# Vandermode/TFPnP

Hardware: AMD Instinct MI355X
Metric: PnP-ADMM iters/sec (and images/sec) at env_batch=48, 256x256, 30 inner iters (higher is better)
Workload: dtype f32 (v_mfma_f32_32x32x2_f32; Winograd F(2x2,3x3) on the layers with cout % 32 == 0); 1 GPU; CS-MRI ADMM 256x256 env_batch=48/GPU radial x4 sigma_n=15, 6 solver calls x 5 inner iters + PSNR reward, no early stop; global_batch=48, parallelism=single GPU

## Files before the change

### include/pnpx.h

```cpp
#ifndef PNPX_H
#define PNPX_H

#include <stddef.h>
#include <stdint.h>

#ifdef __cplusplus
extern "C" {
#endif

typedef struct pnpx_ctx pnpx_ctx;

enum pnpx_status {
  PNPX_OK = 0,
  PNPX_ERR_ARG = 1,
  PNPX_ERR_SHAPE = 2,
  PNPX_ERR_NO_WEIGHTS = 3,
  PNPX_ERR_ALLOC = 4,
  PNPX_ERR_HIP = 5,
  PNPX_ERR_RANGE = 6
};

const char* pnpx_version(void);
const char* pnpx_last_error(void);

int pnpx_ctx_create(int device, pnpx_ctx** out);
int pnpx_ctx_destroy(pnpx_ctx* ctx);
int pnpx_ctx_reserve(pnpx_ctx* ctx, int B, int H, int W);
int pnpx_ctx_set_option(pnpx_ctx* ctx, const char* key, int value);
int pnpx_ctx_get_option(pnpx_ctx* ctx, const char* key, int* value);
int pnpx_ctx_status(pnpx_ctx* ctx);
size_t pnpx_ctx_bytes(const pnpx_ctx* ctx);

size_t pnpx_unet_num_params(void);
int pnpx_unet_load(pnpx_ctx* ctx, const float* params_host, size_t n_params);
int pnpx_unet_denoise(pnpx_ctx* ctx, const float* x, const float* sigma, float* out, float* out_preclamp,
                      int B, int H, int W, void* stream);
size_t pnpx_drunet_num_params(int nb);
int pnpx_drunet_load(pnpx_ctx* ctx, const float* params_host, size_t n_params, int nb);
int pnpx_unet_denoise_backward(pnpx_ctx* ctx, const float* x, const float* sigma, const float* grad_out,
                               float* grad_x, float* grad_sigma, int B, int H, int W, void* stream);
int pnpx_unet_denoise_train(pnpx_ctx* ctx, const float* x, const float* sigma, float* out, int B, int H, int W,
                            unsigned long long* ticket, void* stream);
int pnpx_unet_denoise_backward_ticket(pnpx_ctx* ctx, const float* x, const float* sigma, const float* grad_out,
                                      float* grad_x, float* grad_sigma, int B, int H, int W, unsigned long long ticket,
                                      void* stream);
int pnpx_unet_profile(pnpx_ctx* ctx, const float* x, const float* sigma, float* out, int B, int H, int W,
                      void* stream, int cap, float* ms_out, double* flops_out, const char** names_out,
                      int* n_out);

size_t pnpx_policy_num_params(int num_inputs, int n_det, int spi_head);
int pnpx_policy_load(pnpx_ctx* ctx, const float* params_host, size_t n_params, int num_inputs, int n_det,
                     int spi_head);
int pnpx_policy_forward(pnpx_ctx* ctx, const float* ob, float* probs, float* det, int B, int H, int W,
                        void* stream);
int pnpx_policy_load_device(pnpx_ctx* ctx, const float* params_dev, size_t n_params, int num_inputs, int n_det, int spi_head,
                            void* stream);
int pnpx_policy_params(pnpx_ctx* ctx, float* dst_dev, size_t n_params, void* stream);
int pnpx_policy_forward_train(pnpx_ctx* ctx, const float* ob, float* probs, float* det, int B, int H, int W, float momentum,
                              int update_running, void* stream);
size_t pnpx_policy_num_bn_channels(void);
int pnpx_policy_bn_stats(pnpx_ctx* ctx, float* mean_dev, float* var_dev, size_t n, void* stream);
int pnpx_policy_param_grad(pnpx_ctx* ctx, const float* ob, const float* grad_probs , const float* grad_det ,
                           float* grad_params, size_t n_params, int B, int H, int W, void* stream);
int pnpx_policy_forward_train_keep(pnpx_ctx* ctx, const float* ob, float* probs, float* det, int B, int H, int W, float momentum,
                                   int update_running, void* stream);
int pnpx_policy_param_grad_kept(pnpx_ctx* ctx, const float* grad_probs , const float* grad_det ,
                                float* grad_params, size_t n_params, void* stream);
int pnpx_policy_adam_step(pnpx_ctx* ctx, const float* grad_dev, size_t n_params, float lr, float beta1, float beta2, float eps,
                          float max_norm, float* grad_norm_dev, void* stream);
int pnpx_policy_optim_state(pnpx_ctx* ctx, float* exp_avg_dst, float* exp_avg_sq_dst, size_t n_params, long long* step_host,
                            void* stream);
int pnpx_policy_optim_reset(pnpx_ctx* ctx);
int pnpx_policy_frozen_ranges(int num_inputs, int n_det, int spi_head, size_t* first, size_t* count, int capacity);

size_t pnpx_critic_num_params(int num_inputs);
int pnpx_critic_load(pnpx_ctx* ctx, const float* params_host, size_t n_params, int num_inputs);
int pnpx_critic_load_device(pnpx_ctx* ctx, const float* params_dev, size_t n_params, int num_inputs, void* stream);
int pnpx_critic_soft_update(pnpx_ctx* ctx, const float* src_params_dev, size_t n_params, float one_minus_tau, float tau,
                            void* stream);
int pnpx_critic_params(pnpx_ctx* ctx, float* dst_dev, size_t n_params, void* stream);
int pnpx_critic_forward(pnpx_ctx* ctx, const float* ob, float* value, int B, int H, int W, void* stream);
int pnpx_critic_backward(pnpx_ctx* ctx, const float* ob, const float* grad_value, float* grad_ob, int B, int H, int W,
                         void* stream);

int pnpx_critic_param_grad(pnpx_ctx* ctx, const float* ob, const float* grad_value, float* grad_params, size_t n_params, int B,
                           int H, int W, void* stream);
int pnpx_critic_value_loss_grad(pnpx_ctx* ctx, const float* ob, const float* q_target, float* value, float* loss, float* grad_params,
                                size_t n_params, int B, int H, int W, void* stream);
int pnpx_critic_adam_step(pnpx_ctx* ctx, const float* grad_dev, size_t n_params, float lr, float beta1, float beta2, float eps,
                          float max_norm, float* grad_norm_dev, void* stream);
int pnpx_critic_optim_state(pnpx_ctx* ctx, float* exp_avg_dst, float* exp_avg_sq_dst, size_t n_params, long long* step_host,
                            void* stream);
int pnpx_critic_optim_reset(pnpx_ctx* ctx);

int pnpx_fft2(pnpx_ctx* ctx, const float* in, float* out, int n_img, int H, int W, int inverse,
              int centered, void* stream);
int pnpx_cdp_forward(pnpx_ctx* ctx, const float* x, const float* mask, float* out, int B, int S, int H,
                     int W, void* stream);
int pnpx_cdp_backward(pnpx_ctx* ctx, const float* y, const float* mask, float* out, int B, int S, int H,
                      int W, void* stream);
int pnpx_spi_inverse(pnpx_ctx* ctx, const float* ztilde, const float* K1, const float* K, const float* mu,
                     float* out, int B, int H, int W, void* stream);
int pnpx_psnr(pnpx_ctx* ctx, const float* output, const float* gt, float* psnr, int B, int n_per_item,
              void* stream);

int pnpx_rows_gather(pnpx_ctx* ctx, int n_tensors, const void* const* src_host, void* const* dst_host,
                     const size_t* row_bytes_host, const int64_t* idx, int n_rows, void* stream);
int pnpx_rows_scatter(pnpx_ctx* ctx, int n_tensors, const void* const* src_host, void* const* dst_host,
                      const size_t* row_bytes_host, const int64_t* idx, int n_rows, void* stream);
int pnpx_ring_store(pnpx_ctx* ctx, int n_tensors, const void* const* src_host, void* const* dst_host,
                    const size_t* row_bytes_host, int64_t first_slot, int64_t capacity, int n_rows, void* stream);
int pnpx_live_compact(pnpx_ctx* ctx, const int64_t* idx_left, const int64_t* idx_stop, int n, int64_t* idx_out,
                      int* n_live_host, void* stream);
int pnpx_policy_ob_pack(pnpx_ctx* ctx, int n_entries, const void* const* src_host, const int* kind_host,
                        const int* channels_host, const int64_t* idx, int n_rows, int H, int W, float* out,
                        void* stream);

int pnpx_policy_ob_unpack(pnpx_ctx* ctx, int n_entries, void* const* dst_host, const int* kind_host,
                          const int* channels_host, int n_rows, int H, int W, const float* grad_out, void* stream);


int pnpx_csmri_admm(pnpx_ctx* ctx, const float* vars_in, float* vars_out, const float* y0,
                    const uint8_t* mask, const float* sigma_d, const float* mu, int param_stride, int B,
                    int H, int W, int T, void* stream);
int pnpx_csmri_admm_train(pnpx_ctx* ctx, const float* vars_in, float* vars_out, const float* y0,
                          const uint8_t* mask, const float* sigma_d, const float* mu, int param_stride, int B,
                          int H, int W, int T, float* saved, unsigned long long* ticket, void* stream);
int pnpx_csmri_admm_backward(pnpx_ctx* ctx, const float* y0, const uint8_t* mask, const float* sigma_d,
                             const float* mu, int param_stride, const float* saved, const float* grad_vars_out,
                             float* grad_vars_in, float* grad_sigma_d, float* grad_mu, float* work, int B, int H,
                             int W, int T, unsigned long long ticket, void* stream);
int pnpx_csmri_hqs(pnpx_ctx* ctx, const float* vars_in, float* vars_out, const float* y0,
                   const uint8_t* mask, const float* sigma_d, const float* mu, int param_stride, int B,
                   int H, int W, int T, void* stream);
int pnpx_csmri_hqs_train(pnpx_ctx* ctx, const float* vars_in, float* vars_out, const float* y0,
                         const uint8_t* mask, const float* sigma_d, const float* mu, int param_stride, int B,
                         int H, int W, int T, float* saved, unsigned long long* ticket, void* stream);
int pnpx_csmri_hqs_backward(pnpx_ctx* ctx, const float* y0, const uint8_t* mask, const float* sigma_d,
                            const float* mu, int param_stride, const float* saved, const float* grad_vars_out,
                            float* grad_vars_in, float* grad_sigma_d, float* grad_mu, float* work, int B, int H,
                            int W, int T, unsigned long long ticket, void* stream);
int pnpx_csmri_pg(pnpx_ctx* ctx, const float* vars_in, float* vars_out, const float* y0,
                  const uint8_t* mask, const float* sigma_d, const float* tau, int param_stride, int B,
                  int H, int W, int T, void* stream);
int pnpx_csmri_pg_train(pnpx_ctx* ctx, const float* vars_in, float* vars_out, const float* y0,
                        const uint8_t* mask, const float* sigma_d, const float* tau, int param_stride, int B,
                        int H, int W, int T, float* saved, unsigned long long* ticket, void* stream);
int pnpx_csmri_pg_backward(pnpx_ctx* ctx, const float* y0, const uint8_t* mask, const float* sigma_d,
                           const float* tau, int param_stride, const float* saved, const float* grad_vars_out,
                           float* grad_vars_in, float* grad_sigma_d, float* grad_tau, float* work, int B, int H,
                           int W, int T, unsigned long long ticket, void* stream);
int pnpx_csmri_apg(pnpx_ctx* ctx, const float* vars_in, float* vars_out, const float* y0,
                   const uint8_t* mask, const float* sigma_d, const float* tau, const float* beta,
                   int param_stride, int B, int H, int W, int T, void* stream);
int pnpx_csmri_apg_train(pnpx_ctx* ctx, const float* vars_in, float* vars_out, const float* y0,
                         const uint8_t* mask, const float* sigma_d, const float* tau, const float* beta,
                         int param_stride, int B, int H, int W, int T, float* saved, unsigned long long* ticket,
                         void* stream);
int pnpx_csmri_apg_backward(pnpx_ctx* ctx, const float* y0, const uint8_t* mask, const float* sigma_d,
                            const float* tau, const float* beta, int param_stride, const float* saved,
                            const float* grad_vars_out, float* grad_vars_in, float* grad_sigma_d, float* grad_tau,
                            float* grad_beta, float* work, int B, int H, int W, int T, unsigned long long ticket,
                            void* stream);
int pnpx_csmri_redadmm(pnpx_ctx* ctx, const float* vars_in, float* vars_out, const float* y0,
                       const uint8_t* mask, const float* sigma_d, const float* mu, const float* lamda,
                       int param_stride, int B, int H, int W, int T, void* stream);
int pnpx_csmri_redadmm_train(pnpx_ctx* ctx, const float* vars_in, float* vars_out, const float* y0,
                             const uint8_t* mask, const float* sigma_d, const float* mu, const float* lamda,
                             int param_stride, int B, int H, int W, int T, float* saved, unsigned long long* ticket,
                             void* stream);
int pnpx_csmri_redadmm_backward(pnpx_ctx* ctx, const float* y0, const uint8_t* mask, const float* sigma_d,
                                const float* mu, const float* lamda, int param_stride, const float* saved,
                                const float* grad_vars_out, float* grad_vars_in, float* grad_sigma_d, float* grad_mu,
                                float* grad_lamda, float* work, int B, int H, int W, int T, unsigned long long ticket,
                                void* stream);
int pnpx_csmri_amp(pnpx_ctx* ctx, const float* vars_in, float* vars_out, const float* y0, const uint8_t* mask,
                   const float* sigma_d, const float* probe, int param_stride, int B, int H, int W, int T,
                   void* stream);
int pnpx_pr_iadmm(pnpx_ctx* ctx, const float* vars_in, float* vars_out, const float* y0,
                  const float* mask, const float* sigma_d, const float* mu, const float* tau,
                  int param_stride, int B, int S, int H, int W, int T, void* stream);
int pnpx_pr_iadmm_train(pnpx_ctx* ctx, const float* vars_in, float* vars_out, const float* y0, const float* mask,
                        const float* sigma_d, const float* mu, const float* tau, int param_stride, int B, int S,
                        int H, int W, int T, float* saved, unsigned long long* ticket, void* stream);
int pnpx_pr_iadmm_backward(pnpx_ctx* ctx, const float* y0, const float* mask, const float* sigma_d, const float* mu,
                           const float* tau, int param_stride, const float* saved, const float* grad_vars_out,
                           float* grad_vars_in, float* grad_sigma_d, float* grad_mu, float* grad_tau, float* work,
                           int B, int S, int H, int W, int T, unsigned long long ticket, void* stream);
int pnpx_pr_pg(pnpx_ctx* ctx, const float* vars_in, float* vars_out, const float* y0, const float* mask,
               const float* sigma_d, const float* tau, int param_stride, int B, int S, int H, int W, int T,
               void* stream);
int pnpx_pr_pg_train(pnpx_ctx* ctx, const float* vars_in, float* vars_out, const float* y0, const float* mask,
                     const float* sigma_d, const float* tau, int param_stride, int B, int S, int H, int W, int T,
                     float* saved, unsigned long long* ticket, void* stream);
int pnpx_pr_pg_backward(pnpx_ctx* ctx, const float* y0, const float* mask, const float* sigma_d, const float* tau,
                        int param_stride, const float* saved, const float* grad_vars_out, float* grad_vars_in,
                        float* grad_sigma_d, float* grad_tau, float* work, int B, int S, int H, int W, int T,
                        unsigned long long ticket, void* stream);
int pnpx_spi_admm(pnpx_ctx* ctx, const float* vars_in, float* vars_out, const float* x0,
                  const float* Kmap, const float* sigma_d, const float* mu, int param_stride, int B, int H,
                  int W, int T, void* stream);
int pnpx_spi_admm_train(pnpx_ctx* ctx, const float* vars_in, float* vars_out, const float* x0, const float* Kmap,
                        const float* sigma_d, const float* mu, int param_stride, int B, int H, int W, int T,
                        float* saved, unsigned long long* ticket, void* stream);
int pnpx_spi_admm_backward(pnpx_ctx* ctx, const float* x0, const float* Kmap, const float* sigma_d, const float* mu,
                           int param_stride, const float* saved, const float* grad_vars_out, float* grad_vars_in,
                           float* grad_sigma_d, float* grad_mu, float* work, int B, int H, int W, int T,
                           unsigned long long ticket, void* stream);

int pnpx_radon_det_count(int R);
int pnpx_radon_forward(pnpx_ctx* ctx, const float* img, float* sino, int B, int R, int n_view, void* stream);
int pnpx_radon_backprojection(pnpx_ctx* ctx, const float* sino, float* img, int B, int R, int n_view,
                              void* stream);
int pnpx_ct_iadmm(pnpx_ctx* ctx, const float* vars_in, float* vars_out, const float* y0, int n_view,
                  float opnorm, const float* sigma_d, const float* mu, const float* tau, int param_stride,
                  int B, int R, int T, void* stream);
int pnpx_ct_iadmm_train(pnpx_ctx* ctx, const float* vars_in, float* vars_out, const float* y0, int n_view,
                        float opnorm, const float* sigma_d, const float* mu, const float* tau, int param_stride, int B,
                        int R, int T, float* saved, unsigned long long* ticket, void* stream);
int pnpx_ct_iadmm_backward(pnpx_ctx* ctx, int n_view, float opnorm, const float* sigma_d, const float* mu,
                           const float* tau, int param_stride, const float* saved, const float* grad_vars_out,
                           float* grad_vars_in, float* grad_sigma_d, float* grad_mu, float* grad_tau, float* work,
                           int B, int R, int T, unsigned long long ticket, void* stream);
int pnpx_ct_pg(pnpx_ctx* ctx, const float* vars_in, float* vars_out, const float* y0, int n_view,
               float opnorm, const float* sigma_d, const float* tau, int param_stride, int B, int R, int T,
               void* stream);
int pnpx_ct_pg_train(pnpx_ctx* ctx, const float* vars_in, float* vars_out, const float* y0, int n_view, float opnorm,
                     const float* sigma_d, const float* tau, int param_stride, int B, int R, int T, float* saved,
                     unsigned long long* ticket, void* stream);
int pnpx_ct_pg_backward(pnpx_ctx* ctx, int n_view, float opnorm, const float* sigma_d, const float* tau,
                        int param_stride, const float* saved, const float* grad_vars_out, float* grad_vars_in,
                        float* grad_sigma_d, float* grad_tau, float* work, int B, int R, int T,
                        unsigned long long ticket, void* stream);

void pnpx_winof4_matrices(double* g18, double* bt36, double* at24);
int pnpx_winof4_pack(const float* w, int cout, int cin, float* dst);
int pnpx_winof4_c32_pack(const float* w, int cout, int cin, float* dst);

enum pnpx_probe_kind {
  PNPX_PROBE_DIRECT = 0,
  PNPX_PROBE_WINO4 = 1,
  PNPX_PROBE_WINO8 = 2,
  PNPX_PROBE_WINO8_KSPLIT = 3,
  PNPX_PROBE_WINOF4 = 4,
  PNPX_PROBE_WINO8_UPS = 5,
  PNPX_PROBE_DIRECT_GRAD = 6,
  PNPX_PROBE_WINO8_GRAD = 7,
  PNPX_PROBE_WINOF4_2SRC = 8,
  PNPX_PROBE_WINOF4_UPS = 9,
  PNPX_PROBE_WINOF4_FUSE_UP = 11,
  PNPX_PROBE_WINOF4_C32 = 12
};
int pnpx_conv3x3_probe(pnpx_ctx* ctx, int kind, const float* w_host, const float* bias_host, int cout, const float* in0, int C0,
                       const float* in1, int C1, float* out, const float* res, const float* mask, float slope, float* pool_out,
                       int ks_rule, int B, int H, int W, void* stream);
int pnpx_conv3x3_probe_plan(int kind, int C0, int C1, int cout, int H, int W, int ks_rule);
int pnpx_upsample2x_probe(pnpx_ctx* ctx, const float* src, float* dst, int planes, int h, int w, void* stream);

typedef struct pnpx_conv_hs_probe_desc {
  const float *w, *bias, *outc_w, *outc_b, *first_w, *first_b;
  const void *in0, *in1, *res, *dmask;
  void *out, *pool_out;
  const float *x_in, *first_x, *first_sigma;
  float *out_img, *out_pre;
  int cin, cout, G0, G1, B, H, W;
  float slope;
  int taps, in0_groups, wreg, share, ups_h, ups_w, critic_epi;
  float alpha;
  int res_groups, first_sigma_stride;
  float first_slope;
  int want_range_flag;
  unsigned* range_flag_out;
} pnpx_conv_hs_probe_desc;
enum { PNPX_CONV_HS_PLAN_INTS = 12 };
int pnpx_conv_hs_probe(pnpx_ctx* ctx, const pnpx_conv_hs_probe_desc* desc, void* stream);
int pnpx_conv_hs_probe_plan(const pnpx_conv_hs_probe_desc* desc, int B, int H, int W, int* out);

enum pnpx_vjp_glue_op {
  PNPX_VJP_OUTC_BWD = 0,
  PNPX_VJP_UPSAMPLE_BWD = 1,
  PNPX_VJP_SKIP_POOL_MERGE = 2,
  PNPX_VJP_INPUT_GRAD = 3,
  PNPX_VJP_GRAD_SCALE = 4
};
typedef struct pnpx_vjp_glue_probe_desc {
  int op, family, form;
  int B, C, H, W, Ccat, c_off, Ht, Wt;
  const void *g, *act, *g_pool;
  const float *pre, *w, *g_res, *sc;
  void* out;
  float *out_res, *part, *gsigma;
  unsigned* bits;
} pnpx_vjp_glue_probe_desc;
int pnpx_vjp_glue_probe(pnpx_ctx* ctx, const pnpx_vjp_glue_probe_desc* desc, void* stream);
int pnpx_vjp_glue_probe_plan(const pnpx_vjp_glue_probe_desc* desc);

int pnpx_conv_f32_entry_plan(int opts, int ksplit, int ksplit_rule, int C0, int C1, int cout, int H, int W, int B_call);
int pnpx_conv_f32_forward_plan(int opts, int ksplit, int ksplit_rule, int C0, int C1, int cout, int H, int W, int B_call);

#ifdef __cplusplus
}
#endif
#endif
```

### tfpnp_amd/_lib.py

```python
import ctypes as C
import os
import threading

import torch

_HERE = os.path.dirname(os.path.abspath(__file__))
LIB_PATH = os.environ.get("PNPX_LIB", os.path.join(_HERE, "libpnpx.so"))

_lib = None
_lock = threading.Lock()

c_float_p = C.POINTER(C.c_float)
c_void_p = C.c_void_p


class PnpxError(RuntimeError):
    pass


PNPX_ERR_RANGE = 6


class ConvHsProbeDesc(C.Structure):
    _fields_ = ([(n, c_void_p) for n in ("w", "bias", "outc_w", "outc_b", "first_w", "first_b", "in0", "in1", "res", "dmask", "out", "pool_out",
                                         "x_in", "first_x", "first_sigma", "out_img", "out_pre")] +
                [(n, C.c_int) for n in ("cin", "cout", "G0", "G1", "B", "H", "W")] + [("slope", C.c_float)] +
                [(n, C.c_int) for n in ("taps", "in0_groups", "wreg", "share", "ups_h", "ups_w", "critic_epi")] + [("alpha", C.c_float)] +
                [("res_groups", C.c_int), ("first_sigma_stride", C.c_int), ("first_slope", C.c_float), ("want_range_flag", C.c_int),
                 ("range_flag_out", C.POINTER(C.c_uint))])
PNPX_CONV_HS_PLAN_INTS = 12


class VjpGlueProbeDesc(C.Structure):
    _fields_ = ([(n, C.c_int) for n in ("op", "family", "form", "B", "C", "H", "W", "Ccat", "c_off", "Ht", "Wt")] +
                [(n, c_void_p) for n in ("g", "act", "g_pool", "pre", "w", "g_res", "sc", "out", "out_res", "part", "gsigma", "bits")])


_P = c_void_p
_SIGNATURES = {
    "pnpx_version": (C.c_char_p, []),
    "pnpx_last_error": (C.c_char_p, []),
    "pnpx_ctx_create": (C.c_int, [C.c_int, C.POINTER(c_void_p)]),
    "pnpx_ctx_destroy": (C.c_int, [c_void_p]),
    "pnpx_ctx_reserve": (C.c_int, [c_void_p, C.c_int, C.c_int, C.c_int]),
    "pnpx_ctx_set_option": (C.c_int, [c_void_p, C.c_char_p, C.c_int]),
    "pnpx_ctx_get_option": (C.c_int, [c_void_p, C.c_char_p, C.POINTER(C.c_int)]),
    "pnpx_ctx_status": (C.c_int, [c_void_p]),
    "pnpx_ctx_bytes": (C.c_size_t, [c_void_p]),
    "pnpx_unet_num_params": (C.c_size_t, []),
    "pnpx_unet_load": (C.c_int, [c_void_p, c_void_p, C.c_size_t]),
    "pnpx_drunet_num_params": (C.c_size_t, [C.c_int]),
    "pnpx_drunet_load": (C.c_int, [c_void_p, c_void_p, C.c_size_t, C.c_int]),
    "pnpx_unet_denoise": (C.c_int, [c_void_p, _P, _P, _P, _P, C.c_int, C.c_int, C.c_int, c_void_p]),
    "pnpx_unet_denoise_backward": (C.c_int, [c_void_p, _P, _P, _P, _P, _P, C.c_int, C.c_int, C.c_int, c_void_p]),
    "pnpx_unet_denoise_train": (C.c_int, [c_void_p, _P, _P, _P, C.c_int, C.c_int, C.c_int, C.POINTER(C.c_ulonglong), c_void_p]),
    "pnpx_unet_denoise_backward_ticket": (C.c_int, [c_void_p, _P, _P, _P, _P, _P, C.c_int, C.c_int, C.c_int,
                                                    C.c_ulonglong, c_void_p]),
    "pnpx_policy_num_params": (C.c_size_t, [C.c_int, C.c_int, C.c_int]),
    "pnpx_policy_load": (C.c_int, [c_void_p, c_void_p, C.c_size_t, C.c_int, C.c_int, C.c_int]),
    "pnpx_policy_load_device": (C.c_int, [c_void_p, _P, C.c_size_t, C.c_int, C.c_int, C.c_int, c_void_p]),
    "pnpx_policy_params": (C.c_int, [c_void_p, _P, C.c_size_t, c_void_p]),
    "pnpx_policy_forward": (C.c_int, [c_void_p, _P, _P, _P, C.c_int, C.c_int, C.c_int, c_void_p]),
    "pnpx_policy_forward_train": (C.c_int, [c_void_p, _P, _P, _P, C.c_int, C.c_int, C.c_int, C.c_float, C.c_int, c_void_p]),
    "pnpx_policy_num_bn_channels": (C.c_size_t, []),
    "pnpx_policy_bn_stats": (C.c_int, [c_void_p, _P, _P, C.c_size_t, c_void_p]),
    "pnpx_policy_param_grad": (C.c_int, [c_void_p, _P, _P, _P, _P, C.c_size_t, C.c_int, C.c_int, C.c_int, c_void_p]),
    "pnpx_policy_forward_train_keep": (C.c_int, [c_void_p, _P, _P, _P, C.c_int, C.c_int, C.c_int, C.c_float, C.c_int, c_void_p]),
    "pnpx_policy_param_grad_kept": (C.c_int, [c_void_p, _P, _P, _P, C.c_size_t, c_void_p]),
    "pnpx_policy_adam_step": (C.c_int, [c_void_p, _P, C.c_size_t] + [C.c_float] * 5 + [_P, c_void_p]),
    "pnpx_policy_optim_state": (C.c_int, [c_void_p, _P, _P, C.c_size_t, C.POINTER(C.c_longlong), c_void_p]),
    "pnpx_policy_optim_reset": (C.c_int, [c_void_p]),
    "pnpx_policy_frozen_ranges": (C.c_int, [C.c_int, C.c_int, C.c_int, C.POINTER(C.c_size_t), C.POINTER(C.c_size_t), C.c_int]),
    "pnpx_critic_num_params": (C.c_size_t, [C.c_int]),
    "pnpx_critic_load": (C.c_int, [c_void_p, c_void_p, C.c_size_t, C.c_int]),
    "pnpx_critic_load_device": (C.c_int, [c_void_p, _P, C.c_size_t, C.c_int, c_void_p]),
    "pnpx_critic_soft_update": (C.c_int, [c_void_p, _P, C.c_size_t, C.c_float, C.c_float, c_void_p]),
    "pnpx_critic_params": (C.c_int, [c_void_p, _P, C.c_size_t, c_void_p]),
    "pnpx_critic_forward": (C.c_int, [c_void_p, _P, _P, C.c_int, C.c_int, C.c_int, c_void_p]),
    "pnpx_critic_backward": (C.c_int, [c_void_p, _P, _P, _P, C.c_int, C.c_int, C.c_int, c_void_p]),
    "pnpx_critic_param_grad": (C.c_int, [c_void_p, _P, _P, _P, C.c_size_t, C.c_int, C.c_int, C.c_int, c_void_p]),
    "pnpx_critic_value_loss_grad": (C.c_int, [c_void_p, _P, _P, _P, _P, _P, C.c_size_t, C.c_int, C.c_int, C.c_int, c_void_p]),
    "pnpx_critic_adam_step": (C.c_int, [c_void_p, _P, C.c_size_t] + [C.c_float] * 5 + [_P, c_void_p]),
    "pnpx_critic_optim_state": (C.c_int, [c_void_p, _P, _P, C.c_size_t, C.POINTER(C.c_longlong), c_void_p]),
    "pnpx_critic_optim_reset": (C.c_int, [c_void_p]),
    "pnpx_unet_profile": (C.c_int, [c_void_p, _P, _P, _P, C.c_int, C.c_int, C.c_int, c_void_p, C.c_int,
                                    c_float_p, C.POINTER(C.c_double), C.POINTER(C.c_char_p), C.POINTER(C.c_int)]),
    "pnpx_fft2": (C.c_int, [c_void_p, _P, _P, C.c_int, C.c_int, C.c_int, C.c_int, C.c_int, c_void_p]),
    "pnpx_cdp_forward": (C.c_int, [c_void_p, _P, _P, _P, C.c_int, C.c_int, C.c_int, C.c_int, c_void_p]),
    "pnpx_cdp_backward": (C.c_int, [c_void_p, _P, _P, _P, C.c_int, C.c_int, C.c_int, C.c_int, c_void_p]),
    "pnpx_spi_inverse": (C.c_int, [c_void_p, _P, _P, _P, _P, _P, C.c_int, C.c_int, C.c_int, c_void_p]),
    "pnpx_psnr": (C.c_int, [c_void_p, _P, _P, _P, C.c_int, C.c_int, c_void_p]),
    "pnpx_rows_gather": (C.c_int, [c_void_p, C.c_int, C.POINTER(c_void_p), C.POINTER(c_void_p), C.POINTER(C.c_size_t), _P,
                                   C.c_int, c_void_p]),
    "pnpx_rows_scatter": (C.c_int, [c_void_p, C.c_int, C.POINTER(c_void_p), C.POINTER(c_void_p), C.POINTER(C.c_size_t), _P,
                                    C.c_int, c_void_p]),
    "pnpx_ring_store": (C.c_int, [c_void_p, C.c_int, C.POINTER(c_void_p), C.POINTER(c_void_p), C.POINTER(C.c_size_t),
                                  C.c_int64, C.c_int64, C.c_int, c_void_p]),
    "pnpx_live_compact": (C.c_int, [c_void_p, _P, _P, C.c_int, _P, C.POINTER(C.c_int), c_void_p]),
    "pnpx_policy_ob_pack": (C.c_int, [c_void_p, C.c_int, C.POINTER(c_void_p), C.POINTER(C.c_int), C.POINTER(C.c_int), _P,
                                      C.c_int, C.c_int, C.c_int, _P, c_void_p]),
    "pnpx_policy_ob_unpack": (C.c_int, [c_void_p, C.c_int, C.POINTER(c_void_p), C.POINTER(C.c_int), C.POINTER(C.c_int),
                                        C.c_int, C.c_int, C.c_int, _P, c_void_p]),
    "pnpx_csmri_admm": (C.c_int, [c_void_p, _P, _P, _P, _P, _P, _P] + [C.c_int] * 5 + [c_void_p]),
    "pnpx_csmri_admm_train": (C.c_int, [c_void_p, _P, _P, _P, _P, _P, _P] + [C.c_int] * 5 +
                              [_P, C.POINTER(C.c_ulonglong), c_void_p]),
    "pnpx_csmri_admm_backward": (C.c_int, [c_void_p, _P, _P, _P, _P, C.c_int, _P, _P, _P, _P, _P, _P] + [C.c_int] * 4 +
                                 [C.c_ulonglong, c_void_p]),
    "pnpx_csmri_hqs_train": (C.c_int, [c_void_p, _P, _P, _P, _P, _P, _P] + [C.c_int] * 5 +
                             [_P, C.POINTER(C.c_ulonglong), c_void_p]),
    "pnpx_csmri_hqs_backward": (C.c_int, [c_void_p, _P, _P, _P, _P, C.c_int, _P, _P, _P, _P, _P, _P] + [C.c_int] * 4 +
                                [C.c_ulonglong, c_void_p]),
    "pnpx_csmri_hqs": (C.c_int, [c_void_p, _P, _P, _P, _P, _P, _P] + [C.c_int] * 5 + [c_void_p]),
    "pnpx_csmri_amp": (C.c_int, [c_void_p, _P, _P, _P, _P, _P, _P] + [C.c_int] * 5 + [c_void_p]),
    "pnpx_csmri_pg_train": (C.c_int, [c_void_p, _P, _P, _P, _P, _P, _P] + [C.c_int] * 5 +
                            [_P, C.POINTER(C.c_ulonglong), c_void_p]),
    "pnpx_csmri_pg_backward": (C.c_int, [c_void_p, _P, _P, _P, _P, C.c_int, _P, _P, _P, _P, _P, _P] + [C.c_int] * 4 +
                               [C.c_ulonglong, c_void_p]),
    "pnpx_csmri_pg": (C.c_int, [c_void_p, _P, _P, _P, _P, _P, _P] + [C.c_int] * 5 + [c_void_p]),
    "pnpx_csmri_apg_train": (C.c_int, [c_void_p, _P, _P, _P, _P, _P, _P, _P] + [C.c_int] * 5 +
                             [_P, C.POINTER(C.c_ulonglong), c_void_p]),
    "pnpx_csmri_apg_backward": (C.c_int, [c_void_p, _P, _P, _P, _P, _P, C.c_int, _P, _P, _P, _P, _P, _P, _P] + [C.c_int] * 4 +
                                [C.c_ulonglong, c_void_p]),
    "pnpx_csmri_apg": (C.c_int, [c_void_p, _P, _P, _P, _P, _P, _P, _P] + [C.c_int] * 5 + [c_void_p]),
    "pnpx_csmri_redadmm_train": (C.c_int, [c_void_p, _P, _P, _P, _P, _P, _P, _P] + [C.c_int] * 5 +
                                 [_P, C.POINTER(C.c_ulonglong), c_void_p]),
    "pnpx_csmri_redadmm_backward": (C.c_int, [c_void_p, _P, _P, _P, _P, _P, C.c_int, _P, _P, _P, _P, _P, _P, _P] +
                                    [C.c_int] * 4 + [C.c_ulonglong, c_void_p]),
    "pnpx_csmri_redadmm": (C.c_int, [c_void_p, _P, _P, _P, _P, _P, _P, _P] + [C.c_int] * 5 + [c_void_p]),
    "pnpx_pr_iadmm_train": (C.c_int, [c_void_p, _P, _P, _P, _P, _P, _P, _P] + [C.c_int] * 6 +
                            [_P, C.POINTER(C.c_ulonglong), c_void_p]),
    "pnpx_pr_iadmm_backward": (C.c_int, [c_void_p, _P, _P, _P, _P, _P, C.c_int, _P, _P, _P, _P, _P, _P, _P] + [C.c_int] * 5 +
                               [C.c_ulonglong, c_void_p]),
    "pnpx_pr_iadmm": (C.c_int, [c_void_p, _P, _P, _P, _P, _P, _P, _P] + [C.c_int] * 6 + [c_void_p]),
    "pnpx_pr_pg_train": (C.c_int, [c_void_p, _P, _P, _P, _P, _P, _P] + [C.c_int] * 6 +
                         [_P, C.POINTER(C.c_ulonglong), c_void_p]),
    "pnpx_pr_pg_backward": (C.c_int, [c_void_p, _P, _P, _P, _P, C.c_int, _P, _P, _P, _P, _P, _P] + [C.c_int] * 5 +
                            [C.c_ulonglong, c_void_p]),
    "pnpx_pr_pg": (C.c_int, [c_void_p, _P, _P, _P, _P, _P, _P] + [C.c_int] * 6 + [c_void_p]),
    "pnpx_spi_admm_train": (C.c_int, [c_void_p, _P, _P, _P, _P, _P, _P] + [C.c_int] * 5 +
                            [_P, C.POINTER(C.c_ulonglong), c_void_p]),
    "pnpx_spi_admm_backward": (C.c_int, [c_void_p, _P, _P, _P, _P, C.c_int, _P, _P, _P, _P, _P, _P] + [C.c_int] * 4 +
                               [C.c_ulonglong, c_void_p]),
    "pnpx_spi_admm": (C.c_int, [c_void_p, _P, _P, _P, _P, _P, _P] + [C.c_int] * 5 + [c_void_p]),
    "pnpx_radon_det_count": (C.c_int, [C.c_int]),
    "pnpx_radon_forward": (C.c_int, [c_void_p, _P, _P, C.c_int, C.c_int, C.c_int, c_void_p]),
    "pnpx_radon_backprojection": (C.c_int, [c_void_p, _P, _P, C.c_int, C.c_int, C.c_int, c_void_p]),
    "pnpx_ct_iadmm_train": (C.c_int, [c_void_p, _P, _P, _P, C.c_int, C.c_float, _P, _P, _P] + [C.c_int] * 4 +
                            [_P, C.POINTER(C.c_ulonglong), c_void_p]),
    "pnpx_ct_iadmm_backward": (C.c_int, [c_void_p, C.c_int, C.c_float, _P, _P, _P, C.c_int, _P, _P, _P, _P, _P, _P, _P] +
                               [C.c_int] * 3 + [C.c_ulonglong, c_void_p]),
    "pnpx_ct_pg_train": (C.c_int, [c_void_p, _P, _P, _P, C.c_int, C.c_float, _P, _P] + [C.c_int] * 4 +
                         [_P, C.POINTER(C.c_ulonglong), c_void_p]),
    "pnpx_ct_pg_backward": (C.c_int, [c_void_p, C.c_int, C.c_float, _P, _P, C.c_int, _P, _P, _P, _P, _P, _P] +
                            [C.c_int] * 3 + [C.c_ulonglong, c_void_p]),
    "pnpx_ct_iadmm": (C.c_int, [c_void_p, _P, _P, _P, C.c_int, C.c_float, _P, _P, _P] + [C.c_int] * 4 + [c_void_p]),
    "pnpx_ct_pg": (C.c_int, [c_void_p, _P, _P, _P, C.c_int, C.c_float, _P, _P] + [C.c_int] * 4 + [c_void_p]),
    "pnpx_winof4_matrices": (None, [c_void_p, c_void_p, c_void_p]),
    "pnpx_winof4_pack": (C.c_int, [c_void_p, C.c_int, C.c_int, c_void_p]),
    "pnpx_conv3x3_probe": (C.c_int, [c_void_p, C.c_int, c_void_p, c_void_p, C.c_int, _P, C.c_int, _P, C.c_int, _P, _P, _P, C.c_float, _P,
                                     C.c_int, C.c_int, C.c_int, C.c_int, c_void_p]),
    "pnpx_conv3x3_probe_plan": (C.c_int, [C.c_int] * 7),
    "pnpx_upsample2x_probe": (C.c_int, [c_void_p, _P, _P, C.c_int, C.c_int, C.c_int, c_void_p]),
    "pnpx_conv_f32_entry_plan": (C.c_int, [C.c_int] * 9),
    "pnpx_conv_f32_forward_plan": (C.c_int, [C.c_int] * 9),
    "pnpx_winof4_c32_pack": (C.c_int, [c_void_p, C.c_int, C.c_int, c_void_p]),
    "pnpx_conv_hs_probe": (C.c_int, [c_void_p, c_void_p, c_void_p]),
    "pnpx_conv_hs_probe_plan": (C.c_int, [c_void_p, C.c_int, C.c_int, C.c_int, C.POINTER(C.c_int)]),
    "pnpx_vjp_glue_probe": (C.c_int, [c_void_p, c_void_p, c_void_p]),
    "pnpx_vjp_glue_probe_plan": (C.c_int, [c_void_p]),
}
EXPORTED_SYMBOLS = tuple(_SIGNATURES)


def lib():
    global _lib
    if _lib is None:
        with _lock:
            if _lib is None:
                if not os.path.exists(LIB_PATH):
                    raise PnpxError(
                        f"{LIB_PATH} not found: the HIP library has not been built "
                        "(run `make -C tfpnp_amd/csrc` or __graft_entry__.build()). There is no CPU fallback.")
                l = C.CDLL(LIB_PATH)
                missing = []
                for name, (res, args) in _SIGNATURES.items():
                    try:
                        fn = getattr(l, name)
                    except AttributeError:
                        if "PNPX_LIB" in os.environ:
                            missing.append(name)
                            continue
                        raise
                    fn.restype = res
                    fn.argtypes = args
                if missing:
                    import warnings
                    warnings.warn(f"PNPX_LIB={LIB_PATH} lacks {len(missing)} symbol(s) of include/pnpx.h: "
                                  + ", ".join(missing) + " -- calls to them will fail with AttributeError")
                _lib = l
    return _lib


def check(status):
    if status != 0:
        msg = lib().pnpx_last_error().decode("utf-8", "replace")
        raise PnpxError(f"pnpx call failed (status {status}): {msg}")
```

### tfpnp_amd/csrc/api.hip

```cpp
#include <climits>
#include <cstring>

#include "common.h"
#include "conv3x3.h"
#include "conv_hs.h"
#include "solver_loop.h"

namespace pnpx {

static thread_local std::string g_err;

void set_error(const char* fmt, ...) {
  char buf[1024];
  va_list ap;
  va_start(ap, fmt);
  vsnprintf(buf, sizeof(buf), fmt, ap);
  va_end(ap);
  g_err = buf;
}

int hip_fail(hipError_t e, const char* what, const char* file, int line) {
  set_error("HIP error %d (%s) at %s:%d in %s", (int)e, hipGetErrorString(e), file, line, what);
  return PNPX_ERR_HIP;
}
// ... 213 lines not shown
                          float max_norm, float* grad_norm_dev, void* stream) {
  LOCK_CTX(ctx);
  return policy_adam_step(ctx, grad_dev, n_params, lr, beta1, beta2, eps, max_norm, grad_norm_dev, static_cast<hipStream_t>(stream));
}

int pnpx_policy_optim_state(pnpx_ctx* ctx, float* exp_avg_dst, float* exp_avg_sq_dst, size_t n_params, long long* step_host,
                            void* stream) {
  LOCK_CTX(ctx);
  return policy_optim_state(ctx, exp_avg_dst, exp_avg_sq_dst, n_params, step_host, static_cast<hipStream_t>(stream));
}

int pnpx_policy_optim_reset(pnpx_ctx* ctx) {
  LOCK_CTX(ctx);
  return policy_optim_reset(ctx);
}

int pnpx_policy_frozen_ranges(int num_inputs, int n_det, int spi_head, size_t* first, size_t* count, int capacity) {
  if (num_inputs < 1 || num_inputs > 64 || n_det < 1 || n_det > 64) return -1;
  FrozenRange r[LIVE_OPTIM_MAX_FROZEN];
  int n = 0;
  if (policy_frozen_ranges(num_inputs, n_det, spi_head, r, &n) != PNPX_OK) return -1;
  for (int i = 0; i < n && i < capacity && first && count; ++i) {
    first[i] = r[i].first;
    count[i] = r[i].count;
  }
  return n;
}

size_t pnpx_policy_num_bn_channels(void) { return POLICY_BN_CHANNELS; }

int pnpx_policy_bn_stats(pnpx_ctx* ctx, float* mean_dev, float* var_dev, size_t n, void* stream) {
  LOCK_CTX(ctx);
  return policy_bn_stats(ctx, mean_dev, var_dev, n, static_cast<hipStream_t>(stream));
}

size_t pnpx_critic_num_params(int num_inputs) {
  return (num_inputs >= 1 && num_inputs <= 64) ? critic_num_params(num_inputs) : 0;
}

int pnpx_critic_load(pnpx_ctx* ctx, const float* params_host, size_t n_params, int num_inputs) {
  LOCK_CTX(ctx);
  return critic_load(ctx, params_host, n_params, num_inputs);
}

int pnpx_critic_load_device(pnpx_ctx* ctx, const float* params_dev, size_t n_params, int num_inputs, void* stream) {
  LOCK_CTX(ctx);
  return critic_load_device(ctx, params_dev, n_params, num_inputs, static_cast<hipStream_t>(stream));
}

int pnpx_critic_soft_update(pnpx_ctx* ctx, const float* src_params_dev, size_t n_params, float one_minus_tau, float tau,
                            void* stream) {
  LOCK_CTX(ctx);
  return critic_soft_update(ctx, src_params_dev, n_params, one_minus_tau, tau, static_cast<hipStream_t>(stream));
}

int pnpx_critic_params(pnpx_ctx* ctx, float* dst_dev, size_t n_params, void* stream) {
  LOCK_CTX(ctx);
  return critic_params(ctx, dst_dev, n_params, static_cast<hipStream_t>(stream));
}

int pnpx_critic_forward(pnpx_ctx* ctx, const float* ob, float* value, int B, int H, int W, void* stream) {
  LOCK_CTX(ctx);
  if (!ob || !value) {
    set_error("pnpx_critic_forward: null pointer");
    return PNPX_ERR_ARG;
  }
  return critic_forward(ctx, ob, value, B, H, W, static_cast<hipStream_t>(stream));
}

int pnpx_critic_backward(pnpx_ctx* ctx, const float* ob, const float* grad_value, float* grad_ob, int B, int H, int W,
                         void* stream) {
  LOCK_CTX(ctx);
  if (!ob || !grad_value || !grad_ob) {
    set_error("pnpx_critic_backward: null pointer");
    return PNPX_ERR_ARG;
  }
  return critic_backward(ctx, ob, grad_value, grad_ob, B, H, W, static_cast<hipStream_t>(stream));
}

int pnpx_critic_param_grad(pnpx_ctx* ctx, const float* ob, const float* grad_value, float* grad_params, size_t n_params, int B, int H,
                           int W, void* stream) {
  LOCK_CTX(ctx);
  if (!ob || !grad_value || !grad_params) {
    set_error("pnpx_critic_param_grad: null pointer");
    return PNPX_ERR_ARG;
  }
  return critic_param_grad(ctx, ob, grad_value, grad_params, n_params, B, H, W, static_cast<hipStream_t>(stream));
}

int pnpx_critic_value_loss_grad(pnpx_ctx* ctx, const float* ob, const float* q_target, float* value, float* loss, float* grad_params,
                                size_t n_params, int B, int H, int W, void* stream) {
  LOCK_CTX(ctx);
  if (!ob || !q_target || !value || !loss || !grad_params) {
    set_error("pnpx_critic_value_loss_grad: null pointer");
    return PNPX_ERR_ARG;
  }
  return critic_value_loss_grad(ctx, ob, q_target, value, loss, grad_params, n_params, B, H, W, static_cast<hipStream_t>(stream));
}

int pnpx_critic_adam_step(pnpx_ctx* ctx, const float* grad_dev, size_t n_params, float lr, float beta1, float beta2, float eps,
                          float max_norm, float* grad_norm_dev, void* stream) {
  LOCK_CTX(ctx);
  return critic_adam_step(ctx, grad_dev, n_params, lr, beta1, beta2, eps, max_norm, grad_norm_dev, static_cast<hipStream_t>(stream));
}

int pnpx_critic_optim_state(pnpx_ctx* ctx, float* exp_avg_dst, float* exp_avg_sq_dst, size_t n_params, long long* step_host,
                            void* stream) {
  LOCK_CTX(ctx);
  return critic_optim_state(ctx, exp_avg_dst, exp_avg_sq_dst, n_params, step_host, static_cast<hipStream_t>(stream));
}

int pnpx_critic_optim_reset(pnpx_ctx* ctx) {
  LOCK_CTX(ctx);
  return critic_optim_reset(ctx);
}

int pnpx_ctx_reserve(pnpx_ctx* ctx, int B, int H, int W) {
  LOCK_CTX(ctx);
  if (B <= 0 || H < 16 || W < 16) {
    set_error("pnpx_ctx_reserve: need B > 0 and H, W >= 16");
    return PNPX_ERR_SHAPE;
  }
  return ctx_reserve_unet(ctx, B, H, W);
}

namespace {
struct PlainOption {
  const char* name;
  int pnpx_ctx::*field;
  int lo, hi;
};
const PlainOption PLAIN_OPTIONS[] = {
    {"conv_mode", &pnpx_ctx::conv_mode, CONV_F32, CONV_HS},
    {"subbatch", &pnpx_ctx::opt_subbatch, 0, INT_MAX},
    {"fuse_pool", &pnpx_ctx::opt_fuse_pool, 0, 1},
    {"fuse_outc", &pnpx_ctx::opt_fuse_outc, 0, 1},
    {"fuse_first", &pnpx_ctx::opt_fuse_first, 0, 1},
    {"fold_first", &pnpx_ctx::opt_fold_first, 0, 1},
    {"fft_tile", &pnpx_ctx::opt_fft_tile, 0, 8192},
    {"fft_fast", &pnpx_ctx::opt_fft_fast, 0, 1},
    {"fft_affine", &pnpx_ctx::opt_fft_affine, 0, 1},
    {"chains", &pnpx_ctx::opt_chains, 0, 8},
    {"wreg", &pnpx_ctx::opt_wreg, 0, 2},
    {"fuse_up", &pnpx_ctx::opt_fuse_up, 0, 2},
    {"fp32_winograd", &pnpx_ctx::opt_fp32_winograd, 0, 1},
    {"fp32_chains", &pnpx_ctx::opt_fp32_chains, 0, 8},
    {"fp32_fuse_up", &pnpx_ctx::opt_fp32_fuse_up, 0, 1},
    {"fp32_ksplit", &pnpx_ctx::opt_fp32_ksplit, 0, 2},
    {"fp32_ksplit_rule", &pnpx_ctx::opt_ksplit_rule, 1, 255},
    {"fp32_wino8_layers", &pnpx_ctx::opt_fp32_wino8, 0, (1 << 27) - 1},
    {"fp32_winof4_layers", &pnpx_ctx::opt_fp32_winof4, 0, (1 << 27) - 1},
    {"fp32_winof4_entries", &pnpx_ctx::opt_fp32_winof4_entries, 0, (1 << 27) - 1},
    {"fp32_winof4_fuse_up", &pnpx_ctx::opt_fp32_winof4_fuse_up, 0, (1 << 27) - 1},
};
constexpr int WINOF4_C32_BITS = (1 << 1) | (1 << 2) | (1 << 25);
const PlainOption* plain_option(const char* key) {
  for (const PlainOption& o : PLAIN_OPTIONS)
    if (key && !std::strcmp(key, o.name)) return &o;
  return nullptr;
}
}

int pnpx_ctx_set_option(pnpx_ctx* ctx, const char* key, int value) {
  LOCK_CTX(ctx);
  auto is = [&](const char* k) { return key && !std::strcmp(key, k); };
  if (const PlainOption* o = plain_option(key)) {
    if (value >= o->lo && value <= o->hi) {
      ctx->*(o->field) = value;
      return PNPX_OK;
    }
  }
  if (is("fp32_winof4_c32") && value >= 0 && (value & ~WINOF4_C32_BITS) == 0) {
    ctx->opt_fp32_winof4_c32 = value;
    return PNPX_OK;
  }
  if (is("drunet_shift") && value >= 0 && value <= 8 && (value & 3) == 0) {
    ctx->drunet.shift = value;
    return PNPX_OK;
  }
  if (is("policy_s2_hs") && (value == 0 || value == 1)) return PNPX_OK;
  if (is("range_guard") && value >= 0 && value <= 2) {
    PNPX_HIP(hipDeviceSynchronize());
    ctx->opt_range_guard = value;
    ctx->range_tripped = false;
    *ctx->range_flag_host = 0;
    return PNPX_OK;
  }
  if (is("train_cache_gb") && value >= -1) {
    ctx->opt_train_cache_gb = value;
    ctx->train_alloc_failed = false;
    ctx->train_budget_bytes = 0;
    if (value == 0) pnpx::train_cache_free(ctx);
    return PNPX_OK;
  }
  if (is("train_cache_release")) {
    pnpx::train_cache_free(ctx);
    ctx->train_alloc_failed = false;
    ctx->train_budget_bytes = 0;
    return PNPX_OK;
  }
  set_error("pnpx_ctx_set_option: unknown option '%s' or bad value %d", key ? key : "(null)", value);
  return PNPX_ERR_ARG;
}

int pnpx_ctx_get_option(pnpx_ctx* ctx, const char* key, int* value) {
  LOCK_CTX(ctx);
  auto is = [&](const char* k) { return key && !std::strcmp(key, k); };
  if (!value) {
    set_error("pnpx_ctx_get_option: null value pointer");
    return PNPX_ERR_ARG;
  }
  if (const PlainOption* o = plain_option(key)) *value = ctx->*(o->field);
  else if (is("fp32_winof4_c32")) *value = ctx->opt_fp32_winof4_c32;
  else if (is("drunet_shift")) *value = ctx->drunet.shift;
  else if (is("policy_s2_hs")) *value = 1;
  else if (is("range_guard")) *value = ctx->opt_range_guard;
  else if (is("train_cache_gb")) *value = ctx->opt_train_cache_gb;
  else {
    set_error("pnpx_ctx_get_option: unknown option '%s'", key ? key : "(null)");
    return PNPX_ERR_ARG;
  }
  return PNPX_OK;
}

int pnpx_ctx_status(pnpx_ctx* ctx) {
  LOCK_CTX(ctx);
  range_guard_enter(ctx);
  if (ctx->range_tripped) {
    if (ctx->drunet.loaded)
      set_error("half-split range guard tripped: an activation of an earlier DRUNet call left the f16 hi/lo range (|v| >= 4095 "
                "or NaN); that call's output is invalid.  The context now runs %s (the bias-free network is positively "
                "homogeneous: inputs scaled by 2^-%d, the tail multiplies back; a trip at 2^-8 selects exact fp32); acknowledge "
                "with pnpx_ctx_set_option(ctx, \"range_guard\", 1)", ctx->conv_mode == CONV_HS ? "re-scaled passes" : "conv_mode 0",
                ctx->drunet.shift);
    else
    set_error("half-split range guard tripped: an activation of an earlier call left the f16 hi/lo range (|v| >= 4095 or "
              "NaN); that call's output is invalid.  The context now runs conv_mode 0 (exact fp32 MFMA); re-arm with "
              "pnpx_ctx_set_option(ctx, \"range_guard\", 1)");
    return PNPX_ERR_RANGE;
  }
  return PNPX_OK;
}

size_t pnpx_ctx_bytes(const pnpx_ctx* ctx) {
  if (!ctx) return 0;
  size_t n = ctx->weights.bytes + ctx->arena.buf.bytes + ctx->arena_grad.buf.bytes + ctx->scratch.bytes +
             ctx->drunet.weights.bytes + ctx->drunet.arena.bytes + ctx->drunet.arena_grad.bytes + ctx->drunet.f32_weights.bytes +
             ctx->drunet.f32_arena.bytes + ctx->drunet.f32_weights_bwd.bytes + ctx->drunet.f32_arena_grad.bytes +
             ctx->policy.weights.bytes + ctx->policy.arena.bytes + ctx->policy.live.master.bytes + ctx->policy.pack_ws.ws.bytes + ctx->policy.raw.weights.bytes + ctx->policy.raw_ws.ws.bytes +
             ctx->policy.train_ws.bytes + ctx->policy.bn_buf.bytes + ctx->policy.optim.state.bytes + ctx->critic.weights.bytes + ctx->critic.arena.bytes +
             ctx->critic.live.master.bytes + ctx->critic.pack_ws.ws.bytes + ctx->critic.optim.state.bytes;
  for (const auto& sl : ctx->train_ring) n += sl.arena.buf.bytes + sl.pre.bytes;
  return n;
}

size_t pnpx_unet_num_params(void) {
  LayerSpec L[27];
  unet_layers(L);
  size_t n = 0;
  for (int i = 0; i < 27; ++i) n += (size_t)L[i].cin * L[i].cout * 9 + L[i].cout;
  return n + 32 + 1;
}

size_t pnpx_drunet_num_params(int nb) { return (nb >= 1 && nb <= 8) ? pnpx::drunet_num_params(nb) : 0; }

int pnpx_drunet_load(pnpx_ctx* ctx, const float* params_host, size_t n_params, int nb) {
  LOCK_CTX(ctx);
  return pnpx::drunet_load(ctx, params_host, n_params, nb);
}

int pnpx_unet_load(pnpx_ctx* ctx, const float* params_host, size_t n_params) {
  LOCK_CTX(ctx);
  pnpx::drunet_free(ctx);
  if (!params_host || n_params != pnpx_unet_num_params()) {
    set_error("pnpx_unet_load: expected %zu parameters, got %zu", pnpx_unet_num_params(), n_params);
    return PNPX_ERR_ARG;
  }
  LayerSpec L[27];
  unet_layers(L);
  std::vector<float> host;
  size_t woff[27], boff[27];
  auto align = [&]() { host.resize((host.size() + 255) & ~(size_t)255, 0.f); };
  const float* src = params_host;
  for (int i = 0; i < 27; ++i) {
    const int mt = conv_pack_mt(L[i].cout), cc = conv_pack_cc(L[i].cin);
    align();
    woff[i] = host.size();
    host.resize(host.size() + (size_t)L[i].cin * L[i].cout * 9);
    pack_conv_weights(src, L[i].cout, L[i].cin, mt, cc, host.data() + woff[i]);
    src += (size_t)L[i].cin * L[i].cout * 9;
    align();
    boff[i] = host.size();
    host.insert(host.end(), src, src + L[i].cout);
    src += L[i].cout;
    ctx->conv[i].cin = L[i].cin;
    ctx->conv[i].cout = L[i].cout;
    ctx->conv[i].mt = mt;
    ctx->conv[i].cc = cc;
  }
  size_t uoff[27];
  {
    const float* wsrc = params_host;
    for (int i = 0; i < 27; ++i) {
      uoff[i] = 0;
      if (conv3x3_wino_packs(L[i].cout, L[i].cin)) {
        align();
        uoff[i] = host.size();
        host.resize(host.size() + conv3x3_wino_floats(L[i].cout, L[i].cin));
        pack_conv_weights_wino(wsrc, L[i].cout, L[i].cin, host.data() + uoff[i]);
      }
      wsrc += (size_t)L[i].cin * L[i].cout * 9 + L[i].cout;
    }
  }
  size_t hoff[27];
  float hscale[27];
  for (int i = 0; i < 27; ++i) {
    const int mt = conv_hs_mt(L[i].cout);
    const int cin_pad = (L[i].cin + 15) / 16 * 16;
    align();
    hoff[i] = host.size();
    const size_t n16 = (size_t)L[i].cout * cin_pad * 9 * 2;
    host.resize(host.size() + (n16 + 1) / 2, 0.f);
    const float* wsrc = params_host;
    for (int k = 0; k < i; ++k) wsrc += (size_t)L[k].cin * L[k].cout * 9 + L[k].cout;
    hscale[i] = pack_conv_weights_hs(wsrc, L[i].cout, L[i].cin, mt, reinterpret_cast<uint16_t*>(host.data() + hoff[i]));
    ctx->conv_hs[i].cin = L[i].cin;
    ctx->conv_hs[i].cout = L[i].cout;
    ctx->conv_hs[i].cin_pad = cin_pad;
    ctx->conv_hs[i].mt = mt;
    ctx->conv_hs[i].inv_scale = 1.0f / (hscale[i] * HS_ASCALE);
  }
  size_t toff[27];
  for (int i = 0; i < 27; ++i) {
    const int cout_pad = (L[i].cin + 31) / 32 * 32;
    const int mt = (cout_pad % 64 == 0) ? 64 : 32;
    align();
    toff[i] = host.size();
    host.resize(host.size() + (size_t)cout_pad * L[i].cout * 9);
    const float* wsrc = params_host;
    for (int k = 0; k < i; ++k) wsrc += (size_t)L[k].cin * L[k].cout * 9 + L[k].cout;
    pack_conv_weights_transposed(wsrc, L[i].cout, L[i].cin, cout_pad, mt, 8, host.data() + toff[i]);
    ctx->conv_bwd[i].cin = L[i].cout;
    ctx->conv_bwd[i].cout = cout_pad;
    ctx->conv_bwd[i].mt = mt;
    ctx->conv_bwd[i].cc = 8;
  }
  size_t u4off[27];
  {
    const float* wsrc = params_host;
    for (int i = 0; i < 27; ++i) {
      u4off[i] = 0;
      const bool plain = (i >= 3 && i <= 11) || i == 16 || i == 17 || i == 19 || i == 20 || i == 22 || i == 23;
      const bool entry = i == 15 || i == 18 || i == 21;
      if ((plain || entry) && conv3x3_winof4_packs(L[i].cout, L[i].cin)) {
        align();
        u4off[i] = host.size();
        host.resize(host.size() + conv3x3_winof4_floats(L[i].cout, L[i].cin));
        pack_conv_weights_winof4(wsrc, L[i].cout, L[i].cin, host.data() + u4off[i]);
      }
      wsrc += (size_t)L[i].cin * L[i].cout * 9 + L[i].cout;
    }
  }
  size_t u4c32off[27];
  {
    const float* wsrc = params_host;
    for (int i = 0; i < 27; ++i) {
      u4c32off[i] = 0;
      if (((WINOF4_C32_BITS >> i) & 1) && conv3x3_winof4_c32_packs(L[i].cout, L[i].cin)) {
        align();
        u4c32off[i] = host.size();
        host.resize(host.size() + conv3x3_winof4_floats(L[i].cout, L[i].cin));
        pack_conv_weights_winof4_c32(wsrc, L[i].cout, L[i].cin, host.data() + u4c32off[i]);
      }
      wsrc += (size_t)L[i].cin * L[i].cout * 9 + L[i].cout;
    }
  }
  size_t thoff[27], tuoff[27];
  float thscale[27];
  {
    std::vector<float> wt;
    for (int i = 0; i < 27; ++i) {
      const int cin_t = L[i].cout;
      const int cout_t = (L[i].cin + 31) / 32 * 32;
      const int mt = (cout_t % 64 == 0) ? 64 : 32;
      const float* wsrc = params_host;
      for (int k = 0; k < i; ++k) wsrc += (size_t)L[k].cin * L[k].cout * 9 + L[k].cout;
      transpose_flip_conv_weights(wsrc, L[i].cout, L[i].cin, cout_t, wt);
      align();
      thoff[i] = host.size();
      const size_t n16 = (size_t)cout_t * cin_t * 9 * 2;
      host.resize(host.size() + (n16 + 1) / 2, 0.f);
      thscale[i] = pack_conv_weights_hs(wt.data(), cout_t, cin_t, mt, reinterpret_cast<uint16_t*>(host.data() + thoff[i]));
      tuoff[i] = 0;
      if (conv3x3_wino_packs(cout_t, cin_t)) {
        align();
        tuoff[i] = host.size();
        host.resize(host.size() + conv3x3_wino_floats(cout_t, cin_t));
        pack_conv_weights_wino(wt.data(), cout_t, cin_t, host.data() + tuoff[i]);
      }
      ctx->conv_hs_bwd[i].cin = cin_t;
      ctx->conv_hs_bwd[i].cout = cout_t;
      ctx->conv_hs_bwd[i].cin_pad = cin_t;
      ctx->conv_hs_bwd[i].mt = mt;
      ctx->conv_hs_bwd[i].inv_scale = 1.0f / (thscale[i] * HS_ASCALE);
    }
  }
  align();
  const size_t oc0 = host.size();
  host.insert(host.end(), params_host, params_host + 32 * 2 * 9);
  align();
  const size_t ozero = host.size();
  host.resize(host.size() + 768, 0.f);
  align();
  const size_t ow = host.size();
  host.insert(host.end(), src, src + 32);
  src += 32;
  align();
  const size_t ob = host.size();
  host.push_back(*src);
  host.resize(host.size() + 1024, 0.f);
  PNPX_HIP(hipDeviceSynchronize());
  if (ctx->weights.p) PNPX_HIP(hipFree(ctx->weights.p));
  ctx->weights = DeviceBuf();
  ctx->has_weights = false;
  void* p = nullptr;
  hipError_t e = hipMalloc(&p, host.size() * sizeof(float));
  if (e != hipSuccess) {
    set_error("weight allocation of %zu bytes failed: %s", host.size() * sizeof(float), hipGetErrorString(e));
    return PNPX_ERR_ALLOC;
  }
  PNPX_HIP(hipMemcpy(p, host.data(), host.size() * sizeof(float), hipMemcpyHostToDevice));
  float* d = static_cast<float*>(p);
  for (int i = 0; i < 27; ++i) {
    ctx->conv[i].w = d + woff[i];
    ctx->conv[i].b = d + boff[i];
    ctx->conv_wino_u[i] = uoff[i] ? d + uoff[i] : nullptr;
    ctx->conv_wino_u_bwd[i] = tuoff[i] ? d + tuoff[i] : nullptr;
    ctx->conv_winof4_u[i] = u4off[i] ? d + u4off[i] : nullptr;
    ctx->conv_winof4_c32_u[i] = u4c32off[i] ? d + u4c32off[i] : nullptr;
    ctx->conv_hs[i].w = reinterpret_cast<char*>(d + hoff[i]);
    ctx->conv_bwd[i].w = d + toff[i];
    ctx->conv_bwd[i].b = nullptr;
    ctx->conv_hs_bwd[i].w = reinterpret_cast<char*>(d + thoff[i]);
  }
  ctx->conv0_w = d + oc0;
  ctx->zero_bias = d + ozero;
  ctx->outc_w = d + ow;
  ctx->outc_b = d + ob;
  ctx->weights.p = p;
  ctx->weights.bytes = host.size() * sizeof(float);
  ctx->has_weights = true;
  pnpx::train_cache_free(ctx);
  return PNPX_OK;
}

int pnpx_unet_denoise(pnpx_ctx* ctx, const float* x, const float* sigma, float* out, float* out_preclamp, int B,
                      int H, int W, void* stream) {
  LOCK_CTX(ctx);
  return pnpx::guarded(ctx, static_cast<hipStream_t>(stream), [&]() -> int {
  if (!x || !sigma || !out) {
    set_error("pnpx_unet_denoise: null pointer");
    return PNPX_ERR_ARG;
  }
  return unet_denoise(ctx, x, sigma, 1, out, out_preclamp, B, H, W, static_cast<hipStream_t>(stream), nullptr);
  });
}

int pnpx_unet_denoise_backward(pnpx_ctx* ctx, const float* x, const float* sigma, const float* grad_out, float* grad_x,
                               float* grad_sigma, int B, int H, int W, void* stream) {
  LOCK_CTX(ctx);
  return pnpx::guarded(ctx, static_cast<hipStream_t>(stream), [&]() -> int {
  if (!x || !sigma || !grad_out || !grad_x || !grad_sigma) {
    set_error("pnpx_unet_denoise_backward: null pointer");
    return PNPX_ERR_ARG;
  }
  return unet_denoise_backward(ctx, x, sigma, 1, grad_out, grad_x, grad_sigma, B, H, W, static_cast<hipStream_t>(stream));
  });
}

int pnpx_unet_denoise_train(pnpx_ctx* ctx, const float* x, const float* sigma, float* out, int B, int H, int W,
                            unsigned long long* ticket, void* stream) {
  LOCK_CTX(ctx);
  return pnpx::guarded(ctx, static_cast<hipStream_t>(stream), [&]() -> int {
    if (!x || !sigma || !out || !ticket) {
      set_error("pnpx_unet_denoise_train: null pointer");
      return PNPX_ERR_ARG;
    }
    return unet_denoise_train(ctx, x, sigma, 1, out, B, H, W, static_cast<hipStream_t>(stream), ticket);
  });
}

int pnpx_unet_denoise_backward_ticket(pnpx_ctx* ctx, const float* x, const float* sigma, const float* grad_out,
                                      float* grad_x, float* grad_sigma, int B, int H, int W, unsigned long long ticket,
                                      void* stream) {
  LOCK_CTX(ctx);
  return pnpx::guarded(ctx, static_cast<hipStream_t>(stream), [&]() -> int {
    if (!x || !sigma || !grad_out || !grad_x || !grad_sigma) {
      set_error("pnpx_unet_denoise_backward_ticket: null pointer");
      return PNPX_ERR_ARG;
    }
    return unet_denoise_backward_ticket(ctx, x, sigma, 1, grad_out, grad_x, grad_sigma, B, H, W,
                                        static_cast<hipStream_t>(stream), ticket);
  });
}

int pnpx_unet_profile(pnpx_ctx* ctx, const float* x, const float* sigma, float* out, int B, int H, int W,
                      void* stream, int cap, float* ms_out, double* flops_out, const char** names_out, int* n_out) {
  LOCK_CTX(ctx);
  if (!x || !sigma || !out || !ms_out || !flops_out || !names_out || !n_out || cap <= 0) {
    set_error("pnpx_unet_profile: null pointer");
    return PNPX_ERR_ARG;
  }
  hipStream_t s = static_cast<hipStream_t>(stream);
  PNPX_TRY(unet_denoise(ctx, x, sigma, 1, out, nullptr, B, H, W, s, nullptr));
  while (ctx->events.size() < 1024) {
    hipEvent_t e;
    PNPX_HIP(hipEventCreate(&e));
    ctx->events.push_back(e);
  }
  ProfileSink sink;
  sink.events = &ctx->events;
  PNPX_TRY(unet_denoise(ctx, x, sigma, 1, out, nullptr, B, H, W, s, &sink));
  PNPX_HIP(hipStreamSynchronize(s));
  int n = sink.n < cap ? sink.n : cap;
  for (int i = 0; i < n; ++i) {
    float ms = 0.f;
    PNPX_HIP(hipEventElapsedTime(&ms, ctx->events[i], ctx->events[i + 1]));
    ms_out[i] = ms;
    flops_out[i] = sink.flops[i];
    names_out[i] = sink.names[i];
  }
  *n_out = n;
  return PNPX_OK;
}

int pnpx_fft2(pnpx_ctx* ctx, const float* in, float* out, int n_img, int H, int W, int inverse, int centered,
              void* stream) {
  LOCK_CTX(ctx);
  if (!in || !out) {
    set_error("pnpx_fft2: null pointer");
    return PNPX_ERR_ARG;
  }
  return fft2(ctx, in, out, n_img, H, W, inverse != 0, centered != 0, static_cast<hipStream_t>(stream));
}

}
```

### tfpnp_amd/csrc/common.h

```cpp
#pragma once
#include <hip/hip_runtime.h>

#include <cstdarg>
#include <cstdint>
#include <cstdio>
#include <map>
#include <mutex>
#include <string>
#include <vector>

#include "pnpx.h"

namespace pnpx {

void set_error(const char* fmt, ...);
int hip_fail(hipError_t e, const char* what, const char* file, int line);

#define PNPX_HIP(expr)                                                       \
  do {                                                                       \
    hipError_t _e = (expr);                                                  \
    if (_e != hipSuccess) return ::pnpx::hip_fail(_e, #expr, __FILE__, __LINE__); \
  } while (0)
#define PNPX_TRY(expr)          \
  do {                          \
// ... 22 lines not shown
struct DeviceBuf {
  void* p = nullptr;
  size_t bytes = 0;
};
int alloc_dev(DeviceBuf& b, size_t bytes, const char* what);

}
#include "live_params.h"
namespace pnpx {

struct UNetArena {
  DeviceBuf buf;
  int capB = 0, capH = 0, capW = 0, mode = -1;
};

struct ConvLayerHsDev {
  int cin = 0, cout = 0, cin_pad = 0, mt = 0;
  char* w = nullptr;
  float inv_scale = 1.f;
};

enum ConvMode { CONV_F32 = 0, CONV_HS = 1 };

struct PolicyPack {
  ConvLayerHsDev hs[21];
  const float* hs_bias[21] = {};
  const float* fc_sm_w = nullptr;
  const float* fc_sm_b = nullptr;
  const float* fc_det_w = nullptr;
  const float* fc_det_b = nullptr;
  const float* fc_det2_w = nullptr;
  const float* fc_det2_b = nullptr;
  DeviceBuf weights;
};
struct PolicyNet : PolicyPack {
  bool loaded = false;
  int num_inputs = 0, cin_pad = 0, n_det = 0, spi_head = 0;
  DeviceBuf arena;
  int capB = 0, capH = 0, capW = 0;
  LiveParams live;
  PackWorkspace pack_ws;
  PolicyPack raw;
  PackWorkspace raw_ws;
  bool raw_valid = false, eval_stale = false;
  DeviceBuf train_ws;
  int tcapB = 0, tcapH = 0, tcapW = 0;
  DeviceBuf bn_buf;
  bool bn_have_stats = false;
  ConvLayerHsDev raw_bwd[21];
  DeviceBuf raw_adj, raw_adj_table;
  const float* raw_adj_zero = nullptr;
  bool adj_valid = false;
  DeviceBuf grad_ws;
  int gcapB = 0, gcapH = 0, gcapW = 0;
  DeviceBuf grad_slab;
  bool kept_valid = false;
  int keptB = 0, keptH = 0, keptW = 0, kept_capB = 0, kept_capH = 0, kept_capW = 0;
  const char* kept_lost = "no pnpx_policy_forward_train_keep has run on this actor";
  LiveOptim optim;
};
inline void policy_kept_drop(PolicyNet& N, const char* why) {
  if (N.kept_valid) N.kept_lost = why;
  N.kept_valid = false;
}

struct CriticNet {
  bool loaded = false;
  int num_inputs = 0, cin_pad = 0;
  ConvLayerHsDev fwd[21], bwd[21];
  const float* bias[21] = {};
  float alpha[21] = {};
  const float* fc_w = nullptr;
  const float* fc_b = nullptr;
  const float* zero = nullptr;
  float fc_wmax = 0.f;
  DeviceBuf weights, arena;
  int capB = 0, capH = 0, capW = 0;
  LiveParams live;
  PackWorkspace pack_ws;
  DeviceBuf grad_m, grad_wm, grad_slab;
  LiveOptim optim;
};

int launch_chains(const pnpx_ctx* ctx, int B, int H, int W);
void join_side_streams_after_failure(pnpx_ctx* ctx);
struct DruNet {
  bool loaded = false;
  int nb = 0;
  std::vector<ConvLayerHsDev> layers;
  std::vector<int> taps;
  const float* head_w = nullptr;
  const float* zero = nullptr;
  const float* e0 = nullptr;
  int shift = 0;
  std::vector<ConvLayerHsDev> layers_bwd;
  const float* tail_bwd_w = nullptr;
  DeviceBuf weights, arena, arena_grad;
  std::vector<float> params_host;
  bool f32_ready = false;
  std::vector<ConvLayer> f32_layers;
  std::vector<const float*> f32_wino;
  DeviceBuf f32_weights, f32_arena;
  int f32_capB = 0, f32_capH = 0, f32_capW = 0;
  bool f32_arena_keeps = false;
  bool f32_bwd_ready = false;
  std::vector<ConvLayer> f32_layers_bwd;
  std::vector<const float*> f32_wino_bwd;
  DeviceBuf f32_weights_bwd, f32_arena_grad;
  int f32_gcapB = 0, f32_gcapH = 0, f32_gcapW = 0;
  int capB = 0, capH = 0, capW = 0;
  bool arena_keeps = false;
  int gcapB = 0, gcapH = 0, gcapW = 0;
};

}

struct pnpx_ctx {
  int device = 0;
  std::mutex mu;
  bool has_weights = false;
  pnpx::ConvLayer conv[27];
  pnpx::ConvLayerHsDev conv_hs[27];
  int conv_mode = pnpx::CONV_F32;
  int opt_subbatch = 24;
  int opt_fuse_pool = 1;
  int opt_fuse_outc = 1;
  int opt_fuse_first = 1;
  int opt_fuse_up = 1;
  int opt_fold_first = 0;
  int opt_fft_tile = 0;
  int opt_fft_fast = 1;
  int opt_fft_affine = 1;
  int lds_block_limit = 0;
  int opt_chains = 0;
  std::vector<hipStream_t> side_streams;
  std::vector<hipEvent_t> ev_pool;
  size_t ev_next = 0;
  int opt_wreg = 2;
  int opt_range_guard = 1;
  int opt_train_cache_gb = -1;
  size_t train_budget_bytes = 0;
  unsigned* range_flag_host = nullptr;
  unsigned* range_flag_dev = nullptr;
  bool range_tripped = false;
  float* conv_wino_u[27] = {};
  float* conv_wino_u_bwd[27] = {};
  int opt_fp32_winograd = 1;
  int opt_fp32_wino8 = (1 << 27) - 1;
  float* conv_winof4_u[27] = {};
  int opt_fp32_winof4 = (0x1ff << 3) | (3 << 16) | (3 << 19) | (3 << 22);
  int opt_fp32_winof4_entries = (1 << 15) | (1 << 18) | (1 << 21);
  int opt_fp32_winof4_fuse_up = 1 << 21;
  float* conv_winof4_c32_u[27] = {};
  int opt_fp32_winof4_c32 = (1 << 1) | (1 << 25);
  int opt_fp32_chains = 2;
  int opt_fp32_ksplit = 1;
  int opt_ksplit_rule = 1;
  int opt_fp32_fuse_up = 1;
  pnpx::ConvLayer conv_bwd[27];
  pnpx::ConvLayerHsDev conv_hs_bwd[27];
  float* zero_bias = nullptr;
  float* conv0_w = nullptr;
  float* outc_w = nullptr;
  float* outc_b = nullptr;
  pnpx::DeviceBuf weights;
  pnpx::UNetArena arena, arena_grad;
  struct TrainSlot {
    pnpx::UNetArena arena;
    pnpx::DeviceBuf pre;
    unsigned long long ticket = 0;
    int B = 0;
  };
  std::vector<TrainSlot> train_ring;
  unsigned long long train_counter = 0;
  int train_H = 0, train_W = 0, train_mode = -1;
  bool train_alloc_failed = false;
  pnpx::PolicyNet policy;
  pnpx::CriticNet critic;
  pnpx::DruNet drunet;
  pnpx::DeviceBuf scratch;
  std::map<int, float2*> twiddle;
  std::vector<hipEvent_t> events;
};

namespace pnpx {

int chain_event(pnpx_ctx* ctx, hipEvent_t* ev);
int chain_streams(pnpx_ctx* ctx, int chains);
template <class F>
int fan_out_chains(pnpx_ctx* ctx, int chains, int B, hipStream_t s, F&& run_slice) {
  PNPX_TRY(chain_streams(ctx, chains));
  hipEvent_t fork = nullptr, joins[16] = {};
  PNPX_TRY(chain_event(ctx, &fork));
  PNPX_HIP(hipEventRecord(fork, s));
  auto fail = [&](int rc) {
    join_side_streams_after_failure(ctx);
    return rc;
  };
  auto hip = [&](hipError_t e, const char* what) { return e == hipSuccess ? PNPX_OK : hip_fail(e, what, __FILE__, __LINE__); };
  for (int c = chains - 1; c >= 0; --c) {
    const int lo = (int)((long long)B * c / chains), hi = (int)((long long)B * (c + 1) / chains);
    hipStream_t st = c ? ctx->side_streams[c - 1] : s;
    int rc = c ? hip(hipStreamWaitEvent(st, fork, 0), "hipStreamWaitEvent(fork)") : PNPX_OK;
    if (rc == PNPX_OK) rc = run_slice(lo, hi, st);
    if (rc == PNPX_OK && c) rc = chain_event(ctx, &joins[c]);
    if (rc == PNPX_OK && c) rc = hip(hipEventRecord(joins[c], st), "hipEventRecord(join)");
    if (rc != PNPX_OK) return fail(rc);
  }
  for (int c = 1; c < chains; ++c) {
    const int rc = hip(hipStreamWaitEvent(s, joins[c], 0), "hipStreamWaitEvent(join)");
    if (rc != PNPX_OK) return fail(rc);
  }
  return PNPX_OK;
}

int ctx_reserve_unet(pnpx_ctx* ctx, int B, int H, int W);
int reserve_arena(pnpx_ctx* ctx, UNetArena& ar, int mode, int B, int H, int W, size_t extra_bytes);
int ctx_scratch(pnpx_ctx* ctx, size_t bytes, void** out);
int ctx_twiddle(pnpx_ctx* ctx, int N, const float2** out);
void range_guard_enter(pnpx_ctx* ctx);
int range_guard_strict(pnpx_ctx* ctx, hipStream_t s, bool* rerun);
template <class F>
int guarded(pnpx_ctx* ctx, hipStream_t s, F&& body) {
  range_guard_enter(ctx);
  int st = body();
  for (int attempt = 0; attempt < 4 && st == PNPX_OK && ctx->opt_range_guard == 2 && ctx->conv_mode == CONV_HS; ++attempt) {
    bool rerun = false;
    PNPX_TRY(range_guard_strict(ctx, s, &rerun));
    if (!rerun) break;
    st = body();
  }
  return st;
}

struct ProfileSink {
  std::vector<hipEvent_t>* events = nullptr;
  std::vector<const char*> names;
  std::vector<double> flops;
  int n = 0;
};

int unet_denoise(pnpx_ctx* ctx, const float* x, const float* sigma, int sigma_stride, float* out, float* out_pre,
                 int B, int H, int W, hipStream_t s, ProfileSink* prof, UNetArena* arena = nullptr, int mode = -1,
                 bool keep_all = false);
int unet_denoise_backward(pnpx_ctx* ctx, const float* x, const float* sigma, int sigma_stride, const float* grad_out,
                          float* grad_x, float* grad_sigma, int B, int H, int W, hipStream_t s,
                          UNetArena* cached = nullptr, const float* cached_pre = nullptr);
size_t unet_arena_bytes(int mode, int B, int H, int W);
void train_cache_free(pnpx_ctx* ctx);
int unet_denoise_train(pnpx_ctx* ctx, const float* x, const float* sigma, int sigma_stride, float* out, int B, int H,
                       int W, hipStream_t s, unsigned long long* ticket);
int unet_denoise_backward_ticket(pnpx_ctx* ctx, const float* x, const float* sigma, int sigma_stride,
                                 const float* grad_out, float* grad_x, float* grad_sigma, int B, int H, int W,
                                 hipStream_t s, unsigned long long ticket);

size_t drunet_num_params(int nb);
int drunet_load(pnpx_ctx* ctx, const float* params, size_t n, int nb);
int drunet_denoise(pnpx_ctx* ctx, const float* x, const float* sigma, int sigma_stride, float* out, float* out_pre, int B,
                   int H, int W, hipStream_t s, bool keep_mids = false);
int drunet_denoise_backward(pnpx_ctx* ctx, const float* x, const float* sigma, int sigma_stride, const float* grad_out,
                            float* grad_x, float* grad_sigma, int B, int H, int W, hipStream_t s);
void drunet_free(pnpx_ctx* ctx);
int drunet_denoise_f32(pnpx_ctx* ctx, const float* x, const float* sigma, int sigma_stride, float* out, float* out_pre, int B, int H,
                       int W, hipStream_t s, bool keep_mids = false);
int drunet_denoise_backward_f32(pnpx_ctx* ctx, const float* x, const float* sigma, int sigma_stride, const float* grad_out, float* grad_x,
                                float* grad_sigma, int B, int H, int W, hipStream_t s);
void drunet_f32_free(pnpx_ctx* ctx);

size_t policy_num_params(int num_inputs, int n_det, int spi_head);
int policy_load(pnpx_ctx* ctx, const float* params, size_t n, int num_inputs, int n_det, int spi_head);
int policy_forward(pnpx_ctx* ctx, const float* ob, float* probs, float* det, int B, int H, int W, hipStream_t s);
void policy_free(pnpx_ctx* ctx);
int policy_load_device(pnpx_ctx* ctx, const float* params_dev, size_t n, int num_inputs, int n_det, int spi_head, hipStream_t s);
int policy_params(pnpx_ctx* ctx, float* dst_dev, size_t n, hipStream_t s);
int policy_pack_raw(pnpx_ctx* ctx, hipStream_t s);
int policy_refresh_eval(pnpx_ctx* ctx, hipStream_t s);
struct Packed;
int policy_adopt_host_blob(pnpx_ctx* ctx, const Packed* pk21, const size_t* heads6, size_t total);
int policy_launch_heads(const PolicyPack& P, int n_det, int spi_head, const char* feat_hs, int h, int w, int B, float* probs, float* det,
                         hipStream_t s);
constexpr size_t POLICY_BN_CHANNELS = 4864;
int policy_forward_train(pnpx_ctx* ctx, const float* ob, float* probs, float* det, int B, int H, int W, float momentum, int update_running,
                         hipStream_t s);
int policy_bn_stats(pnpx_ctx* ctx, float* mean_dev, float* var_dev, size_t n, hipStream_t s);
int policy_param_grad(pnpx_ctx* ctx, const float* ob, const float* grad_probs, const float* grad_det, float* grad_params, size_t n, int B,
                      int H, int W, hipStream_t s);
int policy_pack_adj(pnpx_ctx* ctx, hipStream_t s);
int policy_forward_train_keep(pnpx_ctx* ctx, const float* ob, float* probs, float* det, int B, int H, int W, float momentum,
                              int update_running, hipStream_t s);
int policy_param_grad_kept(pnpx_ctx* ctx, const float* grad_probs, const float* grad_det, float* grad_params, size_t n, hipStream_t s);
int policy_frozen_ranges(int num_inputs, int n_det, int spi_head, FrozenRange* out, int* n_out);
int policy_upload_frozen(pnpx_ctx* ctx);
int policy_adam_step(pnpx_ctx* ctx, const float* grad_dev, size_t n, float lr, float beta1, float beta2, float eps, float max_norm,
                     float* grad_norm_dev, hipStream_t s);
int policy_optim_state(pnpx_ctx* ctx, float* exp_avg_dst, float* exp_avg_sq_dst, size_t n, long long* step_host, hipStream_t s);
int policy_optim_reset(pnpx_ctx* ctx);

size_t critic_num_params(int num_inputs);
int critic_load(pnpx_ctx* ctx, const float* params, size_t n, int num_inputs);
int critic_load_device(pnpx_ctx* ctx, const float* params_dev, size_t n, int num_inputs, hipStream_t s);
int critic_soft_update(pnpx_ctx* ctx, const float* src_dev, size_t n, float one_minus_tau, float tau, hipStream_t s);
int critic_params(pnpx_ctx* ctx, float* dst_dev, size_t n, hipStream_t s);
int critic_forward(pnpx_ctx* ctx, const float* ob, float* value, int B, int H, int W, hipStream_t s);
int critic_backward(pnpx_ctx* ctx, const float* ob, const float* grad_value, float* grad_ob, int B, int H, int W, hipStream_t s);
int critic_param_grad(pnpx_ctx* ctx, const float* ob, const float* grad_value, float* grad_params, size_t n, int B, int H, int W,
                      hipStream_t s);
int critic_value_loss_grad(pnpx_ctx* ctx, const float* ob, const float* q_target, float* value, float* loss, float* grad_params, size_t n,
// ... 12 lines not shown
```

### tfpnp_amd/csrc/conv3x3.h

```cpp
#pragma once
#include "common.h"

namespace pnpx {

struct ConvArgs {
  const float* in0;
  const float* in1;
  const float* wpk;
  const float* bias;
  float* out;
  int C0, C1;
  int H, W, Hp, Wp;
  int tilesX, tilesY, nct;
  float slope;
  int mode;
  const float* dmask;
  const char* dmask_hs = nullptr;
  const float* res = nullptr;
};

int conv_pack_mt(int cout);
int conv_pack_cc(int cin);
void pack_conv_weights(const float* w, int cout, int cin, int mt, int cc, float* dst);
int launch_conv3x3(const ConvLayer& L, const float* in0, int C0, const float* in1, int C1, float* out, int B,
                   int H, int W, hipStream_t s);
int launch_conv3x3_act(const ConvLayer& L, const float* in0, int C0, const float* in1, int C1, float* out, int B,
                       int H, int W, float slope, const float* res, hipStream_t s);
int launch_conv1x1_act(const ConvLayer& L, const float* in0, float* out, int B, int H, int W, float slope, const float* res, hipStream_t s);
void pack_conv_weights_1x1(const float* w, int cout, int cin, float* dst);
int launch_conv3x3_grad(const ConvLayer& L, const float* gin, float* gout, const float* dmask, int B, int H, int W,
                        hipStream_t s, const char* dmask_hs = nullptr, float mask_slope = 0.2f);
bool conv3x3_wino_ok(int C0, int C1, int cout, int H, int W);
bool conv3x3_wino_packs(int cout, int cin);
size_t conv3x3_wino_floats(int cout, int cin);
void pack_conv_weights_wino(const float* w, int cout, int cin, float* dst);
int launch_conv3x3_wino(const float* u, const float* bias, int cout, const float* in0, int C0, const float* in1, int C1,
                        float* out, int B, int H, int W, hipStream_t s, float slope = 0.2f, const float* res = nullptr,
                        float* pool_out = nullptr);
bool conv3x3_wino_outc_ok(int cin, int cout, int H, int W);
int launch_conv3x3_wino_outc(const float* u, const float* bias, const float* in0, int cin, const float* outc_w, const float* outc_b,
                             const float* x_img, float* img, float* img_pre, int B, int H, int W, hipStream_t s);
bool conv3x3_wino8_ok(int C0, int C1, int cout, int H, int W);
int launch_conv3x3_wino8(const float* u, const float* bias, int cout, const float* in0, int C0, const float* in1, int C1,
                         float* out, int B, int H, int W, hipStream_t s, float slope = 0.2f, const float* res = nullptr,
                         float* pool_out = nullptr, float* ks_part = nullptr, int ks_rule = 1);
int conv3x3_wino8_ksplit(int C0, int C1, int cout, int H, int W, int rule = 1);
size_t conv3x3_wino8_ksplit_bytes_per_image();
int launch_conv3x3_wino8_grad(const float* u, const float* zero_bias, int cout, const float* gin, int cin, float* gout, const float* dmask,
                              float mask_slope, int B, int H, int W, hipStream_t s);
bool conv3x3_wino8_ups_ok(int C0, int C1, int cout, int H, int W);
int launch_conv3x3_wino8_ups(const float* u, const float* bias, int cout, const float* in0, int C0, const float* in1_lowres, int C1,
                             float* out, int B, int H, int W, hipStream_t s, float slope = 0.2f);
int launch_conv3x3_wino8_outc(const float* u, const float* bias, const float* in0, int cin, const float* outc_w, const float* outc_b,
                              const float* x_img, float* img, float* img_pre, int B, int H, int W, hipStream_t s);
bool conv3x3_winof4_ok(int C0, int C1, int cout, int H, int W);
bool conv3x3_winof4_entry_ok(int C0, int C1, int cout, int H, int W);
bool conv3x3_winof4_packs(int cout, int cin);
size_t conv3x3_winof4_floats(int cout, int cin);
void pack_conv_weights_winof4(const float* w, int cout, int cin, float* dst);
int launch_conv3x3_winof4(const float* u, const float* bias, int cout, const float* in0, int C0, const float* in1, int C1, float* out, int B,
                          int H, int W, hipStream_t s, float slope = 0.2f, float* pool_out = nullptr);
bool conv3x3_winof4_c32_ok(int C0, int C1, int cout, int H, int W);
bool conv3x3_winof4_c32_packs(int cout, int cin);
void pack_conv_weights_winof4_c32(const float* w, int cout, int cin, float* dst);
int launch_conv3x3_winof4_c32(const float* u, const float* bias, int cout, const float* in0, int C0, float* out, int B, int H, int W,
                              hipStream_t s, float slope = 0.2f, float* pool_out = nullptr);
bool conv3x3_winof4_ups_ok(int C0, int C1, int cout, int H, int W);
int launch_conv3x3_winof4_ups(const float* u, const float* bias, int cout, const float* in0, int C0, const float* in1_lowres, int C1,
                              float* out, int B, int H, int W, hipStream_t s, float slope = 0.2f);
void launch_upsample2x_f32(const float* src, float* dst, size_t bc, int h, int w, int Ht, int Wt, hipStream_t s);
void pack_conv_weights_transposed(const float* w, int cout, int cin, int cout_pad, int mt, int cc, float* dst);
void transpose_flip_conv_weights(const float* w, int cout, int cin, int cout_pad, std::vector<float>& wt);

}
```

### tfpnp_amd/csrc/conv3x3_winof4.hip

```cpp
#include <cmath>
#include <mutex>
#include <utility>
#include <vector>

#include "common.h"
#include "conv3x3.h"
#include "wino_common.h"
#include "winof4_mats.h"

namespace pnpx {

namespace {

using namespace wino;

template <int CT_, int RW_, int NS>
struct GeoF4 {
  static constexpr int CT = CT_, RW = RW_, CK = 8;
  static constexpr int RWL = RW + 8;
  static constexpr int RPXL = 18 * RWL + 2;
  static constexpr int RAW_ELEMS = CK * RPXL;
  static constexpr int RAW_INSTR = (RAW_ELEMS + 63) / 64;
  static constexpr int RAW_BYTES = RAW_INSTR * 256;
  static constexpr int RAW_PER_WAVE = (RAW_INSTR + 7) / 8;
// ... 8 lines not shown
  static constexpr int NUW = USTG / 8192;
  static constexpr int SR = 11, SC = 20;
  static constexpr int QPLANE = SR * SC * 16;
  static constexpr int ST_INSTR = (2 * QPLANE + 255) / 256;
  static constexpr int ST_STRIDE = ST_INSTR * 256;
  static constexpr int ST_PER_WAVE = (ST_INSTR + 7) / 8;
  static constexpr int NST = ST_INSTR / 8;
  static constexpr int OFF_RAW_UPS = OFF_V + 2 * VSTG, OFF_ST = OFF_RAW_UPS + 2 * RAW_BYTES, OFF_TAB = OFF_ST + 2 * ST_STRIDE;
  static constexpr int LDS_USED_UPS = OFF_TAB + (18 + 34) * 16;
};
constexpr int LDS_REQF4 = 160 * 1024;
#ifndef WINOF4_ABL
#define WINOF4_ABL 0
#endif
static_assert(CfgF4::LDS_USED <= LDS_REQF4 && CfgF4::LDS_USED_UPS <= LDS_REQF4, "LDS budget");

template <int A>
__device__ __forceinline__ float bt_row(float d0, float d1, float d2, float d3, float d4, float d5) {
  if (A == 0) return fmaf(0.25f, d0, fmaf(-1.25f, d2, d4));
  if (A == 1) return fmaf(-0.25f, d2, d4) + fmaf(-0.25f, d1, d3);
  if (A == 2) return fmaf(-0.25f, d2, d4) - fmaf(-0.25f, d1, d3);
  if (A == 3) return fmaf(0.5f, d3 - d1, d4 - d2);
  if (A == 4) return fmaf(-0.5f, d3 - d1, d4 - d2);
  return fmaf(0.25f, d1, fmaf(-1.25f, d3, d5));
}
__device__ __forceinline__ void at_rows(float m0, float m1, float m2, float m3, float m4, float m5, float& o0, float& o1, float& o2, float& o3) {
  const float p12 = m1 + m2, m12 = m1 - m2, p34 = m3 + m4, m34 = m3 - m4;
  o0 = (m0 + p12) + p34;
  o1 = fmaf(0.5f, m34, m12);
  o2 = fmaf(0.25f, p34, p12);
  o3 = fmaf(0.125f, m34, m12) + m5;
}


struct Walk {
  int nregions, nx, xcd, slot, nslot;
};
__device__ __forceinline__ Walk make_walk(const WinoArgs& a) {
  Walk wk;
  wk.nregions = a.rx * a.ry * a.B;
  wk.nx = (gridDim.x % 8 == 0 && wk.nregions >= 32) ? 8 : 1;
  wk.xcd = blockIdx.x % wk.nx;
  wk.slot = blockIdx.x / wk.nx;
  wk.nslot = gridDim.x / wk.nx;
  return wk;
}
struct Tile {
  const float* s0;
  const float* w;
  int ct, b, x0, y0, ok;
};
template <class C>
__device__ __forceinline__ Tile decode_tile(const WinoArgs& a, const Walk& wk, int HpWp, int k) {
  Tile T;
  const int j = wk.slot + wk.nslot * k;
  const int q = j / a.nct;
  T.ct = j - q * a.nct;
  const int reg = wk.nx * q + wk.xcd;
  T.ok = reg < wk.nregions;
  const int t1 = reg / a.rx;
  const int tx = reg - t1 * a.rx;
  const int t2 = t1 / a.ry;
  const int ty = t1 - t2 * a.ry;
  T.b = t2;
  T.x0 = tx * C::RW;
  T.y0 = ty * 16;
  T.s0 = a.in0 + (size_t)T.b * a.C0 * HpWp + (size_t)T.y0 * a.Wp + T.x0 + (PADL - 1);
  T.w = a.u + (size_t)T.ct * a.nch * 3 * (C::USTG / 4);
  return T;
}

__device__ __forceinline__ void sync_all() {
  asm volatile("s_waitcnt vmcnt(0) lgkmcnt(0)" ::: "memory");
  __builtin_amdgcn_s_barrier();
}

template <class C>
struct HaloGather {
  unsigned roff[C::RAW_PER_WAVE];
  unsigned raw0;
  int wave;
  __device__ __forceinline__ HaloGather(const WinoArgs& a, int HpWp, unsigned raw0_, int wave_, int lane) : raw0(raw0_), wave(wave_) {
#pragma unroll
    for (int k = 0; k < C::RAW_PER_WAVE; ++k) {
      const int idx = (wave + 8 * k) * 64 + lane;
      const int c = idx / C::RPXL, r = idx - c * C::RPXL;
      const int hy = r / C::RWL, hx = r - hy * C::RWL;
      roff[k] = (c < C::CK && hy < 18 && hx < C::RW + 2) ? 4u * (unsigned)(c * HpWp + hy * a.Wp + hx) : 0u;
    }
  }
  __device__ __forceinline__ void piece(const float* src, int rbuf, int k) const {
    if (WINOF4_ABL & 2) return;
    if (k < C::NRAW || wave + 8 * k < C::RAW_INSTR) glds4(src, roff[k], raw0 + rbuf * C::RAW_BYTES + (wave + 8 * k) * 256);
  }
  __device__ __forceinline__ void all(const float* src, int rbuf) const {
#pragma unroll
    for (int k = 0; k < C::RAW_PER_WAVE; ++k) piece(src, rbuf, k);
  }
};

template <int A, int RWL, int VCP>
__device__ __forceinline__ void transform_tile(const char* rb, char* vb) {
  float d[6][6];
#pragma unroll
  for (int y = 0; y < 6; ++y) {
    const bool need = (A == 0) ? (y % 2 == 0) : (A == 5) ? (y % 2 == 1) : (y >= 1 && y <= 4);
#pragma unroll
    for (int x = 0; x < 6; x += 2) {
      if (need) {
        const f32x2 v = *reinterpret_cast<const f32x2*>(rb + (y * RWL + x) * 4);
        d[y][x] = v[0];
        d[y][x + 1] = v[1];
      } else {
        d[y][x] = d[y][x + 1] = 0.f;
      }
    }
  }
  float t[6];
#pragma unroll
  for (int x = 0; x < 6; ++x) t[x] = bt_row<A>(d[0][x], d[1][x], d[2][x], d[3][x], d[4][x], d[5][x]);
  *reinterpret_cast<f32x2*>(vb) = (f32x2){bt_row<0>(t[0], t[1], t[2], t[3], t[4], t[5]), bt_row<1>(t[0], t[1], t[2], t[3], t[4], t[5])};
  *reinterpret_cast<f32x2*>(vb + VCP) = (f32x2){bt_row<2>(t[0], t[1], t[2], t[3], t[4], t[5]), bt_row<3>(t[0], t[1], t[2], t[3], t[4], t[5])};
  *reinterpret_cast<f32x2*>(vb + 2 * VCP) = (f32x2){bt_row<4>(t[0], t[1], t[2], t[3], t[4], t[5]), bt_row<5>(t[0], t[1], t[2], t[3], t[4], t[5])};
}

template <int S, int UCP, int VCP, class Piece>
__device__ __forceinline__ void mfma_stage(f32x4 (&acc)[6][6], const char* ua, const char* vb, Piece&& piece) {
  f32x4 af[6], bf[6];
#pragma unroll
  for (int q = 0; q < 6; ++q) {
    af[q] = *reinterpret_cast<const f32x4*>(ua + q * UCP);
    bf[q] = *reinterpret_cast<const f32x4*>(vb + q * VCP);
  }
  static_for<6>([&](auto q_tag) {
    constexpr int Q = decltype(q_tag)::value, R = Q / 3, CP = Q % 3;
#pragma unroll
    for (int ks = 0; ks < 2; ++ks)
#pragma unroll
      for (int pos = 0; pos < 2; ++pos) {
        acc[2 * S + R][2 * CP + pos] = __builtin_amdgcn_mfma_f32_16x16x4f32(af[Q][2 * ks + pos], bf[Q][2 * ks + pos], acc[2 * S + R][2 * CP + pos], 0, 0, 0);
        piece(4 * Q + 2 * ks + pos);
        __builtin_amdgcn_sched_barrier(0);
      }
  });
}

__device__ __forceinline__ void clear_acc(f32x4 (&acc)[6][6]) {
#pragma unroll
  for (int i = 0; i < 6; ++i)
#pragma unroll
    for (int j = 0; j < 6; ++j) acc[i][j] = (f32x4){0.f, 0.f, 0.f, 0.f};
}

__device__ __forceinline__ void epilogue_tile(const WinoArgs& a, const f32x4 (&acc)[6][6], int HpWp, const Tile& T, int ty, int tx, int cbase) {
  float* ob = a.out + ((size_t)T.b * a.Cout + cbase) * HpWp + (size_t)(T.y0 + 4 * ty + 1) * a.Wp + T.x0 + 4 * tx + PADL;
  const int Hp_pool = padded_h(a.H / 2), Wp_pool = padded_w(a.W / 2);
  const size_t HpWp_pool = (size_t)Hp_pool * Wp_pool;
  float* pb = a.pool ? a.pool + ((size_t)T.b * a.Cout + cbase) * HpWp_pool + (size_t)(T.y0 / 2 + 2 * ty + 1) * Wp_pool + T.x0 / 2 + 2 * tx + PADL : nullptr;
  float bias4[4];
#pragma unroll
  for (int j = 0; j < 4; ++j) bias4[j] = a.bias[cbase + j];
  static_for<4>([&](auto j_tag) {
    constexpr int j = decltype(j_tag)::value;
    float s[4][6];
#pragma unroll
    for (int b = 0; b < 6; ++b) at_rows(acc[0][b][j], acc[1][b][j], acc[2][b][j], acc[3][b][j], acc[4][b][j], acc[5][b][j], s[0][b], s[1][b], s[2][b], s[3][b]);
    const float bias = bias4[j];
    float* o = ob + (size_t)j * HpWp;
    f32x4 y[4];
#pragma unroll
    for (int i = 0; i < 4; ++i) {
      float y0, y1, y2, y3;
      at_rows(s[i][0], s[i][1], s[i][2], s[i][3], s[i][4], s[i][5], y0, y1, y2, y3);
      y0 += bias;
      y1 += bias;
      y2 += bias;
      y3 += bias;
      y[i] = (f32x4){fmaxf(y0, y0 * a.slope), fmaxf(y1, y1 * a.slope), fmaxf(y2, y2 * a.slope), fmaxf(y3, y3 * a.slope)};
      if (!(WINOF4_ABL & 32) || a.slope == 123.f) *reinterpret_cast<f32x4*>(o + i * a.Wp) = y[i];
    }
    if (a.pool && (!(WINOF4_ABL & 32) || a.slope == 123.f)) {
      float* p = pb + (size_t)j * HpWp_pool;
      *reinterpret_cast<f32x2*>(p) = (f32x2){fmaxf(fmaxf(y[0][0], y[0][1]), fmaxf(y[1][0], y[1][1])), fmaxf(fmaxf(y[0][2], y[0][3]), fmaxf(y[1][2], y[1][3]))};
      *reinterpret_cast<f32x2*>(p + Wp_pool) = (f32x2){fmaxf(fmaxf(y[2][0], y[2][1]), fmaxf(y[3][0], y[3][1])), fmaxf(fmaxf(y[2][2], y[2][3]), fmaxf(y[3][2], y[3][3]))};
    }
  });
}

template <bool TWO, bool UPS = false>
__global__ __launch_bounds__(512, 1) void conv3x3_winof4_f32_kernel(WinoArgs a) {
  static_assert(TWO || !UPS, "the up-sampled source is the second one");
  using C = CfgF4;
  constexpr int CK = C::CK, RWL = C::RWL, RPXL = C::RPXL, RAW_BYTES = C::RAW_BYTES, RAW_PER_WAVE = C::RAW_PER_WAVE;
  constexpr int USTG = C::USTG, NUW = C::NUW, VSTG = C::VSTG, OFF_U = C::OFF_U, OFF_V = C::OFF_V, OFF_RAW = UPS ? C::OFF_RAW_UPS : C::OFF_RAW;
  constexpr int SC = C::SC, QPLANE = C::QPLANE, ST_STRIDE = C::ST_STRIDE, ST_PER_WAVE = C::ST_PER_WAVE, OFF_ST = C::OFF_ST, OFF_TAB = C::OFF_TAB;
  constexpr int UQ = USTG / 4;
  extern __shared__ __attribute__((aligned(16))) char lds[];
  const int tid = threadIdx.x, lane = tid & 63;
  const int wave = __builtin_amdgcn_readfirstlane(tid >> 6);
  const int sw = wave & 3;
  const int HpWp = a.Hp * a.Wp;
  const unsigned lds0 = (unsigned)(size_t)(lptr_t)lds;
  const Walk wk = make_walk(a);

  struct Tile2 : Tile {
    const float* s1;
    int rs, cs;
  };
  struct UpsStage {
    int vrd;
    int wait_n;
    bool raw, st, ip;
    const float* st_src;
    int st_buf, ip_sbuf, ip_rbuf;
  };
  const int h_lo = a.ups_h, w_lo = a.ups_w, hp_lo = padded_h(a.ups_h), wp_lo = padded_w(a.ups_w), hpwp_lo = hp_lo * wp_lo;
  auto decode = [&](int k) {
    Tile2 T;
    static_cast<Tile&>(T) = decode_tile<C>(a, wk, HpWp, k);
    if constexpr (UPS) {
      const int rl = (int)__fmul_rn(a.ups_sy, (float)max(T.y0 - 1, 0)) + 1, cl = (int)__fmul_rn(a.ups_sx, (float)max(T.x0 - 1, 0)) + PADL;
      T.rs = min(rl, max(hp_lo - C::SR, 0));
      T.cs = min(cl, wp_lo - SC);
      T.s1 = a.in1 + (size_t)T.b * a.C1 * hpwp_lo + (size_t)T.rs * wp_lo + T.cs;
    } else {
      T.rs = T.cs = 0;
      T.s1 = TWO ? a.in1 + (size_t)T.b * a.C1 * HpWp + (size_t)T.y0 * a.Wp + T.x0 + (PADL - 1) : nullptr;
    }
    return T;
  };
  const int nch0 = a.C0 / CK;
  auto raw_of = [&](const Tile2& X, int c) {
    if (TWO && !UPS && c >= nch0) return X.s1 + (size_t)CK * (c - nch0) * HpWp;
    return X.s0 + (size_t)CK * c * HpWp;
  };
  auto st_of = [&](const Tile2& X, int c) { return X.s1 + (size_t)CK * (c - nch0) * hpwp_lo; };

  const HaloGather<C> halo(a, HpWp, lds0 + OFF_RAW, wave, lane);
  const unsigned uoff = lane * 16u;
  auto dma_u_piece = [&](const float* src, int uslot, int k) {
    if (WINOF4_ABL & 4) return;
    glds16(src + wave * 256 + k * 2048, uoff, lds0 + OFF_U + uslot * USTG + (wave + 8 * k) * 1024);
  };
  auto dma_u = [&](const float* src, int uslot) {
#pragma unroll
    for (int k = 0; k < NUW; ++k) dma_u_piece(src, uslot, k);
  };

  unsigned stoff[UPS ? ST_PER_WAVE : 1];
  if constexpr (UPS) {
#pragma unroll
    for (int k = 0; k < ST_PER_WAVE; ++k) {
      const int idx = (wave + 8 * k) * 64 + lane;
      const int e = idx & 3, g = idx >> 2;
      const int sc = g % SC, g2 = g / SC;
      const int sr = g2 % C::SR, q = g2 / C::SR;
      stoff[k] = (q < CK / 4) ? 4u * (unsigned)((4 * q + e) * hpwp_lo + min(sr, hp_lo - 1) * wp_lo + sc) : 0u;
    }
  }
  auto dma_st_piece = [&](const float* src, int sbuf, int k) {
    if (WINOF4_ABL & 2) return;
    if (k < C::NST || wave + 8 * k < C::ST_INSTR) glds4(src, stoff[UPS ? k : 0], lds0 + OFF_ST + sbuf * ST_STRIDE + (wave + 8 * k) * 256);
  };
  auto write_tables = [&](const Tile2& X) {
    if (tid < 18 + 34) {
      const bool row = tid < 18;
      const int g = (row ? X.y0 : X.x0) - 1 + (row ? tid : tid - 18);
      const bool valid = g >= 0 && g < (row ? a.H : a.W);
      const float f = __fmul_rn(row ? a.ups_sy : a.ups_sx, (float)g);
      const int i0 = (int)f;
      const int i1 = i0 + (i0 < (row ? h_lo : w_lo) - 1 ? 1 : 0);
      const float l = __fsub_rn(f, (float)i0), h = __fsub_rn(1.f, l);
      f32x4 ent;
      ent[0] = __int_as_float(valid ? (row ? (i0 + 1 - X.rs) * SC * 16 : (i0 + PADL - X.cs) * 16) : 0);
      ent[1] = valid ? h : -1.f;
      ent[2] = valid ? l : 0.f;
      ent[3] = __int_as_float(valid ? (row ? (i1 + 1 - X.rs) * SC * 16 : (i1 + PADL - X.cs) * 16) : 0);
      *reinterpret_cast<f32x4*>(lds + OFF_TAB + tid * 16) = ent;
    }
  };
  auto blend = [](float hy, float ly, float hx, float lx, float v00, float v01, float v10, float v11) {
    return fmaf(hy, fmaf(hx, v00, __fmul_rn(lx, v01)), __fmul_rn(ly, fmaf(hx, v10, __fmul_rn(lx, v11))));
  };
  auto interp = [&](auto step_tag, int sbuf, int rbuf) {
    constexpr int STEP = decltype(step_tag)::value;
    if (WINOF4_ABL & 1) return;
    const int pix = STEP < 2 ? tid : min(512 + (tid >> 2), 18 * 34 - 1);
    const int hyi = pix / 34, hxi = pix - hyi * 34;
    const f32x4 rt = *reinterpret_cast<const f32x4*>(lds + OFF_TAB + hyi * 16);
    const f32x4 ct = *reinterpret_cast<const f32x4*>(lds + OFF_TAB + (18 + hxi) * 16);
    const bool inside = rt[1] >= 0.f && ct[1] >= 0.f;
    const int r0 = __float_as_int(rt[0]), r1 = __float_as_int(rt[3]), c0 = __float_as_int(ct[0]), c1 = __float_as_int(ct[3]);
    char* ob = lds + OFF_RAW + rbuf * RAW_BYTES + (hyi * RWL + hxi) * 4;
    if (STEP < 2) {
      const char* sb = lds + OFF_ST + sbuf * ST_STRIDE + STEP * QPLANE;
      const f32x4 v00 = *reinterpret_cast<const f32x4*>(sb + r0 + c0), v01 = *reinterpret_cast<const f32x4*>(sb + r0 + c1);
      const f32x4 v10 = *reinterpret_cast<const f32x4*>(sb + r1 + c0), v11 = *reinterpret_cast<const f32x4*>(sb + r1 + c1);
#pragma unroll
      for (int e = 0; e < 4; ++e)
        *reinterpret_cast<float*>(ob + (4 * STEP + e) * RPXL * 4) = inside ? blend(rt[1], rt[2], ct[1], ct[2], v00[e], v01[e], v10[e], v11[e]) : 0.f;
    } else {
      const int ch = 2 * (tid & 3);
      const char* sb = lds + OFF_ST + sbuf * ST_STRIDE + (ch >> 2) * QPLANE + (ch & 3) * 4;
      const f32x2 v00 = *reinterpret_cast<const f32x2*>(sb + r0 + c0), v01 = *reinterpret_cast<const f32x2*>(sb + r0 + c1);
      const f32x2 v10 = *reinterpret_cast<const f32x2*>(sb + r1 + c0), v11 = *reinterpret_cast<const f32x2*>(sb + r1 + c1);
#pragma unroll
      for (int e = 0; e < 2; ++e)
        *reinterpret_cast<float*>(ob + (ch + e) * RPXL * 4) = inside ? blend(rt[1], rt[2], ct[1], ct[2], v00[e], v01[e], v10[e], v11[e]) : 0.f;
    }
  };

  auto body = [&](auto role_tag) {
  constexpr int P = decltype(role_tag)::value;

  const int t_ks = lane & 1, t_t16 = (lane >> 1) & 15, t_kq = (lane >> 5) | ((sw & 1) << 1), t_wn = sw >> 1;
  const int t_tile = t_wn * 16 + t_t16;
  const int t_rd = ((2 * t_kq + t_ks) * RPXL + 4 * (t_tile >> 3) * RWL + 4 * (t_tile & 7)) * 4;
  const int t_wr = (P * 3 * 2 + t_wn) * 1024 + (t_kq * 16 + t_t16) * 16 + t_ks * 8;
  auto transform_row = [&](auto s_tag, int rbuf, int vslot_ups = 0) {
    constexpr int S = decltype(s_tag)::value;
    if (WINOF4_ABL & 1) return;
    transform_tile<2 * S + P, RWL, C::VCP>(lds + OFF_RAW + rbuf * RAW_BYTES + t_rd, lds + OFF_V + (UPS ? vslot_ups : S) * VSTG + t_wr);
  };

  const int mb = 2 * (sw & 1) + P, wn = sw >> 1;
  const int a_lane = mb * 1024 + lane * 16;
  const int b_lane = wn * 1024 + lane * 16;
  f32x4 acc[6][6];

  auto stage = [&](auto s_tag, auto wait_tag, const float* u_src, const float* raw_src, int raw_buf, int t_rbuf, const UpsStage& x) {
    constexpr int S = decltype(s_tag)::value, SN = (S + 1) % 3;
    constexpr int WAITN = decltype(wait_tag)::value;
    auto side = [&]() {
      transform_row(std::integral_constant<int, SN>{}, t_rbuf, x.vrd ^ 1);
      if constexpr (UPS) {
        if (x.ip) interp(std::integral_constant<int, SN>{}, x.ip_sbuf, x.ip_rbuf);
      }
    };
    auto piece = [&](int m) {
      if (m < NUW) dma_u_piece(u_src, (S + 2) % 3, m);
      if (S == 2 && m >= 4 && m < 4 + RAW_PER_WAVE && (!UPS || x.raw)) halo.piece(raw_src, raw_buf, m - 4);
      if constexpr (UPS) {
        if (S == 2 && m >= 16 && m < 16 + ST_PER_WAVE && x.st) dma_st_piece(x.st_src, x.st_buf, m - 16);
      }
    };
    auto mfmas = [&]() {
      if (WINOF4_ABL & 16) return;
      mfma_stage<S, C::UCP, C::VCP>(acc, lds + OFF_U + S * USTG + a_lane, lds + OFF_V + (UPS ? x.vrd : S) * VSTG + b_lane, piece);
    };
    if (P == 0) {
      mfmas();
      __builtin_amdgcn_sched_barrier(0);
      side();
    } else {
      side();
      __builtin_amdgcn_sched_barrier(0);
      mfmas();
    }
    if constexpr (UPS && S != 1) {
      if (x.wait_n == NUW + C::NRAW + C::NST) asm volatile("s_waitcnt vmcnt(%0) lgkmcnt(0)" ::"n"(NUW + C::NRAW + C::NST) : "memory");
      else if (x.wait_n == NUW + C::NRAW) asm volatile("s_waitcnt vmcnt(%0) lgkmcnt(0)" ::"n"(NUW + C::NRAW) : "memory");
      else if (x.wait_n == NUW + C::NST) asm volatile("s_waitcnt vmcnt(%0) lgkmcnt(0)" ::"n"(NUW + C::NST) : "memory");
      else asm volatile("s_waitcnt vmcnt(%0) lgkmcnt(0)" ::"n"(NUW) : "memory");
    } else {
      asm volatile("s_waitcnt vmcnt(%0) lgkmcnt(0)" ::"n"(WAITN) : "memory");
    }
    __builtin_amdgcn_s_barrier();
  };

  auto epilogue = [&](const Tile& T) {
    const int tile = wn * 16 + (lane & 15);
    epilogue_tile(a, acc, HpWp, T, tile >> 3, tile & 7, T.ct * 64 + mb * 16 + 4 * (lane >> 4));
  };

  using I0 = std::integral_constant<int, 0>;
  using I1 = std::integral_constant<int, 1>;
  using I2 = std::integral_constant<int, 2>;
  using WaitHalo = std::integral_constant<int, NUW + C::NRAW>;
  using WaitU = std::integral_constant<int, NUW>;

  int k = 0;
  Tile2 T = decode(0);
  if (!T.ok) return;
  halo.all(T.s0, 0);
  dma_u(T.w, 0);
  dma_u(T.w + UQ, 1);
  halo.all(raw_of(T, 1), 1);
  if constexpr (UPS) {
    if (nch0 == 2) {
#pragma unroll
      for (int q = 0; q < ST_PER_WAVE; ++q) dma_st_piece(st_of(T, 2), 0, q);
    }
  }
  sync_all();
  transform_row(I0{}, 0);
  sync_all();

  int cc = 0;
  int wait_prev = NUW;
  for (;;) {
    Tile2 Tn = decode(k + 1);
    const bool more = Tn.ok;
    if (!more) Tn = T;
    if constexpr (UPS) write_tables(T);
    clear_acc(acc);
    for (int c = 0; c < a.nch; ++c, ++cc) {
      const float* w_c = T.w + (size_t)c * 3 * UQ;
      const float* nu = (c + 1 < a.nch) ? w_c + 3 * UQ : Tn.w;
      const float* nraw = (c + 2 < a.nch) ? raw_of(T, c + 2) : raw_of(Tn, c + 2 - a.nch);
      const int rcur = cc & 1;
      if constexpr (UPS) {
        const bool up1 = c + 1 < a.nch && c + 1 >= nch0, up2 = c + 2 < a.nch && c + 2 >= nch0;
        const bool up3 = c + 3 < a.nch ? c + 3 >= nch0 : c + 3 - a.nch >= nch0;
        const float* nst = c + 3 < a.nch ? st_of(T, c + 3) : st_of(Tn, c + 3 - a.nch);
        const int wait_cur = NUW + (up2 ? 0 : C::NRAW) + (up3 ? C::NST : 0);
        UpsStage x{};
        x.ip = up1;
        x.ip_sbuf = x.ip_rbuf = rcur ^ 1;
        x.vrd = rcur;
        x.wait_n = wait_prev;
        stage(I0{}, WaitHalo{}, w_c + 2 * UQ, nullptr, 0, rcur, x);
        x.vrd = rcur ^ 1;
        stage(I1{}, WaitU{}, nu, nullptr, 0, rcur, x);
        x.vrd = rcur;
        x.ip = up2;
        x.ip_sbuf = x.ip_rbuf = rcur;
        x.raw = !up2;
        x.st = up3;
        x.st_src = nst;
        x.st_buf = rcur ^ 1;
        x.wait_n = wait_prev = wait_cur;
        stage(I2{}, WaitHalo{}, nu + UQ, nraw, rcur, rcur ^ 1, x);
        continue;
      }
      stage(I0{}, WaitHalo{}, w_c + 2 * UQ, nullptr, 0, rcur, UpsStage{});
      stage(I1{}, WaitU{}, nu, nullptr, 0, rcur, UpsStage{});
      stage(I2{}, WaitHalo{}, nu + UQ, nraw, rcur, rcur ^ 1, UpsStage{});
    }
    if (!(WINOF4_ABL & 8)) epilogue(T);
    if (!more) break;
    T = Tn;
    ++k;
  }
  sync_all();
  };
  if (wave < 4) body(std::integral_constant<int, 0>{});
  else body(std::integral_constant<int, 1>{});
}

using CfgF4C32 = GeoF4<32, 64, 2>;
static_assert(CfgF4C32::LDS_USED <= LDS_REQF4 && CfgF4C32::RAW_PER_WAVE + 3 <= 24 && CfgF4C32::USTG == 12 * 1024, "32-cout instance");

__global__ __launch_bounds__(512, 1) void conv3x3_winof4_c32_f32_kernel(WinoArgs a) {
  using C = CfgF4C32;
  constexpr int CK = C::CK, RWL = C::RWL, RPXL = C::RPXL, RAW_BYTES = C::RAW_BYTES, RAW_PER_WAVE = C::RAW_PER_WAVE;
  constexpr int USTG = C::USTG, VSTG = C::VSTG, OFF_U = C::OFF_U, OFF_V = C::OFF_V, OFF_RAW = C::OFF_RAW;
  constexpr int UQ = USTG / 4;
  extern __shared__ __attribute__((aligned(16))) char lds[];
  const int tid = threadIdx.x, lane = tid & 63;
  const int wave = __builtin_amdgcn_readfirstlane(tid >> 6);
  const int sw = wave & 3;
  const int HpWp = a.Hp * a.Wp;
  const unsigned lds0 = (unsigned)(size_t)(lptr_t)lds;
  const Walk wk = make_walk(a);
  auto decode = [&](int k) { return decode_tile<C>(a, wk, HpWp, k); };
  auto raw_of = [&](const Tile& X, int c) { return X.s0 + (size_t)CK * c * HpWp; };

  const HaloGather<C> halo(a, HpWp, lds0 + OFF_RAW, wave, lane);
  const unsigned uoff = lane * 16u;
  auto dma_u_piece = [&](const float* src, int uslot, int p) {
    if (WINOF4_ABL & 4) return;
    glds16(src + p * 256, uoff, lds0 + OFF_U + uslot * USTG + p * 1024);
  };

  auto body = [&](auto role_tag) {
  constexpr int P = decltype(role_tag)::value;

  const int t_ks = lane & 1, t_t16 = (lane >> 1) & 15, t_kq = (lane >> 5) | ((sw & 1) << 1), t_wn = sw >> 1;
  const int t_rd = ((2 * t_kq + t_ks) * RPXL + 4 * t_wn * RWL + 4 * t_t16) * 4;
  const int t_wr = (P * 3 * 4 + t_wn) * 1024 + (t_kq * 16 + t_t16) * 16 + t_ks * 8;
  auto transform_row = [&](auto s_tag, int rbuf, int vslot) {
    constexpr int S = decltype(s_tag)::value;
    if (WINOF4_ABL & 1) return;
    const char* rb = lds + OFF_RAW + rbuf * RAW_BYTES + t_rd;
    char* vb = lds + OFF_V + vslot * VSTG + t_wr;
    transform_tile<2 * S + P, RWL, C::VCP>(rb, vb);
    transform_tile<2 * S + P, RWL, C::VCP>(rb + 8 * RWL * 4, vb + 2048);
  };

  const int a_lane = P * 1024 + lane * 16;
  const int b_lane = sw * 1024 + lane * 16;
  f32x4 acc[6][6];

  auto stage = [&](auto s_tag, const float* u_src, const float* raw_src, int raw_buf, int t_rbuf, int vrd) {
    constexpr int S = decltype(s_tag)::value, SN = (S + 1) % 3;
    auto piece = [&](int m) {
      if (m == 0) dma_u_piece(u_src, vrd ^ 1, wave);
      if (m == 1 && P == 1) dma_u_piece(u_src, vrd ^ 1, 4 + wave);
      if (S == 2 && m >= 3 && m < 3 + RAW_PER_WAVE) halo.piece(raw_src, raw_buf, m - 3);
    };
    auto mfmas = [&]() {
      if (WINOF4_ABL & 16) {
#pragma unroll
        for (int m = 0; m < 24; ++m) piece(m);
        return;
      }
      mfma_stage<S, C::UCP, C::VCP>(acc, lds + OFF_U + vrd * USTG + a_lane, lds + OFF_V + vrd * VSTG + b_lane, piece);
    };
    if (P == 0) {
      mfmas();
      __builtin_amdgcn_sched_barrier(0);
      transform_row(std::integral_constant<int, SN>{}, t_rbuf, vrd ^ 1);
    } else {
      transform_row(std::integral_constant<int, SN>{}, t_rbuf, vrd ^ 1);
      __builtin_amdgcn_sched_barrier(0);
      mfmas();
    }
    if (S == 2 && !(WINOF4_ABL & 2)) asm volatile("s_waitcnt vmcnt(%0) lgkmcnt(0)" ::"n"(C::NRAW) : "memory");
    else asm volatile("s_waitcnt vmcnt(0) lgkmcnt(0)" ::: "memory");
    __builtin_amdgcn_s_barrier();
  };

  auto epilogue = [&](const Tile& T) { epilogue_tile(a, acc, HpWp, T, sw, lane & 15, T.ct * 32 + P * 16 + 4 * (lane >> 4)); };

  using I0 = std::integral_constant<int, 0>;
  using I1 = std::integral_constant<int, 1>;
  using I2 = std::integral_constant<int, 2>;

  int k = 0;
  Tile T = decode(0);
  if (!T.ok) return;
  halo.all(T.s0, 0);
  dma_u_piece(T.w, 0, wave);
  if (P == 1) dma_u_piece(T.w, 0, 4 + wave);
  halo.all(raw_of(T, 1), 1);
  sync_all();
  transform_row(I0{}, 0, 0);
  sync_all();

  int cc = 0;
  for (;;) {
    Tile Tn = decode(k + 1);
    const bool more = Tn.ok;
    if (!more) Tn = T;
    clear_acc(acc);
    for (int c = 0; c < a.nch; ++c, ++cc) {
      const float* w_c = T.w + (size_t)c * 3 * UQ;
      const float* nu = (c + 1 < a.nch) ? w_c + 3 * UQ : Tn.w;
      const float* nraw = (c + 2 < a.nch) ? raw_of(T, c + 2) : raw_of(Tn, c + 2 - a.nch);
      const int rcur = cc & 1;
      stage(I0{}, w_c + UQ, nullptr, 0, rcur, rcur);
      stage(I1{}, w_c + 2 * UQ, nullptr, 0, rcur, rcur ^ 1);
      stage(I2{}, nu, nraw, rcur, rcur ^ 1, rcur);
    }
    if (!(WINOF4_ABL & 8)) epilogue(T);
    if (!more) break;
    T = Tn;
    ++k;
  }
  sync_all();
  };
  if (wave < 4) body(std::integral_constant<int, 0>{});
  else body(std::integral_constant<int, 1>{});
}

}

bool conv3x3_winof4_ok(int C0, int C1, int cout, int H, int W) {
  return C1 == 0 && C0 >= 16 && C0 % 8 == 0 && cout > 0 && cout % 64 == 0 && H >= 16 && H % 16 == 0 && W >= 32 && W % 32 == 0;
}
bool conv3x3_winof4_entry_ok(int C0, int C1, int cout, int H, int W) {
  return conv3x3_winof4_ok(16, 0, cout, H, W) && H % 2 == 0 && W % 2 == 0 && C0 >= 8 && C0 % 8 == 0 && C1 >= 8 && C1 % 8 == 0;
}
bool conv3x3_winof4_ups_ok(int C0, int C1, int cout, int H, int W) { return conv3x3_winof4_entry_ok(C0, C1, cout, H, W) && C0 >= 16; }
bool conv3x3_winof4_packs(int cout, int cin) { return conv3x3_winof4_ok(cin, 0, cout, 16, 32); }
size_t conv3x3_winof4_floats(int cout, int cin) { return (size_t)36 * cout * cin; }

static void pack_winof4(const float* w, int cout, int cin, float* dst, int CT) {
  const int nch = cin / 8, nmb = CT / 16;
  for (int co = 0; co < cout; ++co)
    for (int ci = 0; ci < cin; ++ci) {
      const float* g = w + ((size_t)co * cin + ci) * 9;
      double gg[6][3], u[6][6];
      for (int i = 0; i < 6; ++i)
        for (int x = 0; x < 3; ++x) gg[i][x] = WINOF4_G[i][0] * g[0 * 3 + x] + WINOF4_G[i][1] * g[1 * 3 + x] + WINOF4_G[i][2] * g[2 * 3 + x];
      for (int i = 0; i < 6; ++i)
        for (int j = 0; j < 6; ++j) u[i][j] = gg[i][0] * WINOF4_G[j][0] + gg[i][1] * WINOF4_G[j][1] + gg[i][2] * WINOF4_G[j][2];
      const int ct = co / CT, mb = (co % CT) / 16, m = co % 16, ch = ci / 8, kq = (ci % 8) / 2, ks = ci % 2;
      for (int i = 0; i < 6; ++i)
        for (int j = 0; j < 6; ++j) {
          const size_t idx = (((((((((size_t)ct * nch + ch) * 3 + i / 2) * 2 + i % 2) * 3 + j / 2) * nmb + mb) * 4 + kq) * 16 + m) * 2 + ks) * 2 + j % 2;
          dst[idx] = (float)u[i][j];
        }
    }
}
void pack_conv_weights_winof4(const float* w, int cout, int cin, float* dst) { pack_winof4(w, cout, cin, dst, CfgF4::CT); }

bool conv3x3_winof4_c32_ok(int C0, int C1, int cout, int H, int W) {
  return C1 == 0 && C0 >= 16 && C0 % 8 == 0 && cout > 0 && cout % 32 == 0 && cout % 64 != 0 && H >= 16 && H % 16 == 0 && W >= 64 && W % 64 == 0;
}
bool conv3x3_winof4_c32_packs(int cout, int cin) { return conv3x3_winof4_c32_ok(cin, 0, cout, 16, 64); }
void pack_conv_weights_winof4_c32(const float* w, int cout, int cin, float* dst) { pack_winof4(w, cout, cin, dst, CfgF4C32::CT); }

enum class F4Inst { PLAIN, ENTRY, UPS, C32 };
static int launch_winof4(F4Inst inst, const float* u, const float* bias, int cout, const float* in0, int C0, const float* in1, int C1, float* out,
                         int B, int H, int W, hipStream_t s, float slope, float* pool_out) {
  const bool c32 = inst == F4Inst::C32, ups = inst == F4Inst::UPS;
  const bool ok = c32 ? conv3x3_winof4_c32_ok(C0, C1, cout, H, W)
                  : ups ? conv3x3_winof4_ups_ok(C0, C1, cout, H, W)
                        : inst == F4Inst::ENTRY ? conv3x3_winof4_entry_ok(C0, C1, cout, H, W) : conv3x3_winof4_ok(C0, C1, cout, H, W);
  if (!ok) {
    if (c32) set_error("conv3x3_winof4_c32: unsupported geometry (%d -> %d channels, %d x %d)", C0, cout, H, W);
    else set_error("conv3x3_winof4: unsupported geometry (%d + %d -> %d channels, %d x %d)", C0, C1, cout, H, W);
    return PNPX_ERR_SHAPE;
  }
  WinoArgs a{};
  a.in0 = in0;
  a.in1 = C1 != 0 ? in1 : in0;
  a.u = u;
  a.bias = bias;
  a.pool = pool_out;
  a.out = out;
  a.B = B;
  a.H = H;
  a.W = W;
  a.Hp = padded_h(H);
  a.Wp = padded_w(W);
  a.C0 = C0;
  a.C1 = C1;
  a.Cout = cout;
  a.slope = slope;
  a.nct = cout / (c32 ? CfgF4C32::CT : CfgF4::CT);
  a.nch = (C0 + C1) / CfgF4::CK;
  a.nch_all = a.nch;
  a.ksplit = 1;
  a.rx = W / (c32 ? CfgF4C32::RW : CfgF4::RW);
  a.ry = H / 16;
  if (ups) {
    a.ups_h = H / 2;
    a.ups_w = W / 2;
    a.ups_sy = (float)(H / 2 - 1) / (float)(H - 1);
    a.ups_sx = (float)(W / 2 - 1) / (float)(W - 1);
  }
  using Kernel = void (*)(WinoArgs);
  static const Kernel kernels[4] = {conv3x3_winof4_f32_kernel<false>, conv3x3_winof4_f32_kernel<true>, conv3x3_winof4_f32_kernel<true, true>,
                                    conv3x3_winof4_c32_f32_kernel};
  static std::once_flag attr_once[64];
  int dev = 0;
  PNPX_HIP(hipGetDevice(&dev));
  if (dev >= 0 && dev < 64) {
    hipError_t e = hipSuccess;
    std::call_once(attr_once[dev], [&] {
      for (int i = 0; i < 4 && e == hipSuccess; ++i)
        e = hipFuncSetAttribute(reinterpret_cast<const void*>(kernels[i]), hipFuncAttributeMaxDynamicSharedMemorySize, LDS_REQF4);
    });
    PNPX_HIP(e);
  }
  const long long nreg = (long long)a.rx * a.ry * a.B, ntiles = nreg * a.nct;
  long long grid = 256;
  if (grid >= ntiles) grid = ntiles;
  else if ((grid / 8) % a.nct != 0 && grid >= 8LL * a.nct) grid -= grid % (8 * a.nct);
  hipLaunchKernelGGL(kernels[(int)inst], dim3((unsigned)grid), dim3(512), LDS_REQF4, s, a);
  PNPX_LAUNCH_CHECK();
  return PNPX_OK;
}

int launch_conv3x3_winof4(const float* u, const float* bias, int cout, const float* in0, int C0, const float* in1, int C1, float* out, int B,
                          int H, int W, hipStream_t s, float slope, float* pool_out) {
  return launch_winof4(C1 != 0 ? F4Inst::ENTRY : F4Inst::PLAIN, u, bias, cout, in0, C0, in1, C1, out, B, H, W, s, slope, pool_out);
}
int launch_conv3x3_winof4_ups(const float* u, const float* bias, int cout, const float* in0, int C0, const float* in1_lowres, int C1,
                              float* out, int B, int H, int W, hipStream_t s, float slope) {
  return launch_winof4(F4Inst::UPS, u, bias, cout, in0, C0, in1_lowres, C1, out, B, H, W, s, slope, nullptr);
}
int launch_conv3x3_winof4_c32(const float* u, const float* bias, int cout, const float* in0, int C0, float* out, int B, int H, int W,
                              hipStream_t s, float slope, float* pool_out) {
  return launch_winof4(F4Inst::C32, u, bias, cout, in0, C0, nullptr, 0, out, B, H, W, s, slope, pool_out);
}

}

extern "C" void pnpx_winof4_matrices(double* g18, double* bt36, double* at24) {
  for (int i = 0; i < 6; ++i)
    for (int j = 0; j < 3; ++j) g18[i * 3 + j] = pnpx::WINOF4_G[i][j];
  for (int i = 0; i < 6; ++i)
    for (int j = 0; j < 6; ++j) bt36[i * 6 + j] = pnpx::WINOF4_BT[i][j];
  for (int i = 0; i < 4; ++i)
    for (int j = 0; j < 6; ++j) at24[i * 6 + j] = pnpx::WINOF4_AT[i][j];
}
extern "C" int pnpx_winof4_pack(const float* w, int cout, int cin, float* dst) {
  if (!w || !dst || cout <= 0 || cout % 64 != 0 || cin <= 0 || cin % 8 != 0) return PNPX_ERR_SHAPE;
  pnpx::pack_conv_weights_winof4(w, cout, cin, dst);
  return PNPX_OK;
}
extern "C" int pnpx_winof4_c32_pack(const float* w, int cout, int cin, float* dst) {
  if (!w || !dst || cout <= 0 || cout % 32 != 0 || cin <= 0 || cin % 8 != 0) return PNPX_ERR_SHAPE;
  pnpx::pack_conv_weights_winof4_c32(w, cout, cin, dst);
  return PNPX_OK;
}
```

### tfpnp_amd/csrc/conv_f32_select.h

```cpp
#pragma once
#include "conv3x3.h"

namespace pnpx {

enum class ConvF32Kernel { Direct, Wino4, Wino8, WinoF4, WinoF4C32 };

struct ConvF32Choice {
  ConvF32Kernel kernel = ConvF32Kernel::Direct;
  int pieces = 1;
  bool fused = false;
  bool wino() const { return kernel != ConvF32Kernel::Direct; }
};

struct ConvF32Sel {
  bool winograd = false;
  bool wino8 = false;
  bool winof4 = false;
  bool winof4_entry = false;
  bool winof4_fuse_up = false;
  bool winof4_c32 = false;
  int ksplit = 0;
  int ksplit_rule = 1;
  bool fuse_up = false;
  const float* u = nullptr;
  const float* u_f4 = nullptr;
  const float* u_f4c32 = nullptr;
  const float* u_bwd = nullptr;
};
ConvF32Sel conv_f32_sel(const pnpx_ctx* ctx, int li);
ConvF32Sel conv_f32_sel_drunet(const pnpx_ctx* ctx, const float* u, const float* u_bwd);

ConvF32Choice conv_f32_forward(const ConvF32Sel& v, int C0, int C1, int cout, int H, int W, int B_call);
ConvF32Choice conv_f32_entry(const ConvF32Sel& v, int C0, int C1, int cout, int H, int W, int B_call);
ConvF32Choice conv_f32_last(const ConvF32Sel& v, int cin, int cout, int H, int W, int B_call);
ConvF32Choice conv_f32_adjoint(const ConvF32Sel& v, int cin, int cout, int H, int W);
bool conv_f32_bottom_all8(const pnpx_ctx* ctx, int H, int W, int B_call, ConvF32Sel v[3], ConvF32Choice c[3]);

struct ConvF32Operands {
  const float* in0;
  int C0;
  const float* in1;
  int C1;
  float* out;
  int B, H, W;
  float slope = 0.2f;
  const float* res = nullptr;
  float* pool_out = nullptr;
  float* ks_part = nullptr;
  bool in1_lowres = false;
};
int launch_conv_f32(const ConvF32Choice& c, const ConvF32Sel& v, const ConvLayer& L, const ConvF32Operands& a, hipStream_t s);

}
```

### tfpnp_amd/csrc/conv_f32_select.hip

```cpp
#include "conv_f32_select.h"

namespace pnpx {

ConvF32Sel conv_f32_sel(const pnpx_ctx* ctx, int li) {
  ConvF32Sel v;
  v.winograd = ctx->opt_fp32_winograd != 0;
  v.wino8 = (ctx->opt_fp32_wino8 >> li) & 1;
  v.winof4 = (ctx->opt_fp32_winof4 >> li) & 1;
  v.winof4_entry = (ctx->opt_fp32_winof4_entries >> li) & 1;
  v.winof4_fuse_up = (ctx->opt_fp32_winof4_fuse_up >> li) & 1;
  v.winof4_c32 = (ctx->opt_fp32_winof4_c32 >> li) & 1;
  v.ksplit = ctx->opt_fp32_ksplit;
  v.ksplit_rule = ctx->opt_ksplit_rule;
  v.fuse_up = ctx->opt_fp32_fuse_up != 0;
  v.u = ctx->conv_wino_u[li];
  v.u_f4 = ctx->conv_winof4_u[li];
  v.u_f4c32 = ctx->conv_winof4_c32_u[li];
  v.u_bwd = ctx->conv_wino_u_bwd[li];
  return v;
}

ConvF32Sel conv_f32_sel_drunet(const pnpx_ctx* ctx, const float* u, const float* u_bwd) {
  ConvF32Sel v;
  v.winograd = ctx->opt_fp32_winograd != 0;
  v.wino8 = ctx->opt_fp32_wino8 != 0;
  v.u = u;
  v.u_bwd = u_bwd;
  return v;
}

static bool ksplit_on(const ConvF32Sel& v, int cout, int H, int W, int B_call) {
  if (v.ksplit == 2) return true;
  return v.ksplit == 1 && (long long)(H / 16) * (W / 16) * (cout / 64) * B_call < 256;
}

ConvF32Choice conv_f32_forward(const ConvF32Sel& v, int C0, int C1, int cout, int H, int W, int B_call) {
  ConvF32Choice c;
  if (!v.winograd || !v.u || !conv3x3_wino_ok(C0, C1, cout, H, W)) return c;
  c.fused = true;
  c.kernel = ConvF32Kernel::Wino4;
  if (!v.wino8 || !conv3x3_wino8_ok(C0, C1, cout, H, W)) return c;
  c.kernel = ConvF32Kernel::Wino8;
  if (ksplit_on(v, cout, H, W, B_call)) c.pieces = conv3x3_wino8_ksplit(C0, C1, cout, H, W, v.ksplit_rule);
  if (c.pieces == 1 && v.winof4 && v.u_f4 && C1 == 0 && conv3x3_winof4_ok(C0, 0, cout, H, W)) c.kernel = ConvF32Kernel::WinoF4;
  else if (c.pieces == 1 && v.winof4_c32 && v.u_f4c32 && C1 == 0 && conv3x3_winof4_c32_ok(C0, 0, cout, H, W)) c.kernel = ConvF32Kernel::WinoF4C32;
  return c;
}

ConvF32Choice conv_f32_entry(const ConvF32Sel& v, int C0, int C1, int cout, int H, int W, int B_call) {
  ConvF32Choice c = conv_f32_forward(v, C0, C1, cout, H, W, B_call);
  if (c.kernel == ConvF32Kernel::Wino8 && c.pieces == 1 && v.winof4_entry && v.u_f4 && conv3x3_winof4_entry_ok(C0, C1, cout, H, W)) {
    c.kernel = ConvF32Kernel::WinoF4;
    c.fused = v.winof4_fuse_up && conv3x3_winof4_ups_ok(C0, C1, cout, H, W);
    return c;
  }
  c.fused = c.kernel == ConvF32Kernel::Wino8 && c.pieces == 1 && v.fuse_up && conv3x3_wino8_ups_ok(C0, C1, cout, H, W);
  return c;
}

ConvF32Choice conv_f32_last(const ConvF32Sel& v, int cin, int cout, int H, int W, int B_call) {
  ConvF32Choice c = conv_f32_forward(v, cin, 0, cout, H, W, B_call);
  c.fused = false;
  if (v.winograd && v.u && conv3x3_wino_outc_ok(cin, cout, H, W)) {
    c.fused = true;
    c.kernel = v.wino8 && conv3x3_wino8_ok(cin, 0, cout, H, W) ? ConvF32Kernel::Wino8 : ConvF32Kernel::Wino4;
  }
  return c;
}

ConvF32Choice conv_f32_adjoint(const ConvF32Sel& v, int cin, int cout, int H, int W) {
  ConvF32Choice c;
  if (v.winograd && v.wino8 && v.u_bwd && conv3x3_wino8_ok(cin, 0, cout, H, W)) c.kernel = ConvF32Kernel::Wino8;
  return c;
}

bool conv_f32_bottom_all8(const pnpx_ctx* ctx, int H, int W, int B_call, ConvF32Sel v[3], ConvF32Choice c[3]) {
  bool all8 = true;
  for (int k = 0; k < 3; ++k) {
    const ConvLayer& L = ctx->conv[12 + k];
    v[k] = conv_f32_sel(ctx, 12 + k);
    v[k].u_f4 = nullptr;
    c[k] = conv_f32_forward(v[k], L.cin, 0, L.cout, H, W, B_call);
    all8 = all8 && c[k].kernel == ConvF32Kernel::Wino8;
  }
  return all8;
}

int launch_conv_f32(const ConvF32Choice& c, const ConvF32Sel& v, const ConvLayer& L, const ConvF32Operands& a, hipStream_t s) {
  switch (c.kernel) {
    case ConvF32Kernel::WinoF4:
      if (a.in1_lowres) return launch_conv3x3_winof4_ups(v.u_f4, L.b, L.cout, a.in0, a.C0, a.in1, a.C1, a.out, a.B, a.H, a.W, s, a.slope);
      return launch_conv3x3_winof4(v.u_f4, L.b, L.cout, a.in0, a.C0, a.in1, a.C1, a.out, a.B, a.H, a.W, s, a.slope, a.pool_out);
    case ConvF32Kernel::WinoF4C32:
      return launch_conv3x3_winof4_c32(v.u_f4c32, L.b, L.cout, a.in0, a.C0, a.out, a.B, a.H, a.W, s, a.slope, a.pool_out);
    case ConvF32Kernel::Wino8:
      return launch_conv3x3_wino8(v.u, L.b, L.cout, a.in0, a.C0, a.in1, a.C1, a.out, a.B, a.H, a.W, s, a.slope, a.res, a.pool_out,
                                  c.pieces > 1 ? a.ks_part : nullptr, v.ksplit_rule);
    case ConvF32Kernel::Wino4:
      return launch_conv3x3_wino(v.u, L.b, L.cout, a.in0, a.C0, a.in1, a.C1, a.out, a.B, a.H, a.W, s, a.slope, a.res, a.pool_out);
    case ConvF32Kernel::Direct:
      break;
  }
  return launch_conv3x3_act(L, a.in0, a.C0, a.in1, a.C1, a.out, a.B, a.H, a.W, a.slope, a.res, s);
}

}

extern "C" int pnpx_conv_f32_entry_plan(int opts, int ksplit, int ksplit_rule, int C0, int C1, int cout, int H, int W, int B_call) {
  static const float packed = 0.f;
  pnpx::ConvF32Sel v;
  v.winograd = opts & 1;
  v.wino8 = opts & 2;
  v.winof4 = opts & 4;
  v.winof4_entry = opts & 8;
  v.fuse_up = opts & 16;
  v.u = (opts & 32) ? &packed : nullptr;
  v.u_f4 = (opts & 64) ? &packed : nullptr;
  v.winof4_fuse_up = opts & 128;
  v.ksplit = ksplit;
  v.ksplit_rule = ksplit_rule;
  if (C0 <= 0 || C1 <= 0 || cout <= 0 || H <= 0 || W <= 0 || B_call <= 0) return -1;
  const pnpx::ConvF32Choice c = pnpx::conv_f32_entry(v, C0, C1, cout, H, W, B_call);
  return static_cast<int>(c.kernel) + 16 * c.pieces + 256 * (c.fused ? 1 : 0);
}

extern "C" int pnpx_conv_f32_forward_plan(int opts, int ksplit, int ksplit_rule, int C0, int C1, int cout, int H, int W, int B_call) {
  static const float packed = 0.f;
  pnpx::ConvF32Sel v;
  v.winograd = opts & 1;
  v.wino8 = opts & 2;
  v.winof4 = opts & 4;
  v.winof4_c32 = opts & 8;
  v.u = (opts & 16) ? &packed : nullptr;
  v.u_f4 = (opts & 32) ? &packed : nullptr;
  v.u_f4c32 = (opts & 64) ? &packed : nullptr;
  v.ksplit = ksplit;
  v.ksplit_rule = ksplit_rule;
  if (C0 <= 0 || C1 < 0 || cout <= 0 || H <= 0 || W <= 0 || B_call <= 0 || ((opts & 128) && C1 != 0)) return -1;
  const pnpx::ConvF32Choice c = (opts & 128) ? pnpx::conv_f32_last(v, C0, cout, H, W, B_call) : pnpx::conv_f32_forward(v, C0, C1, cout, H, W, B_call);
  return static_cast<int>(c.kernel) + 16 * c.pieces + 256 * (c.fused ? 1 : 0);
}
```

### tfpnp_amd/csrc/conv_probe.hip

```cpp
#include "common.h"
#include "conv3x3.h"

using namespace pnpx;

namespace {

bool is_grad(int kind) { return kind == PNPX_PROBE_DIRECT_GRAD || kind == PNPX_PROBE_WINO8_GRAD; }

int direct_ct(int C0, int C1, int cout) {
  if (C0 <= 0 || C1 < 0 || cout <= 0) return 0;
  const int mt = conv_pack_mt(cout), cc = conv_pack_cc(C0 + C1);
  if (C0 % cc != 0 || C1 % cc != 0 || cout % mt != 0 || (mt == 64 && cc != 8)) return 0;
  return mt;
}
int direct_grad_ct(int C0, int cout) {
  if (C0 <= 0 || C0 % 8 != 0 || cout <= 0 || cout % 32 != 0) return 0;
  return cout % 64 == 0 ? 64 : 32;
}

}

extern "C" int pnpx_conv3x3_probe_plan(int kind, int C0, int C1, int cout, int H, int W, int ks_rule) {
  if (C0 <= 0 || C1 < 0 || cout <= 0 || H <= 0 || W <= 0) return 0;
  const int wct = cout % 64 == 0 ? 64 : 32;
  switch (kind) {
    case PNPX_PROBE_DIRECT: return direct_ct(C0, C1, cout);
    case PNPX_PROBE_WINO4: return conv3x3_wino_ok(C0, C1, cout, H, W) ? wct : 0;
    case PNPX_PROBE_WINO8: return conv3x3_wino8_ok(C0, C1, cout, H, W) ? wct : 0;
    case PNPX_PROBE_WINO8_KSPLIT:
      return conv3x3_wino8_ok(C0, C1, cout, H, W) ? wct + 256 * conv3x3_wino8_ksplit(C0, C1, cout, H, W, ks_rule) : 0;
    case PNPX_PROBE_WINOF4: return conv3x3_winof4_ok(C0, C1, cout, H, W) ? 64 : 0;
    case PNPX_PROBE_WINO8_UPS: return conv3x3_wino8_ups_ok(C0, C1, cout, H, W) ? wct : 0;
    case PNPX_PROBE_DIRECT_GRAD: return C1 == 0 ? direct_grad_ct(C0, cout) : 0;
    case PNPX_PROBE_WINO8_GRAD: return C1 == 0 && conv3x3_wino8_ok(C0, 0, cout, H, W) ? wct : 0;
    case PNPX_PROBE_WINOF4_2SRC: return C1 > 0 && conv3x3_winof4_entry_ok(C0, C1, cout, H, W) ? 64 : 0;
    case PNPX_PROBE_WINOF4_UPS: return 0;
    case PNPX_PROBE_WINOF4_FUSE_UP: return C1 > 0 && conv3x3_winof4_ups_ok(C0, C1, cout, H, W) ? 64 : 0;
    case PNPX_PROBE_WINOF4_C32: return conv3x3_winof4_c32_ok(C0, C1, cout, H, W) ? 32 : 0;
  }
  return 0;
}

extern "C" int pnpx_conv3x3_probe(pnpx_ctx* ctx, int kind, const float* w_host, const float* bias_host, int cout, const float* in0, int C0,
                                  const float* in1, int C1, float* out, const float* res, const float* mask, float slope, float* pool_out,
                                  int ks_rule, int B, int H, int W, void* stream) {
  if (!ctx) {
    set_error("null context");
    return PNPX_ERR_ARG;
  }
  std::lock_guard<std::mutex> lk(ctx->mu);
  PNPX_HIP(hipSetDevice(ctx->device));
  hipStream_t s = static_cast<hipStream_t>(stream);
  const bool grad = is_grad(kind);
  if (kind < PNPX_PROBE_DIRECT || (kind > PNPX_PROBE_WINOF4_UPS && kind != PNPX_PROBE_WINOF4_FUSE_UP && kind != PNPX_PROBE_WINOF4_C32)) {
    set_error("pnpx_conv3x3_probe: unknown kind %d", kind);
    return PNPX_ERR_ARG;
  }
  if (!w_host || (!grad && !bias_host) || !in0 || !out || B <= 0 || H <= 0 || W <= 0 || cout <= 0 || C0 <= 0 || C1 < 0 || (C1 > 0 && !in1)) {
    set_error("pnpx_conv3x3_probe: null pointer or non-positive size");
    return PNPX_ERR_ARG;
  }
  const bool takes_res = kind == PNPX_PROBE_DIRECT || kind == PNPX_PROBE_WINO4 || kind == PNPX_PROBE_WINO8;
  const bool takes_pool = kind == PNPX_PROBE_WINO4 || kind == PNPX_PROBE_WINO8 || kind == PNPX_PROBE_WINOF4 || kind == PNPX_PROBE_WINOF4_2SRC ||
                          kind == PNPX_PROBE_WINOF4_C32;
  if ((res && !takes_res) || (pool_out && !takes_pool) || (mask && !grad) || (res && pool_out)) {
    set_error("pnpx_conv3x3_probe: kind %d takes no %s operand", kind, res && !takes_res ? "res" : (mask && !grad ? "mask" : "pool_out"));
    return PNPX_ERR_ARG;
  }
  if ((grad || kind == PNPX_PROBE_WINOF4 || kind == PNPX_PROBE_WINOF4_C32) && C1 != 0) {
    set_error("pnpx_conv3x3_probe: kind %d is single-source (C1 = %d)", kind, C1);
    return PNPX_ERR_SHAPE;
  }
  if (kind == PNPX_PROBE_WINOF4_UPS || ((kind == PNPX_PROBE_WINOF4_2SRC || kind == PNPX_PROBE_WINOF4_FUSE_UP) && C1 == 0)) {
    set_error(kind == PNPX_PROBE_WINOF4_UPS ? "pnpx_conv3x3_probe: unsupported geometry (kind %d has no instance)"
                                            : "pnpx_conv3x3_probe: unsupported geometry (kind %d needs a second source)", kind);
    return PNPX_ERR_SHAPE;
  }
  const int cin = C0 + C1;
  const int plan = pnpx_conv3x3_probe_plan(kind, C0, C1, cout, H, W, ks_rule);

  auto launch = [&](const float* pk, const float* b, float* ks) -> int {
    ConvLayer L;
    L.cin = grad ? C0 : cin;
    L.cout = cout;
    L.w = const_cast<float*>(pk);
    L.b = const_cast<float*>(b);
    switch (kind) {
      case PNPX_PROBE_DIRECT:
        L.mt = conv_pack_mt(cout);
        L.cc = conv_pack_cc(cin);
        return launch_conv3x3_act(L, in0, C0, in1, C1, out, B, H, W, slope, res, s);
      case PNPX_PROBE_WINO4: return launch_conv3x3_wino(pk, b, cout, in0, C0, in1, C1, out, B, H, W, s, slope, res, pool_out);
      case PNPX_PROBE_WINO8: return launch_conv3x3_wino8(pk, b, cout, in0, C0, in1, C1, out, B, H, W, s, slope, res, pool_out, nullptr, ks_rule);
      case PNPX_PROBE_WINO8_KSPLIT: return launch_conv3x3_wino8(pk, b, cout, in0, C0, in1, C1, out, B, H, W, s, slope, nullptr, nullptr, ks, ks_rule);
      case PNPX_PROBE_WINOF4: return launch_conv3x3_winof4(pk, b, cout, in0, C0, nullptr, 0, out, B, H, W, s, slope, pool_out);
      case PNPX_PROBE_WINOF4_2SRC: return launch_conv3x3_winof4(pk, b, cout, in0, C0, in1, C1, out, B, H, W, s, slope, pool_out);
      case PNPX_PROBE_WINO8_UPS: return launch_conv3x3_wino8_ups(pk, b, cout, in0, C0, in1, C1, out, B, H, W, s, slope);
      case PNPX_PROBE_WINOF4_FUSE_UP: return launch_conv3x3_winof4_ups(pk, b, cout, in0, C0, in1, C1, out, B, H, W, s, slope);
      case PNPX_PROBE_WINOF4_C32: return launch_conv3x3_winof4_c32(pk, b, cout, in0, C0, out, B, H, W, s, slope, pool_out);
      case PNPX_PROBE_DIRECT_GRAD:
        L.mt = cout % 64 == 0 ? 64 : 32;
        L.cc = 8;
        return launch_conv3x3_grad(L, in0, out, mask, B, H, W, s, nullptr, slope);
      case PNPX_PROBE_WINO8_GRAD: return launch_conv3x3_wino8_grad(pk, b, cout, in0, C0, out, mask, slope, B, H, W, s);
    }
    return PNPX_ERR_ARG;
  };
  if (!plan) {
    const int rc = launch(nullptr, nullptr, nullptr);
    if (rc == PNPX_OK) {
      set_error("pnpx_conv3x3_probe: the plan refuses a geometry kind %d's launcher accepts (%d + %d -> %d channels, %d x %d)", kind, C0, C1, cout, H, W);
      return PNPX_ERR_SHAPE;
    }
    return rc;
  }

  std::vector<float> host, wt;
  switch (kind) {
    case PNPX_PROBE_DIRECT:
      host.resize((size_t)cout * cin * 9);
      pack_conv_weights(w_host, cout, cin, conv_pack_mt(cout), conv_pack_cc(cin), host.data());
      break;
    case PNPX_PROBE_WINOF4:
    case PNPX_PROBE_WINOF4_2SRC:
    case PNPX_PROBE_WINOF4_FUSE_UP:
      host.resize(conv3x3_winof4_floats(cout, cin));
      pack_conv_weights_winof4(w_host, cout, cin, host.data());
      break;
    case PNPX_PROBE_WINOF4_C32:
      host.resize(conv3x3_winof4_floats(cout, cin));
      pack_conv_weights_winof4_c32(w_host, cout, cin, host.data());
      break;
    case PNPX_PROBE_DIRECT_GRAD:
      host.resize((size_t)cout * C0 * 9);
      pack_conv_weights_transposed(w_host, C0, cout, cout, cout % 64 == 0 ? 64 : 32, 8, host.data());
      break;
    case PNPX_PROBE_WINO8_GRAD:
      transpose_flip_conv_weights(w_host, C0, cout, cout, wt);
      host.resize(conv3x3_wino_floats(cout, C0));
      pack_conv_weights_wino(wt.data(), cout, C0, host.data());
      break;
    default:
      host.resize(conv3x3_wino_floats(cout, cin));
      pack_conv_weights_wino(w_host, cout, cin, host.data());
  }
  host.resize((host.size() + 255) & ~(size_t)255, 0.f);
  const size_t boff = host.size();
  if (grad) host.resize(boff + cout, 0.f);
  else host.insert(host.end(), bias_host, bias_host + cout);
  host.resize(host.size() + 1024, 0.f);

  DeviceBuf wbuf, ksbuf;
  auto release = [&]() {
    if (wbuf.p) (void)hipFree(wbuf.p);
    if (ksbuf.p) (void)hipFree(ksbuf.p);
  };
  int rc = alloc_dev(wbuf, host.size() * sizeof(float), "probe weight");
  if (rc == PNPX_OK && kind == PNPX_PROBE_WINO8_KSPLIT) rc = alloc_dev(ksbuf, conv3x3_wino8_ksplit_bytes_per_image() * (size_t)B, "probe K-split scratch");
  if (rc == PNPX_OK) {
    const hipError_t e = hipMemcpy(wbuf.p, host.data(), host.size() * sizeof(float), hipMemcpyHostToDevice);
    if (e != hipSuccess) rc = hip_fail(e, "hipMemcpy(probe weights)", __FILE__, __LINE__);
  }
  if (rc == PNPX_OK) rc = launch(static_cast<float*>(wbuf.p), static_cast<float*>(wbuf.p) + boff, static_cast<float*>(ksbuf.p));
  const hipError_t e = hipStreamSynchronize(s);
  release();
  if (rc == PNPX_OK && e != hipSuccess) rc = hip_fail(e, "hipStreamSynchronize(probe)", __FILE__, __LINE__);
  return rc;
}

extern "C" int pnpx_upsample2x_probe(pnpx_ctx* ctx, const float* src, float* dst, int planes, int h, int w, void* stream) {
  if (!ctx || !src || !dst || planes <= 0 || h <= 0 || w <= 0) {
    set_error("pnpx_upsample2x_probe: null pointer or non-positive size");
    return PNPX_ERR_ARG;
  }
  std::lock_guard<std::mutex> lk(ctx->mu);
  PNPX_HIP(hipSetDevice(ctx->device));
  launch_upsample2x_f32(src, dst, (size_t)planes, h, w, 2 * h, 2 * w, static_cast<hipStream_t>(stream));
  PNPX_LAUNCH_CHECK();
  return PNPX_OK;
}
```

### tfpnp_amd/csrc/unet.hip

```cpp
#include <cstdlib>

#include "common.h"
#include "conv_f32_select.h"
#include "conv_hs.h"
#include "conv_first.h"
#include "hs_rec.h"
#include "unet_plan.h"

namespace pnpx {

__global__ void prep_input_kernel(const float* __restrict__ x, const float* __restrict__ sigma, int sigma_stride,
                                  float* __restrict__ dst, int H, int W, int Hp, int Wp) {
  const int b = blockIdx.z;
  const int y = blockIdx.y;
  const int xx = blockIdx.x * blockDim.x + threadIdx.x;
  if (xx >= W) return;
  const float v = x[((size_t)b * H + y) * W + xx];
  float* d = dst + (size_t)b * 2 * Hp * Wp + (size_t)(y + 1) * Wp + xx + PADL;
  d[0] = v;
  d[(size_t)Hp * Wp] = sigma[(size_t)b * sigma_stride];
}

__global__ __launch_bounds__(256) void maxpool2_kernel(const float* __restrict__ src, float* __restrict__ dst,
                                                       size_t n_out, int H, int W) {
  const int Ho = H / 2, Wo = W / 2;
  const int Hp = padded_h(H), Wp = padded_w(W), Hpo = padded_h(Ho), Wpo = padded_w(Wo);
  const size_t i = (size_t)blockIdx.x * blockDim.x + threadIdx.x;
  if (i >= n_out) return;
  const int xo = (int)(i % Wo);
  const size_t t = i / Wo;
  const int yo = (int)(t % Ho);
  const size_t bc = t / Ho;
  const float* s = src + bc * Hp * Wp + (size_t)(2 * yo + 1) * Wp + 2 * xo + PADL;
  const float2 r0 = *reinterpret_cast<const float2*>(s);
  const float2 r1 = *reinterpret_cast<const float2*>(s + Wp);
  dst[bc * Hpo * Wpo + (size_t)(yo + 1) * Wpo + xo + PADL] = fmaxf(fmaxf(r0.x, r0.y), fmaxf(r1.x, r1.y));
}

__global__ __launch_bounds__(256) void upsample2x_kernel(const float* __restrict__ src, float* __restrict__ dst,
                                                         size_t n_out, int h, int w, int Ht, int Wt, float sy, float sx) {
  const int H = 2 * h, W = 2 * w;
  const int hp = padded_h(h), wp = padded_w(w), Hp = padded_h(Ht), Wp = padded_w(Wt);
  const size_t i = (size_t)blockIdx.x * blockDim.x + threadIdx.x;
  if (i >= n_out) return;
  const int x = (int)(i % W);
  const size_t t = i / W;
  const int y = (int)(t % H);
  const size_t bc = t / H;
  const float fy = sy * y, fx = sx * x;
  const int y0 = (int)fy, x0 = (int)fx;
  const int y1 = y0 + (y0 < h - 1 ? 1 : 0), x1 = x0 + (x0 < w - 1 ? 1 : 0);
  const float ly = fy - y0, lx = fx - x0;
  const float hy = 1.f - ly, hx = 1.f - lx;
  const float* s = src + bc * hp * wp + PADL;
  const float v00 = s[(size_t)(y0 + 1) * wp + x0], v01 = s[(size_t)(y0 + 1) * wp + x1];
  const float v10 = s[(size_t)(y1 + 1) * wp + x0], v11 = s[(size_t)(y1 + 1) * wp + x1];
  dst[bc * Hp * Wp + (size_t)(y + 1) * Wp + x + PADL] = hy * (hx * v00 + lx * v01) + ly * (hx * v10 + lx * v11);
}

constexpr int UPS_ROWS = 4;
__global__ __launch_bounds__(256) void upsample2x_v4_kernel(const float* __restrict__ src, float* __restrict__ dst, int h, int w,
                                                            int Ht, int Wt, float sy, float sx) {
  const int W = 2 * w;
  const int hp = padded_h(h), wp = padded_w(w), Hp = padded_h(Ht), Wp = padded_w(Wt);
  const int xq = blockIdx.x * blockDim.x + threadIdx.x;
  const int yb = (blockIdx.y * blockDim.y + threadIdx.y) * UPS_ROWS;
  if (4 * xq >= W || yb >= 2 * h) return;
  const size_t bc = blockIdx.z;
  const int xs = (int)(sx * (4 * xq));
  int i0[4], i1[4], xi[4];
  float lx[4], hx[4];
#pragma unroll
  for (int j = 0; j < 4; ++j) {
    const int x = 4 * xq + j;
    const float fx = sx * x;
    const int x0 = (int)fx;
    const int x1 = x0 + (x0 < w - 1 ? 1 : 0);
    lx[j] = fx - x0;
    hx[j] = 1.f - lx[j];
    i0[j] = x0 - xs;
    i1[j] = x1 - xs;
    xi[j] = xs + j < w ? xs + j : w - 1;
  }
  auto pick = [](const float* v, int i) { return i == 0 ? v[0] : i == 1 ? v[1] : i == 2 ? v[2] : v[3]; };
  const float* sb = src + bc * hp * wp + PADL;
  float* db = dst + bc * Hp * Wp + 4 * xq + PADL;
#pragma unroll
  for (int r = 0; r < UPS_ROWS; ++r) {
    const int y = yb + r;
    if (y >= 2 * h) break;
    const float fy = sy * y;
    const int y0 = (int)fy;
    const int y1 = y0 + (y0 < h - 1 ? 1 : 0);
    const float ly = fy - y0, hy = 1.f - ly;
    const float* s0 = sb + (size_t)(y0 + 1) * wp;
    const float* s1 = sb + (size_t)(y1 + 1) * wp;
    float a0[4], a1[4], o[4];
#pragma unroll
    for (int j = 0; j < 4; ++j) {
      a0[j] = s0[xi[j]];
      a1[j] = s1[xi[j]];
    }
#pragma unroll
    for (int j = 0; j < 4; ++j)
      o[j] = hy * (hx[j] * pick(a0, i0[j]) + lx[j] * pick(a0, i1[j])) + ly * (hx[j] * pick(a1, i0[j]) + lx[j] * pick(a1, i1[j]));
    *reinterpret_cast<float4*>(db + (size_t)(y + 1) * Wp) = make_float4(o[0], o[1], o[2], o[3]);
  }
}

__global__ void outc_residual_kernel(const float* __restrict__ feat, const float* __restrict__ x,
                                     const float* __restrict__ w, const float* __restrict__ bias,
                                     float* __restrict__ out, float* __restrict__ out_pre, int H, int W) {
  const int Hp = padded_h(H), Wp = padded_w(W);
  const int xx = blockIdx.x * blockDim.x + threadIdx.x;
  const int y = blockIdx.y;
  const int b = blockIdx.z;
  if (xx >= W) return;
  const float* f = feat + (size_t)b * 32 * Hp * Wp + (size_t)(y + 1) * Wp + xx + PADL;
  float acc = 0.f;
#pragma unroll
  for (int c = 0; c < 32; ++c) acc = fmaf(w[c], f[(size_t)c * Hp * Wp], acc);
  const size_t o = ((size_t)b * H + y) * W + xx;
  const float v = x[o] + (acc + bias[0]);
  if (out_pre) out_pre[o] = v;
  out[o] = fminf(fmaxf(v, 0.f), 1.f);
}

__global__ __launch_bounds__(256) void prep_input_hs_kernel(const float* __restrict__ x, const float* __restrict__ sigma,
                                                            int sigma_stride, HsRec* __restrict__ dst, int H, int W,
                                                            size_t n) {
  const size_t i = (size_t)blockIdx.x * blockDim.x + threadIdx.x;
  if (i >= n) return;
  const int xx = (int)(i % W);
  const size_t t = i / W;
  const int y = (int)(t % H);
  const size_t b = t / H;
  float v[8] = {x[i] * HS_ASCALE, sigma[b * sigma_stride] * HS_ASCALE, 0.f, 0.f, 0.f, 0.f, 0.f, 0.f};
  dst[(b * 2 * (H + 2) + (y + 1)) * (W + 2) + xx + 1] = hs_pack(v);
}

__global__ __launch_bounds__(256) void maxpool2_hs_kernel(const HsRec* __restrict__ src, HsRec* __restrict__ dst,
                                                          size_t n_out, int H, int W) {
  const int Ho = H / 2, Wo = W / 2;
  const size_t i = (size_t)blockIdx.x * blockDim.x + threadIdx.x;
  if (i >= n_out) return;
  const int xo = (int)(i % Wo);
  const size_t t = i / Wo;
  const int yo = (int)(t % Ho);
  const size_t bg = t / Ho;
  const HsRec* s = src + (bg * (H + 2) + (2 * yo + 1)) * (W + 2) + 2 * xo + 1;
  float a[8], c[8], d[8], e[8], o[8];
  hs_unpack(s[0], a);
  hs_unpack(s[1], c);
  hs_unpack(s[W + 2], d);
  hs_unpack(s[W + 3], e);
#pragma unroll
  for (int k = 0; k < 8; ++k) o[k] = fmaxf(fmaxf(a[k], c[k]), fmaxf(d[k], e[k]));
  dst[(bg * (Ho + 2) + (yo + 1)) * (Wo + 2) + xo + 1] = hs_pack(o);
}

template <int TX, int R>
__global__ __launch_bounds__(256) void upsample2x_hs_kernel(const HsRec* __restrict__ src, HsRec* __restrict__ dst, int h,
                                                            int w, int Ht, int Wt, float sy, float sx) {
  constexpr int TYP = 256 / TX, TY = TYP * R;
  constexpr int SW = TX / 2 + 2, SH = TY / 2 + 2;
  constexpr int NREC = SH * SW;
  __shared__ uint4 tile[NREC * 2];
  const int H = 2 * h, W = 2 * w;
  const int X0 = blockIdx.x * TX, Y0 = blockIdx.y * TY;
  const size_t bg = blockIdx.z;
  const int c_lo = (int)(sx * X0), r_lo = (int)(sy * Y0);
  const uint4* s = reinterpret_cast<const uint4*>(src + bg * (size_t)(h + 2) * (w + 2) + 1);
  for (int k = threadIdx.x; k < NREC * 2; k += 256) {
    const int rec = k >> 1, piece = k & 1;
    const int rr = rec / SW, cc = rec - rr * SW;
    const int yy = min(r_lo + rr, h - 1), xx = min(c_lo + cc, w - 1);
    tile[piece * NREC + rec] = s[((size_t)(yy + 1) * (w + 2) + xx) * 2 + piece];
  }
  __syncthreads();
  const int tx = threadIdx.x % TX, ty0 = threadIdx.x / TX;
  const int x = X0 + tx;
  if (x >= W) return;
  const float fx = sx * x;
  const int x0 = (int)fx;
  const int x1 = x0 + (x0 < w - 1 ? 1 : 0);
  const float lx = fx - x0;
  const float hx = 1.f - lx;
  auto unpack = [&](int idx, float v[8]) {
    HsRec r;
    r.hi = *reinterpret_cast<const h8v*>(&tile[idx]);
    r.lo = *reinterpret_cast<const h8v*>(&tile[NREC + idx]);
    hs_unpack(r, v);
  };
#pragma unroll
  for (int r = 0; r < R; ++r) {
    const int y = Y0 + ty0 + r * TYP;
    if (y >= H) return;
    const float fy = sy * y;
    const int y0 = (int)fy;
    const int y1 = y0 + (y0 < h - 1 ? 1 : 0);
    const float ly = fy - y0;
    const float hy = 1.f - ly;
    float v00[8], v01[8], v10[8], v11[8], o[8];
    unpack((y0 - r_lo) * SW + (x0 - c_lo), v00);
    unpack((y0 - r_lo) * SW + (x1 - c_lo), v01);
    unpack((y1 - r_lo) * SW + (x0 - c_lo), v10);
    unpack((y1 - r_lo) * SW + (x1 - c_lo), v11);
#pragma unroll
    for (int k = 0; k < 8; ++k) o[k] = hy * (hx * v00[k] + lx * v01[k]) + ly * (hx * v10[k] + lx * v11[k]);
    const HsRec ro = hs_pack(o);
    uint4* dp = reinterpret_cast<uint4*>(dst + (bg * (Ht + 2) + (y + 1)) * (Wt + 2) + x + 1);
    dp[0] = __builtin_bit_cast(uint4, ro.hi);
    dp[1] = __builtin_bit_cast(uint4, ro.lo);
  }
}

__global__ __launch_bounds__(256) void outc_residual_hs_kernel(const HsRec* __restrict__ feat, const float* __restrict__ x,
                                                               const float* __restrict__ w, const float* __restrict__ bias,
                                                               float* __restrict__ out, float* __restrict__ out_pre, int H,
                                                               int W, size_t n) {
  const size_t i = (size_t)blockIdx.x * blockDim.x + threadIdx.x;
  if (i >= n) return;
  const int xx = (int)(i % W);
  const size_t t = i / W;
  const int y = (int)(t % H);
  const size_t b = t / H;
  const size_t plane = (size_t)(H + 2) * (W + 2);
  const HsRec* f = feat + b * 4 * plane + (size_t)(y + 1) * (W + 2) + xx + 1;
  float acc = 0.f;
#pragma unroll
  for (int g = 0; g < 4; ++g) {
    float v[8];
    hs_unpack(f[g * plane], v);
#pragma unroll
    for (int k = 0; k < 8; ++k) acc = fmaf(w[g * 8 + k], v[k], acc);
  }
  const float r = x[i] + (acc * (1.f / HS_ASCALE) + bias[0]);
  if (out_pre) out_pre[i] = r;
  out[i] = fminf(fmaxf(r, 0.f), 1.f);
}

int reserve_arena(pnpx_ctx* ctx, UNetArena& ar, int mode, int B, int H, int W, size_t extra_bytes) {
  if (B <= ar.capB && H == ar.capH && W == ar.capW && mode == ar.mode) return PNPX_OK;
  const bool same_geom = (H == ar.capH && W == ar.capW);
  const int nb = same_geom ? (B > ar.capB ? B : ar.capB) : B;
  UNetPlan P = make_plan(mode, nb, H, W);
  const size_t total = P.total + extra_bytes * (size_t)nb;
  PNPX_HIP(hipSetDevice(ctx->device));
  PNPX_HIP(hipDeviceSynchronize());
  if (ar.buf.bytes < total) {
    if (ar.buf.p) PNPX_HIP(hipFree(ar.buf.p));
    ar = UNetArena();
    void* p = nullptr;
    hipError_t e = hipMalloc(&p, total);
    if (e != hipSuccess) {
      set_error("arena allocation of %zu bytes failed: %s", total, hipGetErrorString(e));
      return PNPX_ERR_ALLOC;
    }
    ar.buf.p = p;
    ar.buf.bytes = total;
  }
  PNPX_HIP(hipMemset(ar.buf.p, 0, total));
  PNPX_HIP(hipDeviceSynchronize());
  ar.capB = nb;
  ar.capH = H;
  ar.capW = W;
  ar.mode = mode;
  return PNPX_OK;
}

size_t unet_arena_bytes(int mode, int B, int H, int W) { return make_plan(mode, B, H, W).total; }

void train_cache_free(pnpx_ctx* ctx) {
  (void)hipDeviceSynchronize();
// ... 222 lines not shown
  const Act* below = &P.x[4];
  for (int l = 3; l >= 0; --l) {
    const int h = below->H, w = below->W;
    const float sy = (2 * h > 1) ? (float)(h - 1) / (float)(2 * h - 1) : 0.f;
    const float sx = (2 * w > 1) ? (float)(w - 1) / (float)(2 * w - 1) : 0.f;
    const int sb = sub_of(l);
    for (int b0 = 0; b0 < B; b0 += sb) {
      const int nb = (B - b0 < sb) ? (B - b0) : sb;
      ConvHsFuse f;
      ConvHsFuse f_first;
      bool ups_fused = false;
      if (ctx->opt_fuse_up >= (l == 0 ? 1 : 2)) {
        const ConvLayerHsDev& D0 = ctx->conv_hs[15 + 3 * (3 - l)];
        ConvLayerHs L0;
        L0.cout = D0.cout;
        L0.mt = D0.mt;
        ups_fused = P.u[l].H == 2 * h && P.u[l].W == 2 * w && P.x[l].H == 2 * h && P.x[l].W == 2 * w &&
                    conv_hs_can_fuse_upsample(L0, P.x[l].C / 8, below->C / 8, 2 * h, 2 * w);
      }
      if (ups_fused) {
        f_first.ups_h = h;
        f_first.ups_w = w;
      } else {
        const unsigned nbg = (unsigned)(nb * (below->C / 8));
        const int Wo = 2 * w, Ho = 2 * h;
        if (Wo > 32) {
          hipLaunchKernelGGL((upsample2x_hs_kernel<64, 4>), dim3((Wo + 63) / 64, (Ho + 15) / 16, nbg), dim3(256), 0, s,
                             rat(*below, b0), rat(P.u[l], b0), h, w, P.u[l].H, P.u[l].W, sy, sx);
        } else {
          hipLaunchKernelGGL((upsample2x_hs_kernel<32, 2>), dim3((Wo + 31) / 32, (Ho + 15) / 16, nbg), dim3(256), 0, s,
                             rat(*below, b0), rat(P.u[l], b0), h, w, P.u[l].H, P.u[l].W, sy, sx);
        }
        PNPX_LAUNCH_CHECK();
        PNPX_TRY(rec.mark("upsample2x", 0));
      }
      if (l == 0 && !no_outc_fuse) {
        f.outc_w = ctx->outc_w;
        f.outc_b = ctx->outc_b;
        f.x_in = x + (size_t)b0 * H * W;
        f.out_img = out + (size_t)b0 * H * W;
        f.out_pre = out_pre ? out_pre + (size_t)b0 * H * W : nullptr;
      }
      PNPX_TRY(block(15 + 3 * (3 - l), P.x[l], ups_fused ? below : &P.u[l], l, P.y[l], b0, nb, f, f_first));
    }
    below = &P.y[l];
  }
  if (no_outc_fuse) {
    hipLaunchKernelGGL(outc_residual_hs_kernel, g1d(npix), dim3(256), 0, s, rat(P.y[0], 0), x, ctx->outc_w, ctx->outc_b,
                       out, out_pre, H, W, npix);
    PNPX_LAUNCH_CHECK();
    PNPX_TRY(rec.mark("outc_residual_clamp", 2.0 * 32 * (double)H * W * B));
  }
  return PNPX_OK;
}

static int unet_forward_f32(pnpx_ctx* ctx, UNetArena& ar, const UNetPlan& P, const float* x, const float* sigma, int sigma_stride, float* out,
                            float* out_pre, int B, int H, int W, hipStream_t s, Recorder& rec, bool keep_all, bool level_chains, int b_base = 0, int B_call = 0) {
  if (B_call <= 0) B_call = B;
  char* A = static_cast<char*>(ar.buf.p);
  auto fptr = [&](const Act& d) { return reinterpret_cast<float*>(A + d.off + (size_t)b_base * act_bytes_per_image(CONV_F32, d.C, d.H, d.W)); };
  float* const ks_part0 = reinterpret_cast<float*>(A + P.ks_part + (size_t)b_base * P.ks_part_per_image);
  const bool first_valu = ctx->opt_fuse_first && W % 4 == 0 && ctx->conv[0].cout == 32;
  if (!first_valu) {
    hipLaunchKernelGGL(prep_input_kernel, dim3((W + 63) / 64, H, B), dim3(64), 0, s, x, sigma, sigma_stride, fptr(P.in0), H,
                       W, padded_h(H), padded_w(W));
    PNPX_LAUNCH_CHECK();
    PNPX_TRY(rec.mark("prep_input", 0));
  }
  auto conv = [&](int li, const Act& i0, const Act* i1, const Act& o, const Act* pooled = nullptr, bool* pooled_done = nullptr) -> int {
    const ConvLayer& L = ctx->conv[li];
    const int C1 = i1 ? i1->C : 0;
    const ConvF32Sel v = conv_f32_sel(ctx, li);
    const ConvF32Choice c = conv_f32_forward(v, i0.C, C1, L.cout, o.H, o.W, B_call);
    ConvF32Operands a{fptr(i0), i0.C, i1 ? fptr(*i1) : nullptr, C1, fptr(o), B, o.H, o.W};
    a.pool_out = pooled ? fptr(*pooled) : nullptr;
    a.ks_part = ks_part0;
    PNPX_TRY(launch_conv_f32(c, v, L, a, s));
    if (pooled_done) *pooled_done = pooled && c.fused;
    return rec.mark(c.wino() ? "conv3x3_wino" : "conv3x3", 2.0 * 9.0 * L.cin * L.cout * (double)o.H * o.W * B);
  };
  auto block = [&](int li, const Act& i0, const Act* i1, int lvl, const Act& o, const Act* pooled = nullptr, bool* pooled_done = nullptr) -> int {
    const Act& ta = i1 ? P.da[lvl] : P.a[lvl];
    const Act& tb = i1 ? P.db[lvl] : P.b[lvl];
    if (li == 0 && first_valu) {
      hipLaunchKernelGGL(conv_first_f32_kernel, dim3((H * (W / 4) + 255) / 256, 4, B), dim3(256), 0, s, x, sigma, sigma_stride, ctx->conv0_w,
                         ctx->conv[0].b, fptr(ta), H, W, 0.2f);
      PNPX_LAUNCH_CHECK();
      PNPX_TRY(rec.mark("conv3x3", 2.0 * 9.0 * 2 * 32 * (double)H * W * B));
    } else
    PNPX_TRY(conv(li, i0, i1, ta));
    PNPX_TRY(conv(li + 1, ta, nullptr, tb));
    return conv(li + 2, tb, nullptr, o, pooled, pooled_done);
  };
  bool pooled = false;
  PNPX_TRY(block(0, P.in0, nullptr, 0, P.x[0], &P.p[1], &pooled));
  for (int l = 1; l < 5; ++l) {
    const Act& src = P.x[l - 1];
    if (!pooled) {
      const size_t n_pool = (size_t)B * src.C * (src.H / 2) * (src.W / 2);
      hipLaunchKernelGGL(maxpool2_kernel, g1d(n_pool), dim3(256), 0, s, fptr(src), fptr(P.p[l]), n_pool, src.H, src.W);
      PNPX_LAUNCH_CHECK();
      PNPX_TRY(rec.mark("maxpool2", 0));
    }
    if (l == 4 && level_chains && B >= 2) {
      const Act& o4 = P.x[4];
      ConvF32Sel v4[3];
      ConvF32Choice c4[3];
      const bool all8 = conv_f32_bottom_all8(ctx, o4.H, o4.W, B_call, v4, c4);
      const long long ntiles = (long long)(o4.H / 16) * (o4.W / 16) * B * (ctx->conv[13].cout / 64);
      if (all8 && ntiles > 256 && ntiles < 768 && ntiles % 256 != 0) {
        PNPX_TRY(fan_out_chains(ctx, 2, B, s, [&](int lo, int hi, hipStream_t st) -> int {
          auto slice = [&](int li, const Act& i, const Act& o) -> int {
            ConvF32Operands a{fptr(i) + (size_t)lo * i.C * padded_h(i.H) * padded_w(i.W), i.C, nullptr, 0,
                              fptr(o) + (size_t)lo * o.C * padded_h(o.H) * padded_w(o.W), hi - lo, o.H, o.W};
            a.ks_part = ks_part0 + (size_t)lo * (P.ks_part_per_image / sizeof(float));
            return launch_conv_f32(c4[li - 12], v4[li - 12], ctx->conv[li], a, st);
          };
          PNPX_TRY(slice(12, P.p[4], P.a[4]));
          PNPX_TRY(slice(13, P.a[4], P.b[4]));
          return slice(14, P.b[4], P.x[4]);
        }));
        pooled = false;
        continue;
      }
    }
    PNPX_TRY(block(3 * l, P.p[l], nullptr, l, P.x[l], l < 4 ? &P.p[l + 1] : nullptr, &pooled));
  }
  const ConvF32Choice c26 = conv_f32_last(conv_f32_sel(ctx, 26), ctx->conv[26].cin, ctx->conv[26].cout, H, W, B_call);
  const Act* below = &P.x[4];
  for (int l = 3; l >= 0; --l) {
    const int h = below->H, w = below->W;
    const int li0 = 15 + 3 * (3 - l);
    const ConvF32Sel v0 = conv_f32_sel(ctx, li0);
    const bool even = P.x[l].H == 2 * h && P.x[l].W == 2 * w;
    const ConvF32Choice c0 = even ? conv_f32_entry(v0, P.x[l].C, below->C, ctx->conv[li0].cout, 2 * h, 2 * w, B_call) : ConvF32Choice();
    const bool ups_fused = c0.fused;
    if (!ups_fused) {
      launch_upsample2x_f32(fptr(*below), fptr(P.u[l]), (size_t)B * below->C, h, w, P.u[l].H, P.u[l].W, s);
      PNPX_LAUNCH_CHECK();
      PNPX_TRY(rec.mark("upsample2x", 0));
    }
    auto entry = [&](const Act& ta) -> int {
      const ConvLayer& L = ctx->conv[li0];
      if (c0.kernel == ConvF32Kernel::WinoF4) {
        ConvF32Operands a{fptr(P.x[l]), P.x[l].C, ups_fused ? fptr(*below) : fptr(P.u[l]), P.u[l].C, fptr(ta), B, ta.H, ta.W};
        a.in1_lowres = ups_fused;
        PNPX_TRY(launch_conv_f32(c0, v0, L, a, s));
        return rec.mark("conv3x3_wino", 2.0 * 9.0 * L.cin * L.cout * (double)ta.H * ta.W * B);
      }
      if (!ups_fused) return conv(li0, P.x[l], &P.u[l], ta);
      PNPX_TRY(launch_conv3x3_wino8_ups(ctx->conv_wino_u[li0], L.b, L.cout, fptr(P.x[l]), P.x[l].C, fptr(*below), below->C, fptr(ta), B, 2 * h, 2 * w, s));
      return rec.mark("conv3x3_wino", 2.0 * 9.0 * L.cin * L.cout * (double)(2 * h) * (2 * w) * B);
    };
    if (l == 0 && !keep_all && ctx->opt_fuse_outc && c26.fused) {
      PNPX_TRY(entry(P.da[0]));
      PNPX_TRY(conv(25, P.da[0], nullptr, P.db[0]));
      PNPX_TRY((c26.kernel == ConvF32Kernel::Wino8 ? launch_conv3x3_wino8_outc : launch_conv3x3_wino_outc)(
          ctx->conv_wino_u[26], ctx->conv[26].b, fptr(P.db[0]), ctx->conv[26].cin, ctx->outc_w, ctx->outc_b, x, out, out_pre, B, H, W, s));
      return rec.mark("conv3x3_wino", 2.0 * 9.0 * ctx->conv[26].cin * ctx->conv[26].cout * (double)H * W * B);
    }
    PNPX_TRY(entry(P.da[l]));
    PNPX_TRY(conv(li0 + 1, P.da[l], nullptr, P.db[l]));
    PNPX_TRY(conv(li0 + 2, P.db[l], nullptr, P.y[l]));
    below = &P.y[l];
  }
  hipLaunchKernelGGL(outc_residual_kernel, dim3((W + 63) / 64, H, B), dim3(64), 0, s, fptr(P.y[0]), x, ctx->outc_w,
                     ctx->outc_b, out, out_pre, H, W);
  PNPX_LAUNCH_CHECK();
  PNPX_TRY(rec.mark("outc_residual_clamp", 2.0 * 32 * (double)H * W * B));
  return PNPX_OK;
}

int launch_chains(const pnpx_ctx* ctx, int B, int H, int W) {
  int n = ctx->opt_chains;
  if (n == 0) {
    const long long q = (long long)B * H * W / (256 * 256);
    n = (q >= 5 && q != 8) ? 2 : 1;
  }
  if (n > 8) n = 8;
  return n > B ? B : (n < 1 ? 1 : n);
}

void join_side_streams_after_failure(pnpx_ctx* ctx) {
  for (hipStream_t st : ctx->side_streams) (void)hipStreamSynchronize(st);
}
int chain_streams(pnpx_ctx* ctx, int chains) {
  if (chains > 16) {
    set_error("launch chains: at most 16 slices");
    return PNPX_ERR_ARG;
  }
  while ((int)ctx->side_streams.size() < chains - 1) {
    hipStream_t st = nullptr;
    PNPX_HIP(hipStreamCreateWithFlags(&st, hipStreamNonBlocking));
    ctx->side_streams.push_back(st);
  }
  return PNPX_OK;
}
int chain_event(pnpx_ctx* ctx, hipEvent_t* ev) {
  constexpr size_t POOL = 256;
  if (ctx->ev_pool.size() < POOL) {
    hipEvent_t e = nullptr;
    PNPX_HIP(hipEventCreateWithFlags(&e, hipEventDisableTiming));
    ctx->ev_pool.push_back(e);
    *ev = e;
    return PNPX_OK;
  }
  *ev = ctx->ev_pool[ctx->ev_next++ % POOL];
  return PNPX_OK;
}

int unet_denoise(pnpx_ctx* ctx, const float* x, const float* sigma, int sigma_stride, float* out, float* out_pre,
                 int B, int H, int W, hipStream_t s, ProfileSink* prof, UNetArena* arena, int mode, bool keep_all) {
  if (ctx->drunet.loaded) {
    if (arena || keep_all || prof) {
      set_error("the DRUNet denoiser keeps its activations in its own arena (drunet_denoise_backward re-computes them) and has no per-launch profile");
      return PNPX_ERR_ARG;
    }
    return drunet_denoise(ctx, x, sigma, sigma_stride, out, out_pre, B, H, W, s);
  }
  if (!ctx->has_weights) {
    set_error("denoiser called before pnpx_unet_load");
    return PNPX_ERR_NO_WEIGHTS;
  }
  if (B <= 0 || H < 16 || W < 16) {
    set_error("denoiser: need B > 0 and H, W >= 16 (four 2x2 poolings; got B=%d H=%d W=%d)", B, H, W);
    return PNPX_ERR_SHAPE;
  }
  UNetArena& ar = arena ? *arena : ctx->arena;
  if (mode < 0) mode = ctx->conv_mode;
  PNPX_TRY(reserve_arena(ctx, ar, mode, B, H, W, 0));
  const bool hs = (mode == CONV_HS);
  const UNetPlan P = make_plan(mode, ar.capB, H, W);
  Recorder rec{prof, s};
  if (prof) PNPX_HIP(hipEventRecord((*prof->events)[0], s));
  const int chains = hs && !prof ? launch_chains(ctx, B, H, W) : 1;
  if (chains > 1) {
    const size_t px = (size_t)H * W;
    return fan_out_chains(ctx, chains, B, s, [&](int lo, int hi, hipStream_t st) -> int {
      Recorder none{nullptr, st};
      return unet_forward_hs(ctx, ar, P, x + lo * px, sigma + (size_t)lo * sigma_stride, sigma_stride, out + lo * px,
                             out_pre ? out_pre + lo * px : nullptr, hi - lo, H, W, st, none, keep_all, lo, chains);
    });
  }
  if (hs) return unet_forward_hs(ctx, ar, P, x, sigma, sigma_stride, out, out_pre, B, H, W, s, rec, keep_all);

  if (!prof && ctx->opt_fp32_chains >= 2 && B >= ctx->opt_fp32_chains) {
    const size_t px = (size_t)H * W;
    return fan_out_chains(ctx, ctx->opt_fp32_chains, B, s, [&](int lo, int hi, hipStream_t st) -> int {
      Recorder none{nullptr, st};
      return unet_forward_f32(ctx, ar, P, x + lo * px, sigma + (size_t)lo * sigma_stride, sigma_stride, out + lo * px,
                              out_pre ? out_pre + lo * px : nullptr, hi - lo, H, W, st, none, keep_all, false, lo, B);
    });
  }
  return unet_forward_f32(ctx, ar, P, x, sigma, sigma_stride, out, out_pre, B, H, W, s, rec, keep_all, !prof && ctx->opt_fp32_chains == 1);
}

}
```

Before: 141.3 iters/s.

## Fuse output 1x1 conv and residual clamp into 32-cout Winograd F4 kernel

Adds an OUTC variant of the 32-output-channel Winograd F(4x4) kernel that folds the final 1x1 output conv, residual add and clamp into its epilogue. Partial sums are combined across lanes with shuffles and across the two channel halves through an LDS exchange, so the last feature map need not be written and read back. The fused path is gated by a new option that defaults to off. The default C32 layer mask also gains layer 2, which changes kernel selection for that layer on the default path. A keep-all variant and a Wino8-order residual kernel are added so summation order matches training.

```diff
diff --git a/include/pnpx.h b/include/pnpx.h
--- a/include/pnpx.h
+++ b/include/pnpx.h
@@ -35,6 +35,8 @@
 int pnpx_unet_load(pnpx_ctx* ctx, const float* params_host, size_t n_params);
 int pnpx_unet_denoise(pnpx_ctx* ctx, const float* x, const float* sigma, float* out, float* out_preclamp,
                       int B, int H, int W, void* stream);
+int pnpx_unet_denoise_keep(pnpx_ctx* ctx, const float* x, const float* sigma, float* out, float* out_preclamp,
+                           int B, int H, int W, void* stream);
 size_t pnpx_drunet_num_params(int nb);
 int pnpx_drunet_load(pnpx_ctx* ctx, const float* params_host, size_t n_params, int nb);
 int pnpx_unet_denoise_backward(pnpx_ctx* ctx, const float* x, const float* sigma, const float* grad_out,
@@ -249,12 +251,16 @@
   PNPX_PROBE_WINOF4_2SRC = 8,
   PNPX_PROBE_WINOF4_UPS = 9,
   PNPX_PROBE_WINOF4_FUSE_UP = 11,
-  PNPX_PROBE_WINOF4_C32 = 12
+  PNPX_PROBE_WINOF4_C32 = 12,
+  PNPX_PROBE_WINOF4_C32_OUTC = 13
 };
 int pnpx_conv3x3_probe(pnpx_ctx* ctx, int kind, const float* w_host, const float* bias_host, int cout, const float* in0, int C0,
                        const float* in1, int C1, float* out, const float* res, const float* mask, float slope, float* pool_out,
                        int ks_rule, int B, int H, int W, void* stream);
 int pnpx_conv3x3_probe_plan(int kind, int C0, int C1, int cout, int H, int W, int ks_rule);
+int pnpx_conv3x3_outc_probe(pnpx_ctx* ctx, const float* w_host, const float* bias_host, const float* outc_w_host, const float* outc_b_host,
+                            const float* in0, int cin, const float* x_img, float* img, float* img_pre, float* keep_out, int B, int H, int W,
+                            void* stream);
 int pnpx_upsample2x_probe(pnpx_ctx* ctx, const float* src, float* dst, int planes, int h, int w, void* stream);
 
 typedef struct pnpx_conv_hs_probe_desc {
@@ -297,6 +303,7 @@
 
 int pnpx_conv_f32_entry_plan(int opts, int ksplit, int ksplit_rule, int C0, int C1, int cout, int H, int W, int B_call);
 int pnpx_conv_f32_forward_plan(int opts, int ksplit, int ksplit_rule, int C0, int C1, int cout, int H, int W, int B_call);
+int pnpx_conv_f32_last_plan(int opts, int ksplit, int ksplit_rule, int cin, int cout, int H, int W, int B_call);
 
 #ifdef __cplusplus
 }
diff --git a/tfpnp_amd/_lib.py b/tfpnp_amd/_lib.py
--- a/tfpnp_amd/_lib.py
+++ b/tfpnp_amd/_lib.py
@@ -52,6 +52,7 @@
     "pnpx_drunet_num_params": (C.c_size_t, [C.c_int]),
     "pnpx_drunet_load": (C.c_int, [c_void_p, c_void_p, C.c_size_t, C.c_int]),
     "pnpx_unet_denoise": (C.c_int, [c_void_p, _P, _P, _P, _P, C.c_int, C.c_int, C.c_int, c_void_p]),
+    "pnpx_unet_denoise_keep": (C.c_int, [c_void_p, _P, _P, _P, _P, C.c_int, C.c_int, C.c_int, c_void_p]),
     "pnpx_unet_denoise_backward": (C.c_int, [c_void_p, _P, _P, _P, _P, _P, C.c_int, C.c_int, C.c_int, c_void_p]),
     "pnpx_unet_denoise_train": (C.c_int, [c_void_p, _P, _P, _P, C.c_int, C.c_int, C.c_int, C.POINTER(C.c_ulonglong), c_void_p]),
     "pnpx_unet_denoise_backward_ticket": (C.c_int, [c_void_p, _P, _P, _P, _P, _P, C.c_int, C.c_int, C.c_int,
@@ -164,6 +165,9 @@
     "pnpx_conv_f32_entry_plan": (C.c_int, [C.c_int] * 9),
     "pnpx_conv_f32_forward_plan": (C.c_int, [C.c_int] * 9),
     "pnpx_winof4_c32_pack": (C.c_int, [c_void_p, C.c_int, C.c_int, c_void_p]),
+    "pnpx_conv_f32_last_plan": (C.c_int, [C.c_int] * 8),
+    "pnpx_conv3x3_outc_probe": (C.c_int, [c_void_p, c_void_p, c_void_p, c_void_p, c_void_p, _P, C.c_int, _P, _P, _P, _P,
+                                          C.c_int, C.c_int, C.c_int, c_void_p]),
     "pnpx_conv_hs_probe": (C.c_int, [c_void_p, c_void_p, c_void_p]),
     "pnpx_conv_hs_probe_plan": (C.c_int, [c_void_p, C.c_int, C.c_int, C.c_int, C.POINTER(C.c_int)]),
     "pnpx_vjp_glue_probe": (C.c_int, [c_void_p, c_void_p, c_void_p]),
diff --git a/tfpnp_amd/csrc/api.hip b/tfpnp_amd/csrc/api.hip
--- a/tfpnp_amd/csrc/api.hip
+++ b/tfpnp_amd/csrc/api.hip
@@ -389,8 +389,10 @@
     {"fp32_winof4_layers", &pnpx_ctx::opt_fp32_winof4, 0, (1 << 27) - 1},
     {"fp32_winof4_entries", &pnpx_ctx::opt_fp32_winof4_entries, 0, (1 << 27) - 1},
     {"fp32_winof4_fuse_up", &pnpx_ctx::opt_fp32_winof4_fuse_up, 0, (1 << 27) - 1},
+    {"fp32_winof4_outc", &pnpx_ctx::opt_fp32_winof4_outc, 0, 1},
 };
 constexpr int WINOF4_C32_BITS = (1 << 1) | (1 << 2) | (1 << 25);
+constexpr int WINOF4_C32_PACKED = WINOF4_C32_BITS | (1 << 26);
 const PlainOption* plain_option(const char* key) {
   for (const PlainOption& o : PLAIN_OPTIONS)
     if (key && !std::strcmp(key, o.name)) return &o;
@@ -603,7 +605,7 @@
     const float* wsrc = params_host;
     for (int i = 0; i < 27; ++i) {
       u4c32off[i] = 0;
-      if (((WINOF4_C32_BITS >> i) & 1) && conv3x3_winof4_c32_packs(L[i].cout, L[i].cin)) {
+      if (((WINOF4_C32_PACKED >> i) & 1) && conv3x3_winof4_c32_packs(L[i].cout, L[i].cin)) {
         align();
         u4c32off[i] = host.size();
         host.resize(host.size() + conv3x3_winof4_floats(L[i].cout, L[i].cin));
@@ -703,6 +705,18 @@
   });
 }
 
+int pnpx_unet_denoise_keep(pnpx_ctx* ctx, const float* x, const float* sigma, float* out, float* out_preclamp, int B, int H, int W,
+                           void* stream) {
+  LOCK_CTX(ctx);
+  return pnpx::guarded(ctx, static_cast<hipStream_t>(stream), [&]() -> int {
+    if (!x || !sigma || !out) {
+      set_error("pnpx_unet_denoise_keep: null pointer");
+      return PNPX_ERR_ARG;
+    }
+    return unet_denoise(ctx, x, sigma, 1, out, out_preclamp, B, H, W, static_cast<hipStream_t>(stream), nullptr, &ctx->arena, -1, true);
+  });
+}
+
 int pnpx_unet_denoise_backward(pnpx_ctx* ctx, const float* x, const float* sigma, const float* grad_out, float* grad_x,
                                float* grad_sigma, int B, int H, int W, void* stream) {
   LOCK_CTX(ctx);
diff --git a/tfpnp_amd/csrc/common.h b/tfpnp_amd/csrc/common.h
--- a/tfpnp_amd/csrc/common.h
+++ b/tfpnp_amd/csrc/common.h
@@ -198,7 +198,8 @@
   int opt_fp32_winof4_entries = (1 << 15) | (1 << 18) | (1 << 21);
   int opt_fp32_winof4_fuse_up = 1 << 21;
   float* conv_winof4_c32_u[27] = {};
-  int opt_fp32_winof4_c32 = (1 << 1) | (1 << 25);
+  int opt_fp32_winof4_c32 = (1 << 1) | (1 << 2) | (1 << 25);
+  int opt_fp32_winof4_outc = 0;
   int opt_fp32_chains = 2;
   int opt_fp32_ksplit = 1;
   int opt_ksplit_rule = 1;
diff --git a/tfpnp_amd/csrc/conv3x3.h b/tfpnp_amd/csrc/conv3x3.h
--- a/tfpnp_amd/csrc/conv3x3.h
+++ b/tfpnp_amd/csrc/conv3x3.h
@@ -65,6 +65,9 @@
 void pack_conv_weights_winof4_c32(const float* w, int cout, int cin, float* dst);
 int launch_conv3x3_winof4_c32(const float* u, const float* bias, int cout, const float* in0, int C0, float* out, int B, int H, int W,
                               hipStream_t s, float slope = 0.2f, float* pool_out = nullptr);
+bool conv3x3_winof4_c32_outc_ok(int cin, int cout, int H, int W);
+int launch_conv3x3_winof4_c32_outc(const float* u, const float* bias, const float* in0, int cin, const float* outc_w, const float* outc_b,
+                                   const float* x_img, float* img, float* img_pre, float* keep_out, int B, int H, int W, hipStream_t s);
 bool conv3x3_winof4_ups_ok(int C0, int C1, int cout, int H, int W);
 int launch_conv3x3_winof4_ups(const float* u, const float* bias, int cout, const float* in0, int C0, const float* in1_lowres, int C1,
                               float* out, int B, int H, int W, hipStream_t s, float slope = 0.2f);
diff --git a/tfpnp_amd/csrc/conv3x3_winof4.hip b/tfpnp_amd/csrc/conv3x3_winof4.hip
--- a/tfpnp_amd/csrc/conv3x3_winof4.hip
+++ b/tfpnp_amd/csrc/conv3x3_winof4.hip
@@ -184,7 +184,9 @@
     for (int j = 0; j < 6; ++j) acc[i][j] = (f32x4){0.f, 0.f, 0.f, 0.f};
 }
 
-__device__ __forceinline__ void epilogue_tile(const WinoArgs& a, const f32x4 (&acc)[6][6], int HpWp, const Tile& T, int ty, int tx, int cbase) {
+template <bool OUTC = false>
+__device__ __forceinline__ void epilogue_tile(const WinoArgs& a, const f32x4 (&acc)[6][6], int HpWp, const Tile& T, int ty, int tx, int cbase,
+                                              f32x4* osum = nullptr) {
   float* ob = a.out + ((size_t)T.b * a.Cout + cbase) * HpWp + (size_t)(T.y0 + 4 * ty + 1) * a.Wp + T.x0 + 4 * tx + PADL;
   const int Hp_pool = padded_h(a.H / 2), Wp_pool = padded_w(a.W / 2);
   const size_t HpWp_pool = (size_t)Hp_pool * Wp_pool;
@@ -192,6 +194,14 @@
   float bias4[4];
 #pragma unroll
   for (int j = 0; j < 4; ++j) bias4[j] = a.bias[cbase + j];
+  float ow4[4];
+  if constexpr (OUTC) {
+#pragma unroll
+    for (int j = 0; j < 4; ++j) ow4[j] = a.outc_w[cbase + j];
+#pragma unroll
+    for (int i = 0; i < 4; ++i) osum[i] = (f32x4){0.f, 0.f, 0.f, 0.f};
+  }
+  const bool keep = !OUTC || a.out != nullptr;
   static_for<4>([&](auto j_tag) {
     constexpr int j = decltype(j_tag)::value;
     float s[4][6];
@@ -209,9 +219,15 @@
       y2 += bias;
       y3 += bias;
       y[i] = (f32x4){fmaxf(y0, y0 * a.slope), fmaxf(y1, y1 * a.slope), fmaxf(y2, y2 * a.slope), fmaxf(y3, y3 * a.slope)};
-      if (!(WINOF4_ABL & 32) || a.slope == 123.f) *reinterpret_cast<f32x4*>(o + i * a.Wp) = y[i];
-    }
-    if (a.pool && (!(WINOF4_ABL & 32) || a.slope == 123.f)) {
+      if constexpr (OUTC) {
+#pragma unroll
+        for (int e = 0; e < 4; ++e) osum[i][e] = fmaf(ow4[j], y[i][e], osum[i][e]);
+        if (keep && (!(WINOF4_ABL & 32) || a.slope == 123.f)) *reinterpret_cast<f32x4*>(o + i * a.Wp) = y[i];
+      } else {
+        if (!(WINOF4_ABL & 32) || a.slope == 123.f) *reinterpret_cast<f32x4*>(o + i * a.Wp) = y[i];
+      }
+    }
+    if (!OUTC && a.pool && (!(WINOF4_ABL & 32) || a.slope == 123.f)) {
       float* p = pb + (size_t)j * HpWp_pool;
       *reinterpret_cast<f32x2*>(p) = (f32x2){fmaxf(fmaxf(y[0][0], y[0][1]), fmaxf(y[1][0], y[1][1])), fmaxf(fmaxf(y[0][2], y[0][3]), fmaxf(y[1][2], y[1][3]))};
       *reinterpret_cast<f32x2*>(p + Wp_pool) = (f32x2){fmaxf(fmaxf(y[2][0], y[2][1]), fmaxf(y[3][0], y[3][1])), fmaxf(fmaxf(y[2][2], y[2][3]), fmaxf(y[3][2], y[3][3]))};
@@ -482,8 +498,11 @@
 
 using CfgF4C32 = GeoF4<32, 64, 2>;
 static_assert(CfgF4C32::LDS_USED <= LDS_REQF4 && CfgF4C32::RAW_PER_WAVE + 3 <= 24 && CfgF4C32::USTG == 12 * 1024, "32-cout instance");
-
-__global__ __launch_bounds__(512, 1) void conv3x3_winof4_c32_f32_kernel(WinoArgs a) {
+constexpr int OFF_Z_C32 = CfgF4C32::LDS_USED;
+static_assert(OFF_Z_C32 % 16 == 0 && OFF_Z_C32 + 4096 <= LDS_REQF4, "out-conv exchange region");
+
+template <bool OUTC>
+__device__ __forceinline__ void winof4_c32_body(const WinoArgs a) {
   using C = CfgF4C32;
   constexpr int CK = C::CK, RWL = C::RWL, RPXL = C::RPXL, RAW_BYTES = C::RAW_BYTES, RAW_PER_WAVE = C::RAW_PER_WAVE;
   constexpr int USTG = C::USTG, VSTG = C::VSTG, OFF_U = C::OFF_U, OFF_V = C::OFF_V, OFF_RAW = C::OFF_RAW;
@@ -553,7 +572,43 @@
     __builtin_amdgcn_s_barrier();
   };
 
-  auto epilogue = [&](const Tile& T) { epilogue_tile(a, acc, HpWp, T, sw, lane & 15, T.ct * 32 + P * 16 + 4 * (lane >> 4)); };
+  auto epilogue = [&](const Tile& T) {
+    if constexpr (!OUTC) {
+      epilogue_tile(a, acc, HpWp, T, sw, lane & 15, T.ct * 32 + P * 16 + 4 * (lane >> 4));
+    } else {
+      const int g = lane >> 4;
+      f32x4 os[4];
+      epilogue_tile<true>(a, acc, HpWp, T, sw, lane & 15, P * 16 + 4 * g, os);
+      const size_t px = ((size_t)T.b * a.H + T.y0 + 4 * sw + g) * a.W + T.x0 + 4 * (lane & 15);
+      f32x4 xi = {0.f, 0.f, 0.f, 0.f};
+      if (P == 0) xi = *reinterpret_cast<const f32x4*>(a.x_img + px);
+#pragma unroll
+      for (int i = 0; i < 4; ++i)
+#pragma unroll
+        for (int e = 0; e < 4; ++e) os[i][e] += __shfl_xor(os[i][e], 16);
+#pragma unroll
+      for (int i = 0; i < 4; ++i)
+#pragma unroll
+        for (int e = 0; e < 4; ++e) os[i][e] += __shfl_xor(os[i][e], 32);
+      const f32x4 mine = g == 0 ? os[0] : g == 1 ? os[1] : g == 2 ? os[2] : os[3];
+      char* zb = lds + OFF_Z_C32 + sw * 1024 + lane * 16;
+      if (P == 1) {
+        *reinterpret_cast<f32x4*>(zb) = mine;
+        asm volatile("s_waitcnt lgkmcnt(0)" ::: "memory");
+      }
+      __builtin_amdgcn_s_barrier();
+      if (P == 0) {
+        const f32x4 o = *reinterpret_cast<const f32x4*>(zb);
+        const float ob0 = a.outc_b[0];
+        f32x4 v;
+#pragma unroll
+        for (int e = 0; e < 4; ++e) v[e] = xi[e] + ((mine[e] + o[e]) + ob0);
+        *reinterpret_cast<f32x4*>(a.img_pre + px) = v;
+        *reinterpret_cast<f32x4*>(a.img + px) = (f32x4){fminf(fmaxf(v[0], 0.f), 1.f), fminf(fmaxf(v[1], 0.f), 1.f), fminf(fmaxf(v[2], 0.f), 1.f),
+                                                        fminf(fmaxf(v[3], 0.f), 1.f)};
+      }
+    }
+  };
 
   using I0 = std::integral_constant<int, 0>;
   using I1 = std::integral_constant<int, 1>;
@@ -595,6 +650,9 @@
   if (wave < 4) body(std::integral_constant<int, 0>{});
   else body(std::integral_constant<int, 1>{});
 }
+
+__global__ __launch_bounds__(512, 1) void conv3x3_winof4_c32_f32_kernel(WinoArgs a) { winof4_c32_body<false>(a); }
+__global__ __launch_bounds__(512, 1) void conv3x3_winof4_c32_f32_kernel_outc(WinoArgs a) { winof4_c32_body<true>(a); }
 
 }
 
@@ -632,13 +690,19 @@
   return C1 == 0 && C0 >= 16 && C0 % 8 == 0 && cout > 0 && cout % 32 == 0 && cout % 64 != 0 && H >= 16 && H % 16 == 0 && W >= 64 && W % 64 == 0;
 }
 bool conv3x3_winof4_c32_packs(int cout, int cin) { return conv3x3_winof4_c32_ok(cin, 0, cout, 16, 64); }
+bool conv3x3_winof4_c32_outc_ok(int cin, int cout, int H, int W) { return cout == 32 && conv3x3_winof4_c32_ok(cin, 0, cout, H, W); }
 void pack_conv_weights_winof4_c32(const float* w, int cout, int cin, float* dst) { pack_winof4(w, cout, cin, dst, CfgF4C32::CT); }
 
-enum class F4Inst { PLAIN, ENTRY, UPS, C32 };
+enum class F4Inst { PLAIN, ENTRY, UPS, C32, C32_OUTC };
+struct F4Outc {
+  const float *w, *b, *x_img;
+  float *img, *img_pre;
+};
 static int launch_winof4(F4Inst inst, const float* u, const float* bias, int cout, const float* in0, int C0, const float* in1, int C1, float* out,
-                         int B, int H, int W, hipStream_t s, float slope, float* pool_out) {
-  const bool c32 = inst == F4Inst::C32, ups = inst == F4Inst::UPS;
-  const bool ok = c32 ? conv3x3_winof4_c32_ok(C0, C1, cout, H, W)
+                         int B, int H, int W, hipStream_t s, float slope, float* pool_out, const F4Outc* outc = nullptr) {
+  const bool c32 = inst == F4Inst::C32 || inst == F4Inst::C32_OUTC, ups = inst == F4Inst::UPS;
+  const bool ok = inst == F4Inst::C32_OUTC ? conv3x3_winof4_c32_outc_ok(C0, cout, H, W)
+                  : c32 ? conv3x3_winof4_c32_ok(C0, C1, cout, H, W)
                   : ups ? conv3x3_winof4_ups_ok(C0, C1, cout, H, W)
                         : inst == F4Inst::ENTRY ? conv3x3_winof4_entry_ok(C0, C1, cout, H, W) : conv3x3_winof4_ok(C0, C1, cout, H, W);
   if (!ok) {
@@ -653,6 +717,13 @@
   a.bias = bias;
   a.pool = pool_out;
   a.out = out;
+  if (outc) {
+    a.outc_w = outc->w;
+    a.outc_b = outc->b;
+    a.x_img = outc->x_img;
+    a.img = outc->img;
+    a.img_pre = outc->img_pre ? outc->img_pre : outc->img;
+  }
   a.B = B;
   a.H = H;
   a.W = W;
@@ -675,15 +746,15 @@
     a.ups_sx = (float)(W / 2 - 1) / (float)(W - 1);
   }
   using Kernel = void (*)(WinoArgs);
-  static const Kernel kernels[4] = {conv3x3_winof4_f32_kernel<false>, conv3x3_winof4_f32_kernel<true>, conv3x3_winof4_f32_kernel<true, true>,
-                                    conv3x3_winof4_c32_f32_kernel};
+  static const Kernel kernels[5] = {conv3x3_winof4_f32_kernel<false>, conv3x3_winof4_f32_kernel<true>, conv3x3_winof4_f32_kernel<true, true>,
+                                    conv3x3_winof4_c32_f32_kernel, conv3x3_winof4_c32_f32_kernel_outc};
   static std::once_flag attr_once[64];
   int dev = 0;
   PNPX_HIP(hipGetDevice(&dev));
   if (dev >= 0 && dev < 64) {
     hipError_t e = hipSuccess;
     std::call_once(attr_once[dev], [&] {
-      for (int i = 0; i < 4 && e == hipSuccess; ++i)
+      for (int i = 0; i < 5 && e == hipSuccess; ++i)
         e = hipFuncSetAttribute(reinterpret_cast<const void*>(kernels[i]), hipFuncAttributeMaxDynamicSharedMemorySize, LDS_REQF4);
     });
     PNPX_HIP(e);
@@ -709,6 +780,15 @@
                               hipStream_t s, float slope, float* pool_out) {
   return launch_winof4(F4Inst::C32, u, bias, cout, in0, C0, nullptr, 0, out, B, H, W, s, slope, pool_out);
 }
+int launch_conv3x3_winof4_c32_outc(const float* u, const float* bias, const float* in0, int cin, const float* outc_w, const float* outc_b,
+                                   const float* x_img, float* img, float* img_pre, float* keep_out, int B, int H, int W, hipStream_t s) {
+  if (!outc_w || !outc_b || !x_img || !img) {
+    set_error("conv3x3_winof4_c32_outc: null out-conv operand");
+    return PNPX_ERR_ARG;
+  }
+  const F4Outc o{outc_w, outc_b, x_img, img, img_pre};
+  return launch_winof4(F4Inst::C32_OUTC, u, bias, 32, in0, cin, nullptr, 0, keep_out, B, H, W, s, 0.2f, nullptr, &o);
+}
 
 }
 
diff --git a/tfpnp_amd/csrc/conv_f32_select.h b/tfpnp_amd/csrc/conv_f32_select.h
--- a/tfpnp_amd/csrc/conv_f32_select.h
+++ b/tfpnp_amd/csrc/conv_f32_select.h
@@ -19,6 +19,7 @@
   bool winof4_entry = false;
   bool winof4_fuse_up = false;
   bool winof4_c32 = false;
+  bool winof4_outc = false;
   int ksplit = 0;
   int ksplit_rule = 1;
   bool fuse_up = false;
diff --git a/tfpnp_amd/csrc/conv_f32_select.hip b/tfpnp_amd/csrc/conv_f32_select.hip
--- a/tfpnp_amd/csrc/conv_f32_select.hip
+++ b/tfpnp_amd/csrc/conv_f32_select.hip
@@ -10,6 +10,7 @@
   v.winof4_entry = (ctx->opt_fp32_winof4_entries >> li) & 1;
   v.winof4_fuse_up = (ctx->opt_fp32_winof4_fuse_up >> li) & 1;
   v.winof4_c32 = (ctx->opt_fp32_winof4_c32 >> li) & 1;
+  v.winof4_outc = li == 26 && ctx->opt_fp32_winof4_outc != 0;
   v.ksplit = ctx->opt_fp32_ksplit;
   v.ksplit_rule = ctx->opt_ksplit_rule;
   v.fuse_up = ctx->opt_fp32_fuse_up != 0;
@@ -64,6 +65,7 @@
   if (v.winograd && v.u && conv3x3_wino_outc_ok(cin, cout, H, W)) {
     c.fused = true;
     c.kernel = v.wino8 && conv3x3_wino8_ok(cin, 0, cout, H, W) ? ConvF32Kernel::Wino8 : ConvF32Kernel::Wino4;
+    if (c.kernel == ConvF32Kernel::Wino8 && v.winof4_outc && v.u_f4c32 && conv3x3_winof4_c32_outc_ok(cin, cout, H, W)) c.kernel = ConvF32Kernel::WinoF4C32;
   }
   return c;
 }
@@ -140,3 +142,21 @@
   const pnpx::ConvF32Choice c = (opts & 128) ? pnpx::conv_f32_last(v, C0, cout, H, W, B_call) : pnpx::conv_f32_forward(v, C0, C1, cout, H, W, B_call);
   return static_cast<int>(c.kernel) + 16 * c.pieces + 256 * (c.fused ? 1 : 0);
 }
+
+extern "C" int pnpx_conv_f32_last_plan(int opts, int ksplit, int ksplit_rule, int cin, int cout, int H, int W, int B_call) {
+  static const float packed = 0.f;
+  pnpx::ConvF32Sel v;
+  v.winograd = opts & 1;
+  v.wino8 = opts & 2;
+  v.winof4 = opts & 4;
+  v.winof4_c32 = opts & 8;
+  v.u = (opts & 16) ? &packed : nullptr;
+  v.u_f4 = (opts & 32) ? &packed : nullptr;
+  v.u_f4c32 = (opts & 64) ? &packed : nullptr;
+  v.winof4_outc = opts & 256;
+  v.ksplit = ksplit;
+  v.ksplit_rule = ksplit_rule;
+  if (cin <= 0 || cout <= 0 || H <= 0 || W <= 0 || B_call <= 0) return -1;
+  const pnpx::ConvF32Choice c = pnpx::conv_f32_last(v, cin, cout, H, W, B_call);
+  return static_cast<int>(c.kernel) + 16 * c.pieces + 256 * (c.fused ? 1 : 0);
+}
diff --git a/tfpnp_amd/csrc/conv_probe.hip b/tfpnp_amd/csrc/conv_probe.hip
--- a/tfpnp_amd/csrc/conv_probe.hip
+++ b/tfpnp_amd/csrc/conv_probe.hip
@@ -37,6 +37,7 @@
     case PNPX_PROBE_WINOF4_UPS: return 0;
     case PNPX_PROBE_WINOF4_FUSE_UP: return C1 > 0 && conv3x3_winof4_ups_ok(C0, C1, cout, H, W) ? 64 : 0;
     case PNPX_PROBE_WINOF4_C32: return conv3x3_winof4_c32_ok(C0, C1, cout, H, W) ? 32 : 0;
+    case PNPX_PROBE_WINOF4_C32_OUTC: return C1 == 0 && conv3x3_winof4_c32_outc_ok(C0, cout, H, W) ? 32 : 0;
   }
   return 0;
 }
@@ -52,6 +53,10 @@
   PNPX_HIP(hipSetDevice(ctx->device));
   hipStream_t s = static_cast<hipStream_t>(stream);
   const bool grad = is_grad(kind);
+  if (kind == PNPX_PROBE_WINOF4_C32_OUTC) {
+    set_error("pnpx_conv3x3_probe: kind %d takes the out-conv operands of pnpx_conv3x3_outc_probe", kind);
+    return PNPX_ERR_ARG;
+  }
   if (kind < PNPX_PROBE_DIRECT || (kind > PNPX_PROBE_WINOF4_UPS && kind != PNPX_PROBE_WINOF4_FUSE_UP && kind != PNPX_PROBE_WINOF4_C32)) {
     set_error("pnpx_conv3x3_probe: unknown kind %d", kind);
     return PNPX_ERR_ARG;
@@ -168,6 +173,52 @@
   return rc;
 }
 
+extern "C" int pnpx_conv3x3_outc_probe(pnpx_ctx* ctx, const float* w_host, const float* bias_host, const float* outc_w_host, const float* outc_b_host,
+                                       const float* in0, int cin, const float* x_img, float* img, float* img_pre, float* keep_out, int B, int H, int W,
+                                       void* stream) {
+  if (!ctx) {
+    set_error("null context");
+    return PNPX_ERR_ARG;
+  }
+  std::lock_guard<std::mutex> lk(ctx->mu);
+  PNPX_HIP(hipSetDevice(ctx->device));
+  hipStream_t s = static_cast<hipStream_t>(stream);
+  if (!w_host || !bias_host || !outc_w_host || !outc_b_host || !in0 || !x_img || !img || B <= 0 || H <= 0 || W <= 0 || cin <= 0) {
+    set_error("pnpx_conv3x3_outc_probe: null pointer or non-positive size");
+    return PNPX_ERR_ARG;
+  }
+  if (!pnpx_conv3x3_probe_plan(PNPX_PROBE_WINOF4_C32_OUTC, cin, 0, 32, H, W, 1)) {
+    const int rc = launch_conv3x3_winof4_c32_outc(nullptr, nullptr, in0, cin, outc_w_host, outc_b_host, x_img, img, img_pre, keep_out, B, H, W, s);
+    if (rc == PNPX_OK) {
+      set_error("pnpx_conv3x3_outc_probe: the plan refuses a geometry the launcher accepts (%d -> 32 channels, %d x %d)", cin, H, W);
+      return PNPX_ERR_SHAPE;
+    }
+    return rc;
+  }
+  std::vector<float> host(conv3x3_winof4_floats(32, cin));
+  pack_conv_weights_winof4_c32(w_host, 32, cin, host.data());
+  host.resize((host.size() + 255) & ~(size_t)255, 0.f);
+  const size_t boff = host.size();
+  host.insert(host.end(), bias_host, bias_host + 32);
+  const size_t owoff = host.size();
+  host.insert(host.end(), outc_w_host, outc_w_host + 32);
+  const size_t oboff = host.size();
+  host.push_back(outc_b_host[0]);
+  host.resize(host.size() + 1024, 0.f);
+  DeviceBuf wbuf;
+  int rc = alloc_dev(wbuf, host.size() * sizeof(float), "probe weight");
+  if (rc == PNPX_OK) {
+    const hipError_t e = hipMemcpy(wbuf.p, host.data(), host.size() * sizeof(float), hipMemcpyHostToDevice);
+    if (e != hipSuccess) rc = hip_fail(e, "hipMemcpy(probe weights)", __FILE__, __LINE__);
+  }
+  const float* d = static_cast<const float*>(wbuf.p);
+  if (rc == PNPX_OK) rc = launch_conv3x3_winof4_c32_outc(d, d + boff, in0, cin, d + owoff, d + oboff, x_img, img, img_pre, keep_out, B, H, W, s);
+  const hipError_t e = hipStreamSynchronize(s);
+  if (wbuf.p) (void)hipFree(wbuf.p);
+  if (rc == PNPX_OK && e != hipSuccess) rc = hip_fail(e, "hipStreamSynchronize(probe)", __FILE__, __LINE__);
+  return rc;
+}
+
 extern "C" int pnpx_upsample2x_probe(pnpx_ctx* ctx, const float* src, float* dst, int planes, int h, int w, void* stream) {
   if (!ctx || !src || !dst || planes <= 0 || h <= 0 || w <= 0) {
     set_error("pnpx_upsample2x_probe: null pointer or non-positive size");
diff --git a/tfpnp_amd/csrc/unet.hip b/tfpnp_amd/csrc/unet.hip
--- a/tfpnp_amd/csrc/unet.hip
+++ b/tfpnp_amd/csrc/unet.hip
@@ -120,6 +120,33 @@
   float acc = 0.f;
 #pragma unroll
   for (int c = 0; c < 32; ++c) acc = fmaf(w[c], f[(size_t)c * Hp * Wp], acc);
+  const size_t o = ((size_t)b * H + y) * W + xx;
+  const float v = x[o] + (acc + bias[0]);
+  if (out_pre) out_pre[o] = v;
+  out[o] = fminf(fmaxf(v, 0.f), 1.f);
+}
+
+__global__ void outc_residual_wino8_order_kernel(const float* __restrict__ feat, const float* __restrict__ x,
+                                                 const float* __restrict__ w, const float* __restrict__ bias,
+                                                 float* __restrict__ out, float* __restrict__ out_pre, int H, int W) {
+  const int Hp = padded_h(H), Wp = padded_w(W);
+  const int xx = blockIdx.x * blockDim.x + threadIdx.x;
+  const int y = blockIdx.y;
+  const int b = blockIdx.z;
+  if (xx >= W) return;
+  const float* f = feat + (size_t)b * 32 * Hp * Wp + (size_t)(y + 1) * Wp + xx + PADL;
+  float c[4];
+#pragma unroll
+  for (int q = 0; q < 4; ++q) {
+    float s = 0.f;
+#pragma unroll
+    for (int j = 0; j < 8; ++j) {
+      const int R = 8 * (q >> 1) + j, co = 4 * (q & 1) + (R & 3) + 8 * (R >> 2);
+      s = fmaf(w[co], f[(size_t)co * Hp * Wp], s);
+    }
+    c[q] = s;
+  }
+  const float acc = (c[0] + c[1]) + (c[2] + c[3]);
   const size_t o = ((size_t)b * H + y) * W + xx;
   const float v = x[o] + (acc + bias[0]);
   if (out_pre) out_pre[o] = v;
@@ -648,9 +675,14 @@
       PNPX_TRY(launch_conv3x3_wino8_ups(ctx->conv_wino_u[li0], L.b, L.cout, fptr(P.x[l]), P.x[l].C, fptr(*below), below->C, fptr(ta), B, 2 * h, 2 * w, s));
       return rec.mark("conv3x3_wino", 2.0 * 9.0 * L.cin * L.cout * (double)(2 * h) * (2 * w) * B);
     };
-    if (l == 0 && !keep_all && ctx->opt_fuse_outc && c26.fused) {
+    const bool f4_outc = c26.kernel == ConvF32Kernel::WinoF4C32;
+    if (l == 0 && ctx->opt_fuse_outc && c26.fused && (!keep_all || f4_outc)) {
       PNPX_TRY(entry(P.da[0]));
       PNPX_TRY(conv(25, P.da[0], nullptr, P.db[0]));
+      if (f4_outc)
+        PNPX_TRY(launch_conv3x3_winof4_c32_outc(ctx->conv_winof4_c32_u[26], ctx->conv[26].b, fptr(P.db[0]), ctx->conv[26].cin, ctx->outc_w, ctx->outc_b,
+                                                x, out, out_pre, keep_all ? fptr(P.y[0]) : nullptr, B, H, W, s));
+      else
       PNPX_TRY((c26.kernel == ConvF32Kernel::Wino8 ? launch_conv3x3_wino8_outc : launch_conv3x3_wino_outc)(
           ctx->conv_wino_u[26], ctx->conv[26].b, fptr(P.db[0]), ctx->conv[26].cin, ctx->outc_w, ctx->outc_b, x, out, out_pre, B, H, W, s));
       return rec.mark("conv3x3_wino", 2.0 * 9.0 * ctx->conv[26].cin * ctx->conv[26].cout * (double)H * W * B);
@@ -660,8 +692,9 @@
     PNPX_TRY(conv(li0 + 2, P.db[l], nullptr, P.y[l]));
     below = &P.y[l];
   }
-  hipLaunchKernelGGL(outc_residual_kernel, dim3((W + 63) / 64, H, B), dim3(64), 0, s, fptr(P.y[0]), x, ctx->outc_w,
-                     ctx->outc_b, out, out_pre, H, W);
+  const bool wino8_order = keep_all && ctx->opt_fuse_outc && c26.fused && c26.kernel == ConvF32Kernel::Wino8;
+  hipLaunchKernelGGL(wino8_order ? outc_residual_wino8_order_kernel : outc_residual_kernel, dim3((W + 63) / 64, H, B), dim3(64), 0, s, fptr(P.y[0]), x,
+                     ctx->outc_w, ctx->outc_b, out, out_pre, H, W);
   PNPX_LAUNCH_CHECK();
   PNPX_TRY(rec.mark("outc_residual_clamp", 2.0 * 32 * (double)H * W * B));
   return PNPX_OK;
```

Result: no change. 142.7 iters/s (median of 6 runs) (+1.0%).
